# RyoK3N/Camera-Aware-Neural-Networks-for-Few-View-Depth-Estimation

Measured on AMD Instinct MI355X. Metric: images/sec (640×480 bs32) at 1/2/4/8 MI355X; abs_rel vs CPU ref, higher is better.
Workload: dtype fp32; 1 GPU; baseline_unet train step, configs[1]: bs32/GPU 480x640 fp32 SI-only loss; model=baseline, global_batch=32, height=480, width=640, init_features=64, params=31037633, parallelism=dp1, optimizer=adam(lr1e-4,wd1e-5)+clip1.0

## Files before the change

camera-aware-neural-networks-for-few-view-depth-estimation_amd/csrc/host/cad_api.cpp:

```cpp
#include <hip/hip_runtime.h>

#include <algorithm>
#include <cmath>
#include <cstdio>
#include <cstdlib>
#include <cstring>
#include <deque>
#include <memory>
#include <random>
#include <stdexcept>
#include <string>
#include <vector>

#include "../../../include/cad/cad.h"
#include "../kernels/eval_align.hpp"
#include "../kernels/kernels.hpp"

namespace {

thread_local std::string g_err;

struct CadError : std::runtime_error {
    cad_status st;
    CadError(cad_status s, const std::string& m) : std::runtime_error(m), st(s) {}
};

#define HIPCHK(expr)                                                                            \
    do {                                                                                        \
        hipError_t e_ = (expr);                                                                 \
        if (e_ != hipSuccess)                                                                   \
            throw CadError(e_ == hipErrorOutOfMemory ? CAD_ERR_OOM : CAD_ERR_HIP,               \
                           std::string(#expr) + ": " + hipGetErrorString(e_));                 \
    } while (0)

void require(bool c, const std::string& m, cad_status s = CAD_ERR_INVALID) {
    if (!c) throw CadError(s, m);
}

template <class F>
cad_status guard(F&& f) {
    try {
        f();
        return CAD_OK;
    } catch (const CadError& e) {
        g_err = e.what();
        return e.st;
    } catch (const std::exception& e) {
        g_err = e.what();
        return CAD_ERR_INVALID;
    }
}

inline hipStream_t S(void* s) { return reinterpret_cast<hipStream_t>(s); }

struct Arena {
    char* base = nullptr;
    size_t off = 0;
    void* take(size_t bytes) {
        off = (off + 255) & ~size_t(255);
        void* p = base ? base + off : nullptr;
        off += bytes;
        return p;
    }
    float* f(int64_t n) { return static_cast<float*>(take(sizeof(float) * (size_t)std::max<int64_t>(n, 1))); }
    double* d(int64_t n) { return static_cast<double*>(take(sizeof(double) * (size_t)std::max<int64_t>(n, 1))); }
    uint8_t* u8(int64_t n) { return static_cast<uint8_t*>(take((size_t)std::max<int64_t>(n, 1))); }
    int* i(int64_t n) { return static_cast<int*>(take(sizeof(int) * (size_t)std::max<int64_t>(n, 1))); }
};

enum PKind {
    P_CONV3, P_BNW, P_BNB, P_CONVT_W, P_CONVT_B, P_HEAD_W, P_HEAD_B,
    P_FC_W, P_FC_B,
    P_FILM_HEAD_W, P_FILM_GAMMA_B, P_FILM_BETA_B,
    P_SCONV
};

struct PInfo {
    std::string name;
    int ndim;
    int64_t shape[4];
    PKind kind;
    int64_t off;
    int64_t n_int;
    int64_t n_ref;
    int cin_ref = 0, cin_int = 0, cout = 0;
};

struct BufInfo {
    std::string name;
    int64_t C;
    float* ptr;
};

struct BN {
    int C = 0, widx = -1, bidx = -1;
    float *rm = nullptr, *rv = nullptr;
    float *mean = nullptr, *invstd = nullptr, *scale = nullptr, *shift = nullptr, *coef = nullptr;
};
struct Conv {
    int pidx = -1, cin = 0, cout = 0;
    float* wd = nullptr;
    void *ws = nullptr, *wds = nullptr;
};
struct Film {
    int p0 = -1;
    float *rm1, *rv1, *rm2, *rv2;
    float *xh1, *h1, *xh2, *h2, *is1, *is2, *gam, *bet, *dgam, *dbet, *dh2, *dh1;
};
struct DoubleConv {
    Conv c1, c2;
    BN b1, b2;
    Film film;
    int level = 0;
    float *y1 = nullptr, *a1 = nullptr, *y2 = nullptr;
    bool y1b = false, y2b = false;
    bool y1_f32 = false;
    void* a1s = nullptr;
    int first_param = 0, last_param = 0;
    bool has_film() const { return film.p0 >= 0; }
};
struct Up {
    int widx = -1, bidx = -1, cin = 0, cout = 0;
    float* wf = nullptr;
    void *wfs = nullptr, *wms = nullptr;
};

}

namespace cad {
void set_last_error(const std::string& msg) { g_err = msg; }
}

struct cad_unet {
    int device = 0;
    int model = CAD_MODEL_BASELINE;
    int in_ch = 3, f = 64, Bmax = 1, H = 0, W = 0;
    int x0_ld = 8;
    float* camn = nullptr;
    float max_depth = 10.f;
    bool train = true;
    bool have_fwd = false;
    int64_t nbt = 0, nbt_film = 0;
    int fwd_B = 0;
    std::vector<PInfo> params;
    std::vector<BufInfo> bufs;
    int64_t n_flat = 0;
    float *flat_p = nullptr, *flat_g = nullptr;
    float* norm_coef = nullptr;
    void* arena_base = nullptr;
    hipStream_t side = nullptr;
    hipEvent_t ev_fork = nullptr, evA = nullptr, evB = nullptr, ev_tail = nullptr;
    bool defer_join = false;
    float* Sb2 = nullptr;
    void* dYs2 = nullptr;
    double* dscr2 = nullptr;
    DoubleConv enc[5];
    DoubleConv dec[4];
    Up up[4];
    int head_w = -1, head_b = -1;
    int att_p0[4] = {-1, -1, -1, -1};
    cad::Cbam att[4];
    float* zatt[4] = {};
    float* Sd = nullptr;
    float *hq = nullptr, *hdp = nullptr;
    bool att_head_fused = false;
    bool attn() const { return model == CAD_MODEL_INTRINSICS_ATTN; }
    float* x0 = nullptr;
    float* cat[4] = {};
    float* pool[5] = {};
    uint8_t* pidx[5] = {};
    float* a2_bott = nullptr;
    float* dout[4] = {};
    float* sig = nullptr;
    void* x0s = nullptr;
    void* cats[4] = {};
    void* pools[5] = {};
    void* botts = nullptr;
    void* douts[4] = {};
    void* dcats[4] = {};
    void* dskips[4] = {};
    void* dYs = nullptr;
    int fwd_np = 0;
    bool head_fused = false;
    float* dcat[4] = {};
    float *Sa = nullptr, *Sb = nullptr, *Sc = nullptr;
// ... 88 lines not shown
    for (int l = 3; l >= 0; --l) {
        for (int i = h->dec[l].first_param; i <= h->dec[l].last_param; ++i) order.push_back(i);
        for (int j = 0; j < 5; ++j) order.push_back(h->att_p0[l] + j);
    }
    order.push_back(h->head_w);
    order.push_back(h->head_b);
    if (order.size() != h->params.size()) throw std::runtime_error("internal: attention slab order misses a parameter");
    int64_t off = 0;
    for (int i : order) {
        off = (off + 63) & ~int64_t(63);
        h->params[i].off = off;
        off += h->params[i].n_int;
    }
    h->n_flat = (off + 63) & ~int64_t(63);
}

void build_tables(cad_unet* h) {
    const int f = h->f;
    if (h->model == CAD_MODEL_RAY_FILM)
        add_double_conv(h, h->enc[0], "enc1.", h->in_ch + 3, 8, f, 0);
    else
        add_double_conv(h, h->enc[0], "enc1.", h->in_ch, 8, f, 0);
    h->enc[0].y1_f32 = h->model != CAD_MODEL_RAY_FILM;
    const char* enames[4] = {"enc2", "enc3", "enc4", "bottleneck"};
    for (int i = 0; i < 4; ++i)
        add_double_conv(h, h->enc[i + 1], std::string(enames[i]) + ".conv.", f << i, f << i, f << (i + 1), i + 1);
    for (int k = 0; k < 4; ++k) {
        const int l = 3 - k;
        const int cin = f << (l + 1), cout = f << l;
        const std::string pre = "dec" + std::to_string(l + 1) + ".";
        add_param(h, pre + "up.weight", {cin, cout, 2, 2}, P_CONVT_W);
        add_param(h, pre + "up.bias", {cout}, P_CONVT_B);
        h->up[l] = Up{(int)h->params.size() - 2, (int)h->params.size() - 1, cin, cout, nullptr};
        add_double_conv(h, h->dec[l], pre + "conv.", cin, cin, cout, l);
        h->dec[l].first_param = h->up[l].widx;
    }
    if (h->attn()) {
        for (int l = 3; l >= 0; --l) {
            const int C = f << l, Cr = std::max(1, C / 16);
            const std::string pre = "att" + std::to_string(l + 1) + ".";
            h->att_p0[l] = (int)h->params.size();
            add_param(h, pre + "channel_attention.fc1.weight", {Cr, C}, P_FC_W);
            add_param(h, pre + "channel_attention.fc1.bias", {Cr}, P_FC_B);
            add_param(h, pre + "channel_attention.fc2.weight", {C, Cr}, P_FC_W);
            add_param(h, pre + "channel_attention.fc2.bias", {C}, P_FC_B);
            add_param(h, pre + "spatial_attention.conv.weight", {1, 2, 7, 7}, P_SCONV);
        }
    }
    add_param(h, "out_conv.weight", {1, f, 1, 1}, P_HEAD_W);
    add_param(h, "out_conv.bias", {1}, P_HEAD_B);
    h->head_w = (int)h->params.size() - 2;
    h->head_b = (int)h->params.size() - 1;
    h->n_flat = (h->n_flat + 63) & ~int64_t(63);
    if (h->attn()) assign_attn_slab_offsets(h);
}

void bn_alloc(Arena& a, BN& b) {
    b.rm = a.f(b.C); b.rv = a.f(b.C);
    b.mean = a.f(b.C); b.invstd = a.f(b.C); b.scale = a.f(b.C); b.shift = a.f(b.C); b.coef = a.f(3 * b.C);
}

void film_alloc(Arena& a, DoubleConv& dc, int B) {
    if (!dc.has_film()) return;
    Film& F = dc.film;
    const int H1 = cad::kFilmH1, H2 = cad::kFilmH2, C = dc.c1.cout;
    F.rm1 = a.f(H1); F.rv1 = a.f(H1); F.rm2 = a.f(H2); F.rv2 = a.f(H2);
    F.xh1 = a.f((int64_t)B * H1); F.h1 = a.f((int64_t)B * H1); F.dh1 = a.f((int64_t)B * H1);
    F.xh2 = a.f((int64_t)B * H2); F.h2 = a.f((int64_t)B * H2); F.dh2 = a.f((int64_t)B * H2);
    F.is1 = a.f(H1); F.is2 = a.f(H2);
    F.gam = a.f((int64_t)B * C); F.bet = a.f((int64_t)B * C);
    F.dgam = a.f((int64_t)B * C); F.dbet = a.f((int64_t)B * C);
}

void layout(cad_unet* h, Arena& a) {
    const int B = h->Bmax;
    const bool film = h->model != CAD_MODEL_BASELINE;
    auto sp = [&](int64_t elems) -> void* { return a.take((size_t)elems * 2 * cad::kMaxPlanes); };
    auto conv_split_alloc = [&](Conv& c, bool dgrad) {
        if (c.cin % 8) return;
        const int64_t n = (int64_t)c.cout * 9 * c.cin;
        c.ws = sp(n);
        if (dgrad) c.wds = sp(n);
    };
    h->flat_p = a.f(h->n_flat);
    h->flat_g = a.f(h->n_flat);
    h->norm_coef = a.f(4);
    h->camn = a.f((int64_t)B * 4);
    for (int l = 0; l < 5; ++l) {
        DoubleConv& e = h->enc[l];
        bn_alloc(a, e.b1); bn_alloc(a, e.b2);
        const int64_t MC = h->Ml(l, B) * h->Cl(l);
        e.y1 = a.f(MC); e.y2 = a.f(MC);
        e.a1 = a.f(MC);
        e.a1s = sp(MC);
        film_alloc(a, e, B);
        if (l > 0) e.c1.wd = a.f((int64_t)e.c1.cout * 9 * e.c1.cin);
        e.c2.wd = a.f((int64_t)e.c2.cout * 9 * e.c2.cin);
        conv_split_alloc(e.c1, l > 0);
        conv_split_alloc(e.c2, true);
        if (l < 4) { h->cat[l] = a.f(2 * MC); h->cats[l] = sp(2 * MC); }
        if (l > 0) {
            h->pool[l] = a.f(h->Ml(l, B) * h->Cl(l - 1));
            h->pools[l] = sp(h->Ml(l, B) * h->Cl(l - 1));
            h->pidx[l] = a.u8(h->Ml(l, B) * h->Cl(l - 1));
        }
    }
    h->a2_bott = a.f(h->Ml(4, B) * h->Cl(4));
    h->botts = sp(h->Ml(4, B) * h->Cl(4));
    for (int l = 0; l < 4; ++l) {
        DoubleConv& d = h->dec[l];
        bn_alloc(a, d.b1); bn_alloc(a, d.b2);
        const int64_t MC = h->Ml(l, B) * h->Cl(l);
        d.y1 = a.f(MC); d.y2 = a.f(MC);
        d.a1 = a.f(MC);
        d.a1s = sp(MC);
        film_alloc(a, d, B);
        h->dout[l] = a.f(MC);
        if (l > 0) h->douts[l] = sp(MC);
        d.c1.wd = a.f((int64_t)d.c1.cout * 9 * d.c1.cin);
        d.c2.wd = a.f((int64_t)d.c2.cout * 9 * d.c2.cin);
        conv_split_alloc(d.c1, true);
        conv_split_alloc(d.c2, true);
        h->up[l].wf = a.f((int64_t)4 * h->up[l].cout * h->up[l].cin);
        h->up[l].wfs = sp((int64_t)4 * h->up[l].cout * h->up[l].cin);
        h->up[l].wms = sp((int64_t)4 * h->up[l].cout * h->up[l].cin);
        h->dcat[l] = a.f(2 * MC);
        h->dcats[l] = sp(MC);
        h->dskips[l] = sp(MC);
    }
    h->x0 = a.f(h->Ml(0, B) * h->x0_ld);
    if (h->x0_ld % 8 == 0) h->x0s = sp(h->Ml(0, B) * h->x0_ld);
    h->dYs = sp(h->Ml(0, B) * h->Cl(0));
    h->sig = a.f(h->Ml(0, B));
    const int64_t M0C0 = h->Ml(0, B) * h->Cl(0);
    h->Sa = a.f(M0C0);
    h->Sb = a.f(M0C0);
    h->Sb2 = a.f(M0C0);
    h->dYs2 = sp(h->Ml(0, B) * h->Cl(0));
    h->Sc = a.f(h->Ml(1, B) * h->Cl(0));
    if (h->attn()) {
        h->Sd = a.f(M0C0);
        for (int l = 0; l < 4; ++l) {
            const int C = h->Cl(l), Cr = std::max(1, C / 16);
            const int64_t M = h->Ml(l, B);
            const bool fused = l == 0 && cad::head_fusable(C);
            h->zatt[l] = fused ? nullptr : a.f(M * C);
            cad::Cbam& A = h->att[l];
            A.C = C; A.Cr = Cr;
            A.avg = a.f((int64_t)B * C); A.mx = a.f((int64_t)B * C); A.amax = a.i((int64_t)B * C);
            A.ha = a.f((int64_t)B * Cr); A.hm = a.f((int64_t)B * Cr); A.att = a.f((int64_t)B * C);
            A.s = a.f(2 * M); A.sidx = a.i(M); A.sa = a.f(M);
            A.dlog = a.f(M); A.ds = a.f(2 * M);
            A.dO = a.f((int64_t)B * C); A.dha = a.f((int64_t)B * Cr); A.dhm = a.f((int64_t)B * Cr);
            A.dva = a.f((int64_t)B * C); A.dvm = a.f((int64_t)B * C);
            if (fused) { h->hq = a.f(M); h->hdp = a.f(M); }
        }
    }
    int64_t st = 0, colmax = 0;
    for (int l = 0; l < 5; ++l) {
        const int64_t r = (h->Ml(l, B) + 63) / 64;
        st = std::max<int64_t>(st, r * (2 * h->Cl(l) + 1));
        colmax = std::max<int64_t>(colmax, h->Cl(l));
    }
    h->stats = a.f(st);
    int64_t dscr = (int64_t)(cad::colsum_slices(h->Ml(0, B)) + 2) * 4 * colmax + 4 * colmax + 8192;
    for (int l = 0; l < 5 && film; ++l)
        dscr = std::max(dscr, cad::film_reduce_doubles(B, (int64_t)h->Hl(l) * h->Wl(l), h->Cl(l)) + 8192);
    for (int l = 0; l < 4 && h->attn(); ++l)
        dscr = std::max(dscr, cad::cbam_head_scratch_doubles(B, (int64_t)h->Hl(l) * h->Wl(l), h->Cl(l)) + 8192);
    h->dscr = a.d(dscr);
    h->dscr2 = a.d(dscr);
    int64_t sl = 0;
    for (int l = 0; l < 5; ++l) {
        const int64_t Kp = h->Ml(l, B);
        sl = std::max(sl, cad::wgrad_slab_floats(h->Cl(l), 9 * h->Cl(l) * 2, (int)std::min<int64_t>(Kp, INT32_MAX)));
    }
    h->slab_cap = std::min<int64_t>(sl, (int64_t)64 << 20);
    h->slab = a.f(h->slab_cap);
    h->part_cap = (h->Ml(0, B) + 63) / 64 * 2 * h->Cl(0);
    h->rc_part = a.d(h->part_cap);
    h->bufs.clear();
    auto add_bn_bufs = [&](const std::string& pre, BN& b) {
        h->bufs.push_back({pre + ".running_mean", b.C, b.rm});
        h->bufs.push_back({pre + ".running_var", b.C, b.rv});
    };
    auto add_block = [&](const std::string& pre, DoubleConv& dc) {
        add_bn_bufs(pre + "bn1", dc.b1);
        add_bn_bufs(pre + "bn2", dc.b2);
        if (!dc.has_film()) return;
        h->bufs.push_back({pre + "film.bn1.running_mean", cad::kFilmH1, dc.film.rm1});
        h->bufs.push_back({pre + "film.bn1.running_var", cad::kFilmH1, dc.film.rv1});
        h->bufs.push_back({pre + "film.bn2.running_mean", cad::kFilmH2, dc.film.rm2});
        h->bufs.push_back({pre + "film.bn2.running_var", cad::kFilmH2, dc.film.rv2});
    };
    const char* en[5] = {"enc1.", "enc2.conv.", "enc3.conv.", "enc4.conv.", "bottleneck.conv."};
    for (int l = 0; l < 5; ++l) add_block(en[l], h->enc[l]);
    for (int k = 0; k < 4; ++k) {
        const int l = 3 - k;
        add_block("dec" + std::to_string(l + 1) + ".conv.", h->dec[l]);
    }
}

cad::FilmLayer film_view(const cad_unet* h, const DoubleConv& dc) {
    const Film& F = dc.film;
    const int i = F.p0;
    cad::FilmLayer L;
    L.C = dc.c1.cout;
    L.w1 = h->P(i); L.b1 = h->P(i + 1); L.w2 = h->P(i + 2); L.b2 = h->P(i + 3);
    L.wg = h->P(i + 4); L.bg = h->P(i + 5); L.wb = h->P(i + 6); L.bb = h->P(i + 7);
    L.g1 = h->P(i + 8); L.be1 = h->P(i + 9); L.g2 = h->P(i + 10); L.be2 = h->P(i + 11);
    L.rm1 = F.rm1; L.rv1 = F.rv1; L.rm2 = F.rm2; L.rv2 = F.rv2;
    L.xh1 = F.xh1; L.h1 = F.h1; L.xh2 = F.xh2; L.h2 = F.h2; L.is1 = F.is1; L.is2 = F.is2;
    L.gam = F.gam; L.bet = F.bet; L.dgam = F.dgam; L.dbet = F.dbet; L.dh2 = F.dh2; L.dh1 = F.dh1;
    L.gw1 = h->G(i); L.gb1 = h->G(i + 1); L.gw2 = h->G(i + 2); L.gb2 = h->G(i + 3);
    L.gwg = h->G(i + 4); L.gbg = h->G(i + 5); L.gwb = h->G(i + 6); L.gbb = h->G(i + 7);
    L.gg1 = h->G(i + 8); L.gbe1 = h->G(i + 9); L.gg2 = h->G(i + 10); L.gbe2 = h->G(i + 11);
    return L;
}

cad::Cbam cbam_view(const cad_unet* h, int l) {
    cad::Cbam A = h->att[l];
    const int i = h->att_p0[l];
    A.w1 = h->P(i); A.b1 = h->P(i + 1); A.w2 = h->P(i + 2); A.b2 = h->P(i + 3); A.wsp = h->P(i + 4);
    A.gw1 = h->G(i); A.gb1 = h->G(i + 1); A.gw2 = h->G(i + 2); A.gb2 = h->G(i + 3); A.gwsp = h->G(i + 4);
    return A;
}
cad::CbamHead cbam_head_view(const cad_unet* h) {
    const DoubleConv& d = h->dec[0];
    cad::CbamHead Hd;
    Hd.y = d.y2; Hd.y_bf16 = d.y2b;
    Hd.scale = d.b2.scale; Hd.shift = d.b2.shift;
    Hd.w = h->P(h->head_w); Hd.b = h->P(h->head_b);
    Hd.md = h->max_depth;
    Hd.q = h->hq; Hd.sig = h->sig; Hd.dp = h->hdp;
    Hd.gw = h->G(h->head_w); Hd.gb = h->G(h->head_b);
    return Hd;
}

cad::Split sv(const void* p, int64_t ld, int coff = 0) {
    cad::Split v;
    v.p = p; v.ld = ld; v.coff = coff;
    return v;
}
void split_into(const float* x, int64_t ldx, int xcoff, int C, int64_t M, void* out, int64_t ldo, int ocoff,
                hipStream_t st) {
    if (out) cad::split_rows(x, ldx, xcoff, C, M, out, ldo, ocoff, st);
}
void wprep_add(cad::WPrepList& L, int kind, const float* src, float* d32, void* d16, int cout, int cin, int64_t n) {
    if (!d32 && !d16) return;
    if (L.njobs == cad::kWPrepMaxJobs) throw std::runtime_error("weight_prep: job list full");
    cad::WPrepJob& j = L.job[L.njobs++];
    j.src = src; j.d32 = d32; j.d16 = d16; j.kind = kind; j.cout = cout; j.cin = cin; j.n = n;
}
void prep_fwd_weights(const cad_unet* h, bool ps, hipStream_t st) {
    cad::WPrepList L{};
    for (int l = 0; l < 4; ++l) {
        const Up& u = h->up[l];
        wprep_add(L, cad::WPREP_CONVT, h->P(u.widx), u.wf, ps ? u.wfs : nullptr, u.cout, u.cin, (int64_t)4 * u.cout * u.cin);
    }
    if (ps) {
        auto sw = [&](const Conv& c) {
            if (c.ws) wprep_add(L, cad::WPREP_SPLIT, h->P(c.pidx), nullptr, c.ws, c.cout, c.cin, (int64_t)c.cout * 9 * c.cin);
        };
        for (int l = 0; l < 5; ++l) { sw(h->enc[l].c1); sw(h->enc[l].c2); }
        for (int l = 0; l < 4; ++l) { sw(h->dec[l].c1); sw(h->dec[l].c2); }
    }
    cad::weight_prep(L, st);
}

int env_flag(const char* name, int dflt) {
    const char* e = std::getenv(name);
    return e && e[0] ? std::atoi(e) : dflt;
}
bool conv1_presplit(cad_unet* h, const DoubleConv& dc, bool ps, const cad::Split& in_s) {
    static const bool enc1_ps = env_flag("CAD_ENC1PS", 1) != 0;
    return ps && in_s.p && dc.c1.ws && (enc1_ps || &dc != &h->enc[0]);
}
struct PoolOut {
    float* pool;
    uint8_t* idx;
    void* pool_s;
};
bool bn_pool_on() {
    static const bool on = env_flag("CAD_BNPOOL", 1) != 0;
    return on;
}

void double_conv_fwd(cad_unet* h, DoubleConv& dc, const float* in, int64_t ldin, cad::Split in_s, int B, float* out,
                     int64_t ldo, int ocoff, cad::Split out_s, hipStream_t st, bool out_f32 = true,
                     float* head_pred = nullptr, const PoolOut* pool = nullptr, bool att_head = false) {
    const int l = dc.level, Hh = h->Hl(l), Ww = h->Wl(l), C = dc.c1.cout;
    const int64_t M = h->Ml(l, B);
    const bool tr = h->train;
    const bool ps = h->fwd_np > 0;
    auto bn = [&](BN& b, int cin, bool ps_conv) {
        const int rows = cad::conv3x3_stats_rows(cin, B, Hh, Ww, C, ps_conv);
        if (tr)
            cad::bn_fwd_finalize(h->stats, rows, C, M, h->P(b.widx), h->P(b.bidx), b.rm, b.rv, 0.1f, 1e-5f, h->dscr,
                                 b.mean, b.invstd, b.scale, b.shift, st);
        else
            cad::bn_eval_coeffs(h->P(b.widx), h->P(b.bidx), b.rm, b.rv, C, 1e-5f, b.mean, b.invstd, b.scale, b.shift, st);
    };
    float* stats = tr ? h->stats : nullptr;
    const bool ps1 = conv1_presplit(h, dc, ps, in_s);
    static const bool enc1_bf16 = env_flag("CAD_ENC1BF16", 0) != 0;
    dc.y1b = ps1 && (!dc.y1_f32 || enc1_bf16);
    dc.y2b = ps;
    if (ps1) {
        cad::conv3x3_fwd_ps(in_s, dc.c1.cin, sv(dc.c1.ws, 9 * dc.c1.cin), C, dc.y1, C, 0, B, Hh, Ww, stats, st, dc.y1b);
    } else {
        cad::conv3x3_fwd(in, ldin, 0, dc.c1.cin, h->P(dc.c1.pidx), C, dc.y1, C, 0, B, Hh, Ww, stats, st);
    }
    bn(dc.b1, dc.c1.cin, ps1);
    if (dc.has_film()) {
        cad::film_apply(dc.y1, C, dc.b1.scale, dc.b1.shift, dc.film.gam, dc.film.bet, B, (int64_t)Hh * Ww,
                        ps ? nullptr : dc.a1, st, dc.y1b, ps ? dc.a1s : nullptr);
    } else {
        cad::bn_relu_fwd(dc.y1, C, dc.b1.scale, dc.b1.shift, ps ? nullptr : dc.a1, C, 0, M, st, ps ? dc.a1s : nullptr,
                         C, 0, dc.y1b);
    }
    if (ps)
        cad::conv3x3_fwd_ps(sv(dc.a1s, C), C, sv(dc.c2.ws, 9 * C), C, dc.y2, C, 0, B, Hh, Ww, stats, st, true);
    else
        cad::conv3x3_fwd(dc.a1, C, 0, C, h->P(dc.c2.pidx), C, dc.y2, C, 0, B, Hh, Ww, stats, st);
    bn(dc.b2, C, ps);
    if (head_pred && att_head) {
        cad::cbam_head_fwd(cbam_view(h, 0), cbam_head_view(h), B, Hh, Ww, head_pred, h->dscr, st);
        return;
    }
    if (head_pred) {
        cad::bn_relu_head_fwd(dc.y2, C, dc.b2.scale, dc.b2.shift, h->P(h->head_w), h->P(h->head_b), h->max_depth, h->sig,
                              head_pred, M, st, dc.y2b);
        return;
    }
    const bool twin = ps && out_s.p;
    if (pool) {
        if (ocoff != 0 || (twin && out_s.coff != 0)) throw std::runtime_error("bn_relu_pool_fwd: offset outputs");
        cad::bn_relu_pool_fwd(dc.y2, C, dc.b2.scale, dc.b2.shift, (out_f32 || !twin) ? out : nullptr, ldo,
                              twin ? const_cast<void*>(out_s.p) : nullptr, out_s.ld, B, Hh, Ww, dc.y2b, pool->pool,
                              pool->idx, pool->pool_s, st);
        return;
    }
    cad::bn_relu_fwd(dc.y2, C, dc.b2.scale, dc.b2.shift, (out_f32 || !twin) ? out : nullptr, ldo, ocoff, M, st,
                     twin ? const_cast<void*>(out_s.p) : nullptr, out_s.ld, out_s.coff, dc.y2b);
}

bool dcat_split_on() {
    static const bool on = env_flag("CAD_DCATSPLIT", 1) != 0;
    return on;
}

bool pool_fold_on() {
    static const bool on = env_flag("CAD_POOLFOLD", 1) != 0;
    return on;
}

bool head_fusion_on() {
    static const bool on = [] {
        const char* e = std::getenv("CAD_HEADFUSE");
        return !(e && e[0] == '0');
    }();
    return on;
}

void unet_forward(cad_unet* h, const float* rgb, const float* cam4, float* depth, int B, hipStream_t st) {
    const int f = h->f;
    h->fwd_np = h->f % 8 ? 0 : cad::split_planes();
    const bool ps = h->fwd_np > 0;
    prep_fwd_weights(h, ps, st);
    if (h->model != CAD_MODEL_BASELINE) {
        cad::camera_normalize(cam4, B, h->H, h->W, h->camn, st);
        cad::FilmList fl;
        for (int l = 0; l < 5; ++l) fl.l[fl.n++] = film_view(h, h->enc[l]);
        for (int l = 3; l >= 0; --l) fl.l[fl.n++] = film_view(h, h->dec[l]);
        cad::film_mlp_fwd_all(fl, h->camn, B, h->train, st);
    }
    if (h->model == CAD_MODEL_RAY_FILM)
        cad::rgb_rays_to_nhwc8(rgb, cam4, B, h->H, h->W, h->x0, st);
    else
        cad::rgb_to_nhwc8(rgb, h->x0, B, h->H, h->W, st);
    const cad::Split none{};
    cad::Split x0s = none;
    if (ps && h->x0s) {
        cad::split_rows(h->x0, h->x0_ld, 0, h->x0_ld, h->Ml(0, B), h->x0s, h->x0_ld, 0, st);
        x0s = sv(h->x0s, h->x0_ld);
    }
    auto pool_of = [&](int l) {
        const bool ptwin = ps && h->pools[l];
        return PoolOut{ptwin ? nullptr : h->pool[l], h->pidx[l], ptwin ? h->pools[l] : nullptr};
    };
    const bool fuse_pool = bn_pool_on();
    PoolOut po = pool_of(1);
    double_conv_fwd(h, h->enc[0], h->x0, h->x0_ld, x0s, B, h->cat[0], 2 * f, 0, sv(h->cats[0], 2 * f), st, !ps, nullptr,
                    fuse_pool ? &po : nullptr);
    for (int l = 1; l <= 4; ++l) {
        const int Cp = h->Cl(l - 1);
        if (!fuse_pool) {
            const PoolOut p = pool_of(l);
            cad::maxpool_fwd(ps ? static_cast<const float*>(h->cats[l - 1]) : h->cat[l - 1], 2 * Cp, Cp, B, h->Hl(l - 1),
                             h->Wl(l - 1), p.pool, p.idx, st, p.pool_s, ps);
        }
        const cad::Split pin = sv(h->pools[l], Cp);
        if (l < 4) {
            po = pool_of(l + 1);
            double_conv_fwd(h, h->enc[l], h->pool[l], Cp, pin, B, h->cat[l], 2 * h->Cl(l), 0,
                            sv(h->cats[l], 2 * h->Cl(l)), st, !ps, nullptr, fuse_pool ? &po : nullptr);
        } else {
// ... 3 lines not shown
    }
    const bool attn = h->attn();
    h->head_fused = !attn && head_fusion_on() && cad::head_fusable(f);
    h->att_head_fused = attn && cad::head_fusable(f);
    for (int l = 3; l >= 0; --l) {
        const float* upin = l == 3 ? h->a2_bott : h->dout[l + 1];
        const void* upins = l == 3 ? h->botts : h->douts[l + 1];
        const Up& u = h->up[l];
        const int C = h->Cl(l);
        if (ps) {
            cad::convT_fwd_ps(sv(upins, u.cin), u.cin, sv(u.wfs, u.cin), h->P(u.bidx), u.cout,
                              static_cast<float*>(h->cats[l]), 2 * C, C, B, h->Hl(l + 1), h->Wl(l + 1), st, true);
        } else {
            cad::convT_fwd(upin, u.cin, u.cin, u.wf, h->P(u.bidx), u.cout, h->cat[l], 2 * C, C, B, h->Hl(l + 1),
                           h->Wl(l + 1), st);
        }
        if (attn) {
            if (l == 0 && h->att_head_fused) {
                double_conv_fwd(h, h->dec[0], h->cat[0], 2 * C, sv(h->cats[0], 2 * C), B, nullptr, C, 0, none, st, true,
                                depth, nullptr, true);
                continue;
            }
            double_conv_fwd(h, h->dec[l], h->cat[l], 2 * C, sv(h->cats[l], 2 * C), B, h->zatt[l], C, 0, none, st, true);
            cad::cbam_fwd(cbam_view(h, l), h->zatt[l], B, h->Hl(l), h->Wl(l), h->dout[l], C, 0, h->dscr, st);
            if (ps && l > 0) cad::split_rows(h->dout[l], C, 0, C, h->Ml(l, B), h->douts[l], C, 0, st);
            continue;
        }
        double_conv_fwd(h, h->dec[l], h->cat[l], 2 * C, sv(h->cats[l], 2 * C), B, h->dout[l], C, 0,
                        l > 0 ? sv(h->douts[l], C) : none, st, l == 0, l == 0 && h->head_fused ? depth : nullptr);
    }
    if (!h->head_fused && !h->att_head_fused)
        cad::head_fwd(h->dout[0], f, h->P(h->head_w), h->P(h->head_b), h->max_depth, h->sig, depth, h->Ml(0, B), st);
}

void side_fork(cad_unet* h, hipStream_t st) {
    HIPCHK(hipEventRecord(h->ev_fork, st));
    HIPCHK(hipStreamWaitEvent(h->side, h->ev_fork, 0));
}
void side_join(cad_unet* h, hipStream_t st) {
    HIPCHK(hipEventRecord(h->ev_tail, h->side));
    HIPCHK(hipStreamWaitEvent(st, h->ev_tail, 0));
}
hipStream_t wgrad_stream(cad_unet* h, bool ps, hipStream_t st) {
    const int f = env_flag("CAD_SIDE_WGRAD", -1);
    const bool side = f < 0 ? !ps : f != 0;
    if (!side) return st;
    side_fork(h, st);
    return h->side;
}

void double_conv_bwd(cad_unet* h, DoubleConv& dc, const float* g, int64_t ldg, int gcoff, const float* in,
                     int64_t ldin, cad::Split in_s, int B, float* din, int64_t lddin, hipStream_t st,
                     const cad::HeadGrad* head = nullptr, const cad::PoolAdd* pool = nullptr, void* din_hi = nullptr,
                     bool* din_hi_done = nullptr, bool g_bf16 = false, bool din_bf16 = false) {
    const int l = dc.level, Hh = h->Hl(l), Ww = h->Wl(l), C = dc.c1.cout;
    const int64_t M = h->Ml(l, B);
    const bool ps = h->fwd_np > 0 && h->fwd_np == cad::split_planes();
    hipStream_t sd = h->side;
    float* dY = h->Sb;
    void* dYs = h->dYs;
    float* dY1 = h->Sb2;
    void* dYs1 = h->dYs2;
    float* dA1 = h->Sa;
    HIPCHK(hipStreamWaitEvent(st, h->evA, 0));
    cad::bn_relu_bwd(g, ldg, gcoff, dc.y2, C, dc.b2.mean, dc.b2.invstd, dc.b2.scale, dc.b2.shift, h->P(dc.b2.widx), M,
                     h->dscr, dc.b2.coef, h->G(dc.b2.widx), h->G(dc.b2.bidx), ps ? nullptr : dY, st, nullptr, 1,
                     ps ? dYs : nullptr, true, dc.y2b, head, g_bf16, pool);
    static const bool bnsums = env_flag("CAD_BNSUMS", 1) != 0;
    int bn1_tiles = 0;
    cad::BnSums bs;
    if (bnsums && !ps && !dc.has_film() && h->rc_part) {
        bs.y = dc.y1; bs.ldy = C; bs.y_bf16 = dc.y1b;
        bs.mean = dc.b1.mean; bs.invstd = dc.b1.invstd; bs.scale = dc.b1.scale; bs.shift = dc.b1.shift;
        bs.part = h->rc_part; bs.part_cap = h->part_cap;
    }
    hipStream_t wg = wgrad_stream(h, ps, st);
    if (ps) {
        cad::conv3x3_wgrad_ps(sv(dYs, C), C, sv(dc.a1s, C), C, h->G(dc.c2.pidx), B, Hh, Ww, h->slab, h->slab_cap, wg);
        HIPCHK(hipEventRecord(h->evA, wg));
        cad::conv3x3_dgrad_ps(sv(dYs, C), C, sv(dc.c2.wds, 9 * C), C, dA1, C, B, Hh, Ww, st, true);
    } else {
        cad::conv3x3_wgrad(dY, C, dc.a1, C, 0, C, h->G(dc.c2.pidx), B, Hh, Ww, h->slab, h->slab_cap, wg);
        HIPCHK(hipEventRecord(h->evA, wg));
        if (bs.part) bn1_tiles = cad::conv3x3_dgrad_bnsums(dY, C, dc.c2.wd, C, dA1, C, B, Hh, Ww, bs, st);
        if (!bn1_tiles) cad::conv3x3_dgrad(dY, C, dc.c2.wd, C, dA1, C, B, Hh, Ww, st);
    }
    const int64_t HW = (int64_t)Hh * Ww;
    static const bool film_fuse = env_flag("CAD_FILMFUSE", 1) != 0;
    const bool film_sep = dc.has_film() && !film_fuse;
    if (film_sep)
        cad::film_affine_bwd(dA1, dc.y1, C, dc.b1.scale, dc.b1.shift, B, HW, h->dscr, dc.film.dgam, dc.film.dbet, st,
                             dc.y1b, ps);
    const bool ps1 = conv1_presplit(h, dc, ps, in_s);
    const bool dy1_f32 = !ps1 || (din && !(ps && dc.c1.wds));
    HIPCHK(hipStreamWaitEvent(st, h->evB, 0));
    {
        const bool ff = dc.has_film() && !film_sep;
        cad::bn_relu_bwd(dA1, C, 0, dc.y1, C, dc.b1.mean, dc.b1.invstd, dc.b1.scale, dc.b1.shift, h->P(dc.b1.widx), M,
                         h->dscr, dc.b1.coef, h->G(dc.b1.widx), h->G(dc.b1.bidx), dy1_f32 ? dY1 : nullptr, st,
                         dc.has_film() ? dc.film.gam : nullptr, HW, ps ? dYs1 : nullptr, true, dc.y1b, nullptr, ps,
                         nullptr, ff ? dc.film.dgam : nullptr, ff ? dc.film.dbet : nullptr,
                         bn1_tiles ? h->rc_part : nullptr, bn1_tiles);
    }
    if (dc.has_film()) {
        side_fork(h, st);
        cad::film_mlp_bwd(film_view(h, dc), h->camn, B, sd);
    }
    hipStream_t wg1 = wgrad_stream(h, ps, st);
    if (ps1)
        cad::conv3x3_wgrad_ps(sv(dYs1, C), C, in_s, dc.c1.cin, h->G(dc.c1.pidx), B, Hh, Ww, h->slab, h->slab_cap, wg1);
    else
        cad::conv3x3_wgrad(dY1, C, in, ldin, 0, dc.c1.cin, h->G(dc.c1.pidx), B, Hh, Ww, h->slab, h->slab_cap, wg1);
    HIPCHK(hipEventRecord(h->evB, wg1));
    if (din) {
        if (ps && dc.c1.wds) {
            const bool done = cad::conv3x3_dgrad_ps(sv(dYs1, C), C, sv(dc.c1.wds, 9 * C), dc.c1.cin, din, lddin, B, Hh,
                                                    Ww, st, din_bf16, din_hi, dc.c1.cin / 2, dc.c1.cin / 2);
            if (din_hi_done) *din_hi_done = done && din_hi;
        } else
            cad::conv3x3_dgrad(dY1, C, dc.c1.wd, dc.c1.cin, din, lddin, B, Hh, Ww, st);
    }
}

void repack_dgrad_weights(cad_unet* h, hipStream_t st) {
    const bool ps = h->fwd_np > 0 && h->fwd_np == cad::split_planes();
    cad::WPrepList L{};
    auto rp = [&](Conv& c) {
        wprep_add(L, cad::WPREP_DGRAD, h->P(c.pidx), c.wd, ps ? c.wds : nullptr, c.cout, c.cin, (int64_t)c.cout * 9 * c.cin);
    };
    for (int l = 0; l < 5; ++l) {
        if (l > 0) rp(h->enc[l].c1);
        rp(h->enc[l].c2);
    }
    for (int l = 0; l < 4; ++l) {
        rp(h->dec[l].c1);
        rp(h->dec[l].c2);
        const Up& u = h->up[l];
        if (ps) wprep_add(L, cad::WPREP_SPLIT, h->P(u.widx), nullptr, u.wms, u.cout, u.cin, (int64_t)4 * u.cout * u.cin);
    }
    cad::weight_prep(L, st);
}

constexpr int kStages = 10;

void backward_stage_body(cad_unet* h, int stage, const float* dpred, hipStream_t st);
void backward_stage(cad_unet* h, int stage, const float* dpred, hipStream_t st) {
    backward_stage_body(h, stage, dpred, st);
    if (!h->defer_join) side_join(h, st);
}
void backward_stage_body(cad_unet* h, int stage, const float* dpred, hipStream_t st) {
    const int B = h->fwd_B;
    const int f = h->f;
    const bool ps = h->fwd_np > 0 && h->fwd_np == cad::split_planes();
    if (stage == 0) {
        HIPCHK(hipEventRecord(h->evA, st));
        HIPCHK(hipEventRecord(h->evB, st));
        repack_dgrad_weights(h, st);
        if (h->attn()) {
            if (h->att_head_fused) {
                cad::cbam_head_bwd(cbam_view(h, 0), cbam_head_view(h), dpred, B, h->H, h->W, h->Sa, h->dscr, st);
            } else {
                cad::head_bwd(h->dout[0], f, h->P(h->head_w), dpred, h->sig, h->max_depth, h->Sd, h->Ml(0, B), h->dscr,
                              h->G(h->head_w), h->G(h->head_b), st);
                cad::cbam_bwd(cbam_view(h, 0), h->zatt[0], h->Sd, f, 0, B, h->H, h->W, h->Sa, h->dscr, st);
            }
            return;
        }
        if (h->head_fused) {
            const DoubleConv& d = h->dec[0];
            cad::head_bwd_y(d.y2, f, d.b2.scale, d.b2.shift, dpred, h->sig, h->max_depth, h->Ml(0, B), h->dscr,
                            h->G(h->head_w), h->G(h->head_b), st, d.y2b);
        } else {
            cad::head_bwd(h->dout[0], f, h->P(h->head_w), dpred, h->sig, h->max_depth, h->Sa, h->Ml(0, B), h->dscr,
                          h->G(h->head_w), h->G(h->head_b), st);
        }
        return;
    }
    if (stage <= 4) {
        const int l = stage - 1;
        const int C = h->Cl(l);
        const cad::HeadGrad hg{dpred, h->sig, h->P(h->head_w), h->max_depth};
        const bool hf = l == 0 && h->head_fused;
        const bool split = ps && dcat_split_on() &&
                           cad::conv3x3_dgrad_split_ok(sv(h->dYs, C), C, sv(h->dec[l].c1.wds, 9 * C), 2 * C, h->Wl(l), C);
        bool up_twin = false;
        const bool attn = h->attn();
        const float* g = h->Sa;
        if (attn && l > 0) {
            cad::cbam_bwd(cbam_view(h, l), h->zatt[l], h->Sa, C, 0, B, h->Hl(l), h->Wl(l), h->Sd, h->dscr, st);
            g = h->Sd;
        }
        double_conv_bwd(h, h->dec[l], hf ? nullptr : g, C, 0, h->cat[l], 2 * C, sv(h->cats[l], 2 * C), B,
                        split ? static_cast<float*>(h->dskips[l]) : h->dcat[l], split ? C : 2 * C, st,
                        hf ? &hg : nullptr, nullptr, split ? h->dcats[l] : nullptr, &up_twin, ps && l > 0 && !attn, split);
        if (split != up_twin) throw std::runtime_error("decoder dgrad split store not taken");
        const Up& u = h->up[l];
        const float* upin = l == 3 ? h->a2_bott : h->dout[l + 1];
        const void* upins = l == 3 ? h->botts : h->douts[l + 1];
        if (ps && !split) {
            cad::split_rows(h->dcat[l], 2 * C, C, C, h->Ml(l, B), h->dcats[l], C, 0, st);
            cad::split_rows(h->dcat[l], 2 * C, 0, C, h->Ml(l, B), h->dskips[l], C, 0, st);
        }
        hipStream_t sd = wgrad_stream(h, ps, st);
        if (ps) {
            cad::convT_wgrad_ps(sv(upins, u.cin), u.cin, sv(h->dcats[l], C), u.cout, h->G(u.widx), B, h->Hl(l + 1),
                                h->Wl(l + 1), h->slab, h->slab_cap, sd);
        } else {
            cad::convT_wgrad(upin, u.cin, h->dcat[l], 2 * C, C, u.cout, h->G(u.widx), B, h->Hl(l + 1), h->Wl(l + 1),
                             h->slab, h->slab_cap, sd);
        }
        if (ps) cad::colsum_bf16(h->dcats[l], C, 0, h->Ml(l, B), C, h->dscr2, sd);
// ... 1495 lines not shown
        HIPCHK(hipEventRecord(b->staged, S(stream)));
        float* rgb_tmp = b->tmp;
        float* depth_tmp = b->tmp + 3 * (size_t)b->Bmax * H * W;
        cad::batch_assemble(b->dev, B, H, W, any_aug, any_color, rgb, depth, rgb_tmp, depth_tmp, S(stream));
        HIPCHK(hipGetLastError());
    });
}

struct cad_aug_sampler {
    cad_aug_config cfg;
    std::mt19937 rng;
};
cad_status cad_aug_sampler_create(const cad_aug_config* cfg, uint32_t seed, cad_aug_sampler** out) {
    return guard([&] {
        require(cfg && out, "null argument");
        require(cfg->crop_scale_min > 0.f && cfg->crop_scale_min <= cfg->crop_scale_max && cfg->crop_scale_max <= 1.f,
                "crop scale range must satisfy 0 < min <= max <= 1");
        require(cfg->saturation_delta >= 0.f && cfg->saturation_delta <= 1.f, "saturation_delta must be in [0, 1]");
        require(cfg->hue_delta >= 0.f && cfg->hue_delta <= 0.5f, "hue_delta must be in [0, 0.5]");
        if (cfg->enable_random_gamma) {
            require(std::isfinite(cfg->gamma_min) && cfg->gamma_min > 0.f, "gamma_min must be positive and finite");
            require(std::isfinite(cfg->gamma_max) && cfg->gamma_max >= cfg->gamma_min, "gamma_max must be finite and at least gamma_min");
        }
        auto s = std::make_unique<cad_aug_sampler>();
        s->cfg = *cfg;
        s->rng.seed(seed);
        *out = s.release();
    });
}
void cad_aug_sampler_destroy(cad_aug_sampler* s) { delete s; }
cad_status cad_aug_sampler_draw(cad_aug_sampler* s, int height, int width, cad_sample* smp) {
    return guard([&] {
        require(s && smp && height >= 1 && width >= 1, "bad arguments");
        const cad_aug_config& c = s->cfg;
        smp->aug = 1;
        smp->crop = c.enable_random_crop;
        if (c.enable_random_crop) {
            std::uniform_real_distribution<float> scale_dist(c.crop_scale_min, c.crop_scale_max);
            const float scale = scale_dist(s->rng);
            const int crop_h = static_cast<int>(height * scale), crop_w = static_cast<int>(width * scale);
            std::uniform_int_distribution<int> x_dist(0, std::max(1, width - crop_w));
            std::uniform_int_distribution<int> y_dist(0, std::max(1, height - crop_h));
            smp->crop_scale = scale;
            smp->crop_x = x_dist(s->rng);
            smp->crop_y = y_dist(s->rng);
        }
        smp->flip = 0;
        if (c.enable_horizontal_flip) {
            std::uniform_real_distribution<float> flip_dist(0.0f, 1.0f);
            smp->flip = flip_dist(s->rng) < c.horizontal_flip_prob;
        }
        smp->jitter = c.enable_color_jitter;
        if (c.enable_color_jitter) {
            std::uniform_real_distribution<float> bd(1.0f - c.brightness_delta, 1.0f + c.brightness_delta);
            std::uniform_real_distribution<float> cd(1.0f - c.contrast_delta, 1.0f + c.contrast_delta);
            smp->brightness = bd(s->rng);
            smp->contrast = cd(s->rng);
        }
        smp->color = 0; smp->saturation = 1.f; smp->hue = 0.f;
        if (c.enable_color_jitter && c.saturation_delta > 0.f) {
            std::uniform_real_distribution<float> sd(1.0f - c.saturation_delta, 1.0f + c.saturation_delta);
            smp->saturation = sd(s->rng);
            smp->color = 1;
        }
        if (c.enable_color_jitter && c.hue_delta > 0.f) {
            std::uniform_real_distribution<float> hd(-c.hue_delta, c.hue_delta);
            smp->hue = hd(s->rng);
            smp->color = 1;
        }
        smp->gamma_on = c.enable_random_gamma ? 1 : 0;
        smp->gamma = 1.f;
        if (c.enable_random_gamma) {
            std::uniform_real_distribution<float> gd(c.gamma_min, c.gamma_max);
            smp->gamma = gd(s->rng);
        }
    });
}

cad_status cad_op_conv3x3_fwd(const float* x, int64_t ldx, int xcoff, int cin, const float* w, int cout, float* y,
                              int64_t ldy, int ycoff, int B, int H, int W, void* stream) {
    return guard([&] {
        require(cin % 4 == 0 && cout % 4 == 0 && ldx % 4 == 0 && ldy % 4 == 0 && xcoff % 4 == 0 && ycoff % 4 == 0,
                "channels / strides must be multiples of 4");
        cad::conv3x3_fwd(x, ldx, xcoff, cin, w, cout, y, ldy, ycoff, B, H, W, nullptr, S(stream));
        HIPCHK(hipGetLastError());
    });
}
cad_status cad_op_conv3x3_dgrad(const float* dz, int cout, const float* w, int cin, float* dx, int64_t lddx, int B,
                                int H, int W, void* stream) {
    return guard([&] {
        require(cin % 4 == 0 && cout % 4 == 0, "channels must be multiples of 4");
        float* wd = nullptr;
        HIPCHK(hipMallocAsync((void**)&wd, sizeof(float) * (size_t)cout * 9 * cin, S(stream)));
        cad::repack_conv_dgrad(w, wd, cout, cin, S(stream));
        cad::conv3x3_dgrad(dz, cout, wd, cin, dx, lddx, B, H, W, S(stream));
        HIPCHK(hipFreeAsync(wd, S(stream)));
        HIPCHK(hipGetLastError());
    });
}
cad_status cad_op_conv3x3_wgrad(const float* dz, int cout, const float* x, int64_t ldx, int xcoff, int cin, float* dw,
                                int B, int H, int W, void* stream) {
    return guard([&] {
        require(cin % 4 == 0 && cout % 4 == 0, "channels must be multiples of 4");
        const int64_t cap = cad::wgrad_slab_floats(cout, 9 * cin, B * H * W);
        float* slab = nullptr;
        HIPCHK(hipMallocAsync((void**)&slab, sizeof(float) * (size_t)std::max<int64_t>(cap, 4), S(stream)));
        cad::conv3x3_wgrad(dz, cout, x, ldx, xcoff, cin, dw, B, H, W, slab, cap, S(stream));
        HIPCHK(hipFreeAsync(slab, S(stream)));
        HIPCHK(hipGetLastError());
    });
}
cad_status cad_op_conv3x3_wgrad_bf16(const void* dz, int64_t lddz, int cout, const void* x, int64_t ldx, int xcoff,
                                     int cin, float* dw, int B, int H, int W, void* stream) {
    return guard([&] {
        require(cad::gemm_engine() == 2, "the pre-split weight gradient runs on the bf16 engine (CAD_GEMM_BF16)");
        const int64_t cap = cad::wgrad_slab_floats(cout, 9 * cin, B * H * W);
        float* slab = nullptr;
        HIPCHK(hipMallocAsync((void**)&slab, sizeof(float) * (size_t)std::max<int64_t>(cap, 4), S(stream)));
        cad::conv3x3_wgrad_ps(cad::Split{dz, lddz, 0}, cout, cad::Split{x, ldx, xcoff}, cin, dw, B, H, W, slab, cap,
                              S(stream));
        HIPCHK(hipFreeAsync(slab, S(stream)));
        HIPCHK(hipGetLastError());
    });
}
cad_status cad_op_conv3x3_fwd_bf16(const void* x, int64_t ldx, int xcoff, int cin, const float* w, int cout, void* y,
                                  int64_t ldy, int ycoff, int y_bf16, int with_stats, int B, int H, int W, void* stream) {
    return guard([&] {
        require(cad::gemm_engine() == 2, "the pre-split convolution runs on the bf16 engine (CAD_GEMM_BF16)");
        require(x && w && y && cin % 8 == 0 && xcoff % 8 == 0 && ldx % 8 == 0 && B > 0 && H > 0 && W > 0,
                "bad arguments (bf16 rows: ldx, xcoff, cin multiples of 8)");
        void* ws = nullptr;
        float* stats = nullptr;
        HIPCHK(hipMallocAsync(&ws, sizeof(uint16_t) * (size_t)cout * 9 * cin, S(stream)));
        cad::split_rows(w, 9 * cin, 0, 9 * cin, cout, ws, 9 * cin, 0, S(stream));
        if (with_stats) {
            const int rows = cad::conv3x3_stats_rows(cin, B, H, W, cout, true);
            HIPCHK(hipMallocAsync((void**)&stats, sizeof(float) * ((size_t)rows * (2 * cout + 1) + 4), S(stream)));
        }
        cad::conv3x3_fwd_ps(cad::Split{x, ldx, xcoff}, cin, cad::Split{ws, 9 * cin, 0}, cout, static_cast<float*>(y), ldy,
                            ycoff, B, H, W, stats, S(stream), y_bf16 != 0);
        if (stats) HIPCHK(hipFreeAsync(stats, S(stream)));
        HIPCHK(hipFreeAsync(ws, S(stream)));
        HIPCHK(hipGetLastError());
    });
}
cad_status cad_op_conv3x3_dgrad_bf16(const void* dz, int64_t lddz, int cout, const float* w, int cin, void* dx,
                                    int64_t lddx, int dx_bf16, int B, int H, int W, void* stream) {
    return guard([&] {
        require(cad::gemm_engine() == 2, "the pre-split convolution runs on the bf16 engine (CAD_GEMM_BF16)");
        require(dz && w && dx && cout % 8 == 0 && cin % 8 == 0 && lddz % 8 == 0 && B > 0 && H > 0 && W > 0,
                "bad arguments (bf16 rows: lddz, cout, cin multiples of 8)");
        float* wd = nullptr;
        void* wds = nullptr;
        HIPCHK(hipMallocAsync((void**)&wd, sizeof(float) * (size_t)cout * 9 * cin, S(stream)));
        HIPCHK(hipMallocAsync(&wds, sizeof(uint16_t) * (size_t)cout * 9 * cin, S(stream)));
        cad::repack_conv_dgrad(w, wd, cout, cin, S(stream));
        cad::split_rows(wd, 9 * cout, 0, 9 * cout, cin, wds, 9 * cout, 0, S(stream));
        cad::conv3x3_dgrad_ps(cad::Split{dz, lddz, 0}, cout, cad::Split{wds, 9 * cout, 0}, cin, static_cast<float*>(dx),
                              lddx, B, H, W, S(stream), dx_bf16 != 0);
        HIPCHK(hipFreeAsync(wds, S(stream)));
        HIPCHK(hipFreeAsync(wd, S(stream)));
        HIPCHK(hipGetLastError());
    });
}
cad_status cad_op_mx8_quantize(const void* src, int src_bf16, int64_t lds, int scoff, int C, int64_t M, void* q,
                               void* s, int64_t ldq, int qcoff, void* stream) {
    return guard([&] {
        require(src && q && s && M >= 0, "null argument");
        cad::Mx8 d;
        d.q = q; d.s = s; d.ld = ldq; d.coff = qcoff;
        cad::mx8_quantize(src, src_bf16 != 0, lds, scoff, C, M, d, S(stream));
        HIPCHK(hipGetLastError());
    });
}
cad_status cad_op_dense_x8(const void* xq, const void* xs, int64_t ldx, int K, const void* wq, const void* ws,
                           int64_t ldw, int N, float* y, int64_t M, void* stream) {
    return guard([&] {
        require(cad::dense_x8_ok(K, N), "dense MX-fp8 GEMM: K % 128 == 0 and N % 64 == 0 required");
// ... 81 lines not shown
```

camera-aware-neural-networks-for-few-view-depth-estimation_amd/csrc/kernels/conv_kernels.hip:

```cpp
#include <algorithm>
#include <cstdio>
#include <cstdlib>
#include <stdexcept>

#include "gemm_mfma.hpp"
#include "gemm_s3.hpp"
#include "gemm_ps.hpp"
#include "gemm_win.hpp"
#include "kernels.hpp"
#include "epilogues.hpp"

namespace cad {

template <int WM, int WN, int KB, class Epi>
__global__ __launch_bounds__(256) void k_conv3x3_fwd(GemmArgs a) {
    using LA = KcIm2col3x3<64 * WM, KB>;
    using LB = KcDense<64 * WN, KB>;
    gemm_body<WM, WN, KB, LA, true, LB, true>(
        a,
        [&](LA& l, int r0, int t, int kb) { l.init(a.A, a.lda, a.a_coff, a.a_cin, a.B, a.H, a.W, r0, t, kb); },
        [&](LB& l, int r0, int t, int kb) { l.init(a.Bm, a.ldb, a.b_coff, a.N, a.K, r0, t, kb); }, Epi{});
}

template <int WM, int WN, int KB>
// ... 9 lines not shown
__global__ __launch_bounds__(256) void k_convT_dgrad(GemmArgs a) {
    using LA = KcUpGather<64 * WM, KB>;
    using LB = KcDense<64 * WN, KB>;
    gemm_body<WM, WN, KB, LA, true, LB, true>(
        a, [&](LA& l, int r0, int t, int kb) { l.init(a.A, a.lda, a.a_coff, a.a_cin, a.B, a.H, a.W, r0, t, kb); },
        [&](LB& l, int r0, int t, int kb) { l.init(a.Bm, a.ldb, a.b_coff, a.N, a.K, r0, t, kb); }, EpiStore{});
}

template <int WM, int WN, int KB>
__global__ __launch_bounds__(256) void k_conv3x3_wgrad(GemmArgs a) {
    using LA = MNcDense<64 * WM, KB>;
    using LB = MNcIm2col3x3<64 * WN, KB>;
    gemm_body<WM, WN, KB, LA, false, LB, false>(
        a, [&](LA& l, int r0, int t, int kb) { l.init(a.A, a.lda, a.a_coff, a.M, a.K, r0, t, kb); },
        [&](LB& l, int r0, int t, int kb) { l.init(a.Bm, a.ldb, a.b_coff, a.b_cin, a.B, a.H, a.W, r0, t, kb); },
        EpiSlab{});
}

template <int WM, int WN, int KB>
__global__ __launch_bounds__(256) void k_convT_wgrad(GemmArgs a) {
    using LA = MNcDense<64 * WM, KB>;
    using LB = MNcUpGather<64 * WN, KB>;
    gemm_body<WM, WN, KB, LA, false, LB, false>(
        a, [&](LA& l, int r0, int t, int kb) { l.init(a.A, a.lda, a.a_coff, a.M, a.K, r0, t, kb); },
        [&](LB& l, int r0, int t, int kb) { l.init(a.Bm, a.ldb, a.b_coff, a.b_cin, a.B, a.H, a.W, r0, t, kb); },
        EpiSlab{});
}

template <int NP, int WM, int WN, int MI, int NJ, int KB, class Epi>
__device__ __forceinline__ void conv3x3_fwd_np(const GemmArgs& a) {
    using LA = KcIm2col3x3<32 * MI * WM, KB>;
    using LB = KcDense<32 * NJ * WN, KB>;
    gemm_body_s3<NP, WM, WN, MI, NJ, KB, LA, LB>(
        a,
        [&](LA& l, int r0, int t, int kb) { l.init(a.A, a.lda, a.a_coff, a.a_cin, a.B, a.H, a.W, r0, t, kb); },
        [&](LB& l, int r0, int t, int kb) { l.init(a.Bm, a.ldb, a.b_coff, a.N, a.K, r0, t, kb); }, Epi{});
}
template <int NP, int WM, int WN, int MI, int NJ, int KB>
__device__ __forceinline__ void convT_fwd_np(const GemmArgs& a) {
    using LA = KcDense<32 * MI * WM, KB>;
    using LB = KcDense<32 * NJ * WN, KB>;
    gemm_body_s3<NP, WM, WN, MI, NJ, KB, LA, LB>(
        a, [&](LA& l, int r0, int t, int kb) { l.init(a.A, a.lda, a.a_coff, a.M, a.K, r0, t, kb); },
        [&](LB& l, int r0, int t, int kb) { l.init(a.Bm, a.ldb, a.b_coff, a.N, a.K, r0, t, kb); }, EpiConvT{});
}
template <int NP, int WM, int WN, int MI, int NJ, int KB>
__device__ __forceinline__ void convT_dgrad_np(const GemmArgs& a) {
    using LA = KcUpGather<32 * MI * WM, KB>;
    using LB = KcDense<32 * NJ * WN, KB>;
    gemm_body_s3<NP, WM, WN, MI, NJ, KB, LA, LB>(
        a, [&](LA& l, int r0, int t, int kb) { l.init(a.A, a.lda, a.a_coff, a.a_cin, a.B, a.H, a.W, r0, t, kb); },
        [&](LB& l, int r0, int t, int kb) { l.init(a.Bm, a.ldb, a.b_coff, a.N, a.K, r0, t, kb); }, EpiStore{});
}
template <int NP, int WM, int WN, int MI, int NJ, int KB>
__device__ __forceinline__ void conv3x3_wgrad_np(const GemmArgs& a) {
    using LA = MNcDense<32 * MI * WM, KB>;
    using LB = MNcIm2col3x3<32 * NJ * WN, KB>;
    gemm_body_s3m<NP, WM, WN, MI, NJ, KB, LA, LB>(
        a, [&](LA& l, int r0, int t, int kb) { l.init(a.A, a.lda, a.a_coff, a.M, a.K, r0, t, kb); },
        [&](LB& l, int r0, int t, int kb) { l.init(a.Bm, a.ldb, a.b_coff, a.b_cin, a.B, a.H, a.W, r0, t, kb); },
        EpiSlab{});
}
template <int NP, int WM, int WN, int MI, int NJ, int KB>
__device__ __forceinline__ void convT_wgrad_np(const GemmArgs& a) {
    using LA = MNcDense<32 * MI * WM, KB>;
    using LB = MNcUpGather<32 * NJ * WN, KB>;
    gemm_body_s3m<NP, WM, WN, MI, NJ, KB, LA, LB>(
        a, [&](LA& l, int r0, int t, int kb) { l.init(a.A, a.lda, a.a_coff, a.M, a.K, r0, t, kb); },
        [&](LB& l, int r0, int t, int kb) { l.init(a.Bm, a.ldb, a.b_coff, a.b_cin, a.B, a.H, a.W, r0, t, kb); },
        EpiSlab{});
}

template <int WM, int WN, int KB, class Epi>
__global__ __launch_bounds__(256) void k_conv3x3_fwd_s3(GemmArgs a) { conv3x3_fwd_np<3, WM, WN, 2, 2, KB, Epi>(a); }
template <int WM, int WN, int KB>
__global__ __launch_bounds__(256) void k_convT_fwd_s3(GemmArgs a) { convT_fwd_np<3, WM, WN, 2, 2, KB>(a); }
template <int WM, int WN, int KB>
__global__ __launch_bounds__(256) void k_convT_dgrad_s3(GemmArgs a) { convT_dgrad_np<3, WM, WN, 2, 2, KB>(a); }
template <int WM, int WN, int KB>
__global__ __launch_bounds__(256) void k_conv3x3_wgrad_s3(GemmArgs a) { conv3x3_wgrad_np<3, WM, WN, 2, 2, KB>(a); }
template <int WM, int WN, int KB>
__global__ __launch_bounds__(256) void k_convT_wgrad_s3(GemmArgs a) { convT_wgrad_np<3, WM, WN, 2, 2, KB>(a); }

template <int R, int CW, class Epi>
__global__ __launch_bounds__(256, 3) void k_conv3x3_win_s3(GemmArgs a) {
    conv3x3_win_body<3, R, CW, R * CW == 128 ? 2 : 4, R * CW == 128 ? 2 : 1, Epi>(a);
}

template <int R, int CW, class Epi>
__global__ __launch_bounds__(256, 3) void k_conv3x3_win_bf16p(GemmArgs a) {
    conv3x3_win_ps_body<R, CW, R * CW == 128 ? 2 : 4, R * CW == 128 ? 2 : 1, Epi>(a);
}
template <int R, int CW, class Epi, bool BN64 = false>
__global__ __launch_bounds__(256, 2) void k_conv3x3_win_bf16p4(GemmArgs a) {
    conv3x3_win_ps_body<R, CW, BN64 ? 4 : 2, BN64 ? 1 : 2, Epi, 4, 2, (CW <= 16) || (CAD_WIN16 != 0)>(a);
}

template <int R, int CW, class Epi>
__global__ __launch_bounds__(256, 2) void k_conv3x3_win_bf16p3(GemmArgs a) {
    conv3x3_win_ps_body<R, CW, 4, 1, Epi, 2, 3>(a);
}

__global__ __launch_bounds__(256, 2) void k_conv3x3_wgrad_win_s3(GemmArgs a) { conv3x3_wgrad_win_body<3>(a); }
__global__ __launch_bounds__(256, 2) void k_conv3x3_wgrad_strip_s3(GemmArgs a) { conv3x3_wgrad_strip_body<3>(a); }
template <int P>
__global__ __launch_bounds__(256, 2) void k_conv3x3_wgrad_win_bf16p(GemmArgs a) { conv3x3_wgrad_win_ps_body<P>(a); }
template <int P, int NBUF>
__global__ __launch_bounds__(256, 2) void k_conv3x3_wgrad_win_bf16d(GemmArgs a) { conv3x3_wgrad_win_dma_body<P, NBUF>(a); }
template <int P>
__global__ __launch_bounds__(256, 2) void k_conv3x3_wgrad_strip_bf16d(GemmArgs a) { conv3x3_wgrad_strip_dma_body<P>(a); }
template <int P>
__global__ __launch_bounds__(256, 2) void k_conv3x3_wgrad_strip2_bf16d(GemmArgs a) { conv3x3_wgrad_strip2_dma_body<P>(a); }

template <int WM, int WN, int KB, class Epi>
__global__ __launch_bounds__(256) void k_conv3x3_fwd_bf16(GemmArgs a) { conv3x3_fwd_np<1, WM, WN, 2, 2, KB, Epi>(a); }
template <int WM, int WN, int KB>
__global__ __launch_bounds__(256) void k_convT_fwd_bf16(GemmArgs a) { convT_fwd_np<1, WM, WN, 2, 2, KB>(a); }
template <int WM, int WN, int KB>
__global__ __launch_bounds__(256) void k_convT_dgrad_bf16(GemmArgs a) { convT_dgrad_np<1, WM, WN, 2, 2, KB>(a); }
template <int WM, int WN, int KB>
__global__ __launch_bounds__(256) void k_conv3x3_wgrad_bf16(GemmArgs a) { conv3x3_wgrad_np<1, WM, WN, 2, 2, KB>(a); }
template <int WM, int WN, int KB>
__global__ __launch_bounds__(256) void k_convT_wgrad_bf16(GemmArgs a) { convT_wgrad_np<1, WM, WN, 2, 2, KB>(a); }

template <int NP, int WM, int WN, int MI, int NJ, int KB, class Epi>
__device__ __forceinline__ void conv3x3_fwd_psb(const GemmArgs& a) {
    using LA = PsKcIm2col3x3<32 * MI * WM, KB, NP>;
    using LB = PsKcDense<32 * NJ * WN, KB, NP>;
    gemm_body_ps<NP, WM, WN, MI, NJ, KB, LA, LB>(
        a,
        [&](LA& l, int r0, int t, int kb) {
            l.init(a.A, a.lda, a.a_coff, a.a_cin, a.B, a.H, a.W, r0, t, kb, a.cimajor);
        },
        [&](LB& l, int r0, int t, int kb) { l.init(a.Bm, a.ldb, a.b_coff, a.N, a.K, r0, t, kb, a.cimajor, a.a_cin); },
        Epi{});
}
template <int NP, int WM, int WN, int MI, int NJ, int KB, class Epi = EpiConvT>
__device__ __forceinline__ void convT_fwd_psb(const GemmArgs& a) {
    using LA = PsKcDense<32 * MI * WM, KB, NP>;
    using LB = PsKcDense<32 * NJ * WN, KB, NP>;
    gemm_body_ps<NP, WM, WN, MI, NJ, KB, LA, LB>(
        a, [&](LA& l, int r0, int t, int kb) { l.init(a.A, a.lda, a.a_coff, a.M, a.K, r0, t, kb); },
        [&](LB& l, int r0, int t, int kb) { l.init(a.Bm, a.ldb, a.b_coff, a.N, a.K, r0, t, kb); }, Epi{});
}
template <int NP, int WM, int WN, int MI, int NJ, int KB, class Epi = EpiStore>
__device__ __forceinline__ void convT_dgrad_psb(const GemmArgs& a) {
    using LA = PsKcUpGather<32 * MI * WM, KB, NP>;
    using LB = PsKcDense<32 * NJ * WN, KB, NP>;
    gemm_body_ps<NP, WM, WN, MI, NJ, KB, LA, LB>(
        a, [&](LA& l, int r0, int t, int kb) { l.init(a.A, a.lda, a.a_coff, a.a_cin, a.B, a.H, a.W, r0, t, kb); },
        [&](LB& l, int r0, int t, int kb) { l.init(a.Bm, a.ldb, a.b_coff, a.N, a.K, r0, t, kb); }, Epi{});
}
template <int NP, int WM, int WN, int MI, int NJ, int KB>
__device__ __forceinline__ void conv3x3_wgrad_psb(const GemmArgs& a) {
    using LA = PsMNcDense<32 * MI * WM, KB, NP>;
    using LB = PsMNcIm2col3x3<32 * NJ * WN, KB, NP>;
    gemm_body_psm<NP, WM, WN, MI, NJ, KB, LA, LB>(
        a, [&](LA& l, int r0, int t, int kb) { l.init(a.A, a.lda, a.a_coff, a.M, a.K, r0, t, kb); },
        [&](LB& l, int r0, int t, int kb) { l.init(a.Bm, a.ldb, a.b_coff, a.b_cin, a.B, a.H, a.W, r0, t, kb); },
        EpiSlab{});
}
template <int NP, int WM, int WN, int MI, int NJ, int KB>
__device__ __forceinline__ void convT_wgrad_psb(const GemmArgs& a) {
    using LA = PsMNcDense<32 * MI * WM, KB, NP>;
    using LB = PsMNcUpGather<32 * NJ * WN, KB, NP>;
    gemm_body_psm<NP, WM, WN, MI, NJ, KB, LA, LB>(
        a, [&](LA& l, int r0, int t, int kb) { l.init(a.A, a.lda, a.a_coff, a.M, a.K, r0, t, kb); },
        [&](LB& l, int r0, int t, int kb) { l.init(a.Bm, a.ldb, a.b_coff, a.b_cin, a.B, a.H, a.W, r0, t, kb); },
        EpiSlab{});
// ... 116 lines not shown
        hipLaunchKernelGGL(K::fn(), grid, dim3(256), 0, st, a);
        prof_pop(st);
    } else {
        hipLaunchKernelGGL(K::fn(), grid, dim3(256), 0, st, a);
    }
}
template <template <int, int, int> class KT, int KB>
void launch_cfg(Cfg c, const GemmArgs& a, int splits, hipStream_t st) {
    switch (c) {
        case C41: launch_one<KT, 4, 1, KB>(a, splits, st); break;
        case C22: launch_one<KT, 2, 2, KB>(a, splits, st); break;
        case C14: launch_one<KT, 1, 4, KB>(a, splits, st); break;
    }
}
template <template <int, int, int> class KT, int... KBs>
void launch_kb(Cfg c, int kb, const GemmArgs& a, int splits, hipStream_t st) {
    const bool done = ((kb == KBs ? (launch_cfg<KT, KBs>(c, a, splits, st), true) : false) || ...);
    if (!done) throw std::runtime_error("GEMM stage depth not built for this kernel family");
}
#define CAD_KT(NAME, EXPR, FMT)                                                  \
    template <int WM, int WN, int KB> struct NAME {                              \
        static auto fn() { return EXPR; }                                        \
        static constexpr const char* fmt = FMT;                                  \
    };
CAD_KT(KConvFwd, (k_conv3x3_fwd<WM, WN, KB, EpiStore>), "void cad::k_conv3x3_fwd<%d, %d, %d, cad::EpiStore>(cad::GemmArgs)")
CAD_KT(KConvFwdS, (k_conv3x3_fwd<WM, WN, KB, EpiStoreStats>),
       "void cad::k_conv3x3_fwd<%d, %d, %d, cad::EpiStoreStats>(cad::GemmArgs)")
CAD_KT(KConvWgrad, (k_conv3x3_wgrad<WM, WN, KB>), "void cad::k_conv3x3_wgrad<%d, %d, %d>(cad::GemmArgs)")
CAD_KT(KConvTFwd, (k_convT_fwd<WM, WN, KB>), "void cad::k_convT_fwd<%d, %d, %d>(cad::GemmArgs)")
CAD_KT(KConvTDgrad, (k_convT_dgrad<WM, WN, KB>), "void cad::k_convT_dgrad<%d, %d, %d>(cad::GemmArgs)")
CAD_KT(KConvTWgrad, (k_convT_wgrad<WM, WN, KB>), "void cad::k_convT_wgrad<%d, %d, %d>(cad::GemmArgs)")
#define CAD_NP_KT(SUF, T)                                                                                  \
    CAD_KT(KConvFwd##T, (k_conv3x3_fwd_##SUF<WM, WN, KB, EpiStore>),                                       \
           "void cad::k_conv3x3_fwd_" #SUF "<%d, %d, %d, cad::EpiStore>(cad::GemmArgs)")                   \
    CAD_KT(KConvFwdS##T, (k_conv3x3_fwd_##SUF<WM, WN, KB, EpiStoreStats>),                                 \
           "void cad::k_conv3x3_fwd_" #SUF "<%d, %d, %d, cad::EpiStoreStats>(cad::GemmArgs)")              \
    CAD_KT(KConvTFwd##T, (k_convT_fwd_##SUF<WM, WN, KB>), "void cad::k_convT_fwd_" #SUF "<%d, %d, %d>(cad::GemmArgs)") \
    CAD_KT(KConvTDgrad##T, (k_convT_dgrad_##SUF<WM, WN, KB>),                                              \
           "void cad::k_convT_dgrad_" #SUF "<%d, %d, %d>(cad::GemmArgs)")                                  \
    CAD_KT(KConvWgrad##T, (k_conv3x3_wgrad_##SUF<WM, WN, KB>),                                             \
           "void cad::k_conv3x3_wgrad_" #SUF "<%d, %d, %d>(cad::GemmArgs)")                                \
    CAD_KT(KConvTWgrad##T, (k_convT_wgrad_##SUF<WM, WN, KB>),                                              \
           "void cad::k_convT_wgrad_" #SUF "<%d, %d, %d>(cad::GemmArgs)")
CAD_KT(KDenseP1, (k_dense_bf16p<WM, WN, KB, EpiStore>), "void cad::k_dense_bf16p<%d, %d, %d, cad::EpiStore>(cad::GemmArgs)")
CAD_KT(KDenseSP1, (k_dense_bf16p<WM, WN, KB, EpiStoreStats>),
       "void cad::k_dense_bf16p<%d, %d, %d, cad::EpiStoreStats>(cad::GemmArgs)")
CAD_KT(KDenseP1B, (k_dense_bf16p<WM, WN, KB, EpiStoreB16>), "void cad::k_dense_bf16p<%d, %d, %d, cad::EpiStoreB16>(cad::GemmArgs)")
CAD_KT(KDenseSP1B, (k_dense_bf16p<WM, WN, KB, EpiStoreStatsB16>),
       "void cad::k_dense_bf16p<%d, %d, %d, cad::EpiStoreStatsB16>(cad::GemmArgs)")
CAD_KT(KConvFwdP1B, (k_conv3x3_fwd_bf16p<WM, WN, KB, EpiStoreB16>),
       "void cad::k_conv3x3_fwd_bf16p<%d, %d, %d, cad::EpiStoreB16>(cad::GemmArgs)")
CAD_KT(KConvFwdSP1B, (k_conv3x3_fwd_bf16p<WM, WN, KB, EpiStoreStatsB16>),
       "void cad::k_conv3x3_fwd_bf16p<%d, %d, %d, cad::EpiStoreStatsB16>(cad::GemmArgs)")
CAD_KT(KDenseWgradP1, (k_dense_wgrad_bf16p<WM, WN, KB>), "void cad::k_dense_wgrad_bf16p<%d, %d, %d>(cad::GemmArgs)")
CAD_KT(KConvTFwdP1T, (k_convT_fwd_bf16pt<WM, WN, KB>), "void cad::k_convT_fwd_bf16pt<%d, %d, %d>(cad::GemmArgs)")
CAD_KT(KConvTDgradP1B, (k_convT_dgrad_bf16pb<WM, WN, KB>), "void cad::k_convT_dgrad_bf16pb<%d, %d, %d>(cad::GemmArgs)")
CAD_KT(KDenseAddP1, (k_dense_bf16p<WM, WN, KB, EpiStoreAdd>), "void cad::k_dense_bf16p<%d, %d, %d, cad::EpiStoreAdd>(cad::GemmArgs)")
CAD_NP_KT(s3, 3)
CAD_NP_KT(bf16, B)
CAD_NP_KT(bf16p, P1)
#undef CAD_NP_KT
#undef CAD_KT

template <template <int, int, int> class F, template <int, int, int> class T3, template <int, int, int> class TB>
void launch_on_engine(Cfg c, int kb, const GemmArgs& a, int splits, hipStream_t st) {
    if (engine() == 1) launch_kb<T3, kS3KB>(c, kb, a, splits, st);
    else if (engine() == 2) launch_kb<TB, kB1KB>(c, kb, a, splits, st);
    else launch_kb<F, 16, 32>(c, kb, a, splits, st);
}
int engine_kb(bool fwd_kind, Cfg c) { return engine() == 1 ? kS3KB : engine() == 2 ? kB1KB : f32_kb(fwd_kind, c); }
template <template <int, int, int> class F, template <int, int, int> class T3, template <int, int, int> class TB>
void launch_engine(Cfg c, bool fwd_kind, GemmArgs& a, hipStream_t st) {
    const int kb = engine_kb(fwd_kind, c);
    a.kstages_per_split = cdiv(a.K, kb);
    launch_on_engine<F, T3, TB>(c, kb, a, 1, st);
}

struct WinPick {
    int R = 0, CW = 0;
    bool big = false;
    bool n96 = false;
    int bn() const { return n96 ? 96 : big ? (R * CW == 256 ? 128 : 64) : R * CW == 128 ? 128 : 64; }
};
WinPick pick_win(int cin, int W, int N) {
    WinPick w;
    if (engine() != 1 || cin % 16) return w;
    const int BM = N <= 64 ? 256 : 128;
    if (N % (BM == 128 ? 128 : 64)) return w;
    static const int c128[] = {64, 32, 16, 8}, c256[] = {128, 64};
    const int* cws = BM == 128 ? c128 : c256;
    const int ncw = BM == 128 ? 4 : 2;
    for (int i = 0; i < ncw; ++i)
        if (W % cws[i] == 0) {
            w.CW = cws[i];
            w.R = BM / cws[i];
            return w;
        }
    return w;
}
int win_blocks(const WinPick& w, int B, int H, int W) { return B * cdiv(H, w.R) * (W / w.CW); }
template <bool PS, int R, int CW, class Epi, bool BIG = false, bool N96 = false>
void launch_win1(const GemmArgs& a, hipStream_t st) {
    constexpr int BN = N96 ? 96 : BIG ? (R * CW == 256 ? 128 : 64) : R * CW == 128 ? 128 : 64;
    if (a.N % BN) throw std::runtime_error("window conv: N not a multiple of the tile");
    const dim3 grid(win_blocks(WinPick{R, CW}, a.B, a.H, a.W), cdiv(a.N, BN));
    void (*fn)(GemmArgs);
    if constexpr (N96) fn = k_conv3x3_win_bf16p3<R, CW, Epi>;
    else if constexpr (BIG) fn = k_conv3x3_win_bf16p4<R, CW, Epi, BN == 64>;
    else fn = PS ? (void (*)(GemmArgs))k_conv3x3_win_bf16p<R, CW, Epi> : (void (*)(GemmArgs))k_conv3x3_win_s3<R, CW, Epi>;
    if (prof_enabled()) {
        char name[160];
        snprintf(name, sizeof(name), "void cad::k_conv3x3_win_%s<%d, %d, cad::%s%s>(cad::GemmArgs)",
                 N96 ? "bf16p3" : BIG ? "bf16p4" : PS ? "bf16p" : "s3", R, CW,
                 Epi::STATS ? "EpiStoreStats" : is_bnsums<Epi>::value ? "EpiStoreBnSums" : "EpiStore",
                 Epi::BF16 ? "B16" : "");
        prof_push(name, 2.0 * a.M * a.N * (double)a.K, st);
        hipLaunchKernelGGL(fn, grid, dim3(256), 0, st, a);
        prof_pop(st);
    } else {
        hipLaunchKernelGGL(fn, grid, dim3(256), 0, st, a);
    }
}
template <class Epi, bool PS = false>
void launch_win(const WinPick& w, const GemmArgs& a, hipStream_t st) {
    if constexpr (PS) {
        if (w.n96) {
            switch (w.CW) {
                case 128: launch_win1<PS, 2, 128, Epi, true, true>(a, st); return;
                case 64: launch_win1<PS, 4, 64, Epi, true, true>(a, st); return;
                case 32: launch_win1<PS, 8, 32, Epi, true, true>(a, st); return;
                case 16: launch_win1<PS, 16, 16, Epi, true, true>(a, st); return;
                case 8: launch_win1<PS, 32, 8, Epi, true, true>(a, st); return;
            }
            throw std::runtime_error("window conv: block shape not built");
        }
        if (w.big && w.R * w.CW == 256) {
            switch (w.CW) {
                case 128: launch_win1<PS, 2, 128, Epi, true>(a, st); return;
                case 64: launch_win1<PS, 4, 64, Epi, true>(a, st); return;
                case 32: launch_win1<PS, 8, 32, Epi, true>(a, st); return;
                case 16: launch_win1<PS, 16, 16, Epi, true>(a, st); return;
                case 8: launch_win1<PS, 32, 8, Epi, true>(a, st); return;
            }
            throw std::runtime_error("window conv: block shape not built");
        }
        if (w.big) {
            switch (w.CW) {
                case 128: launch_win1<PS, 4, 128, Epi, true>(a, st); return;
                case 64: launch_win1<PS, 8, 64, Epi, true>(a, st); return;
            }
            throw std::runtime_error("window conv: block shape not built");
        }
    }
    if (w.R * w.CW == 128) {
        switch (w.CW) {
            case 64: launch_win1<PS, 2, 64, Epi>(a, st); return;
            case 32: launch_win1<PS, 4, 32, Epi>(a, st); return;
            case 16: launch_win1<PS, 8, 16, Epi>(a, st); return;
            case 8: launch_win1<PS, 16, 8, Epi>(a, st); return;
        }
    } else {
        switch (w.CW) {
            case 128: launch_win1<PS, 2, 128, Epi>(a, st); return;
            case 64: launch_win1<PS, 4, 64, Epi>(a, st); return;
        }
    }
    throw std::runtime_error("window conv: block shape not built");
}
WinPick pick_win_ps(int cin, int W, int N, int acoff) {
    WinPick w;
    if (engine() != 2 || cin % 32 || acoff % 8) return w;
    if (N % 128 == 0) {
        static const int cb[] = {128, 64, 32, 16, 8};
        for (int cw : cb)
            if (W % cw == 0) {
                w.CW = cw;
                w.R = 256 / cw;
                w.big = true;
                return w;
            }
        return w;
    }
    static const bool big64 = [] {
        const char* e = std::getenv("CAD_WIN64");
        return !(e && e[0] == '0');
    }();
    if (N == 64 && big64 && (W % 128 == 0 || W % 64 == 0)) {
        w.CW = W % 128 == 0 ? 128 : 64;
        w.R = 512 / w.CW;
        w.big = true;
        return w;
    }
    if (N % 96 == 0) {
        static const int cb[] = {128, 64, 32, 16, 8};
        for (int cw : cb)
            if (W % cw == 0) {
                w.CW = cw;
                w.R = 256 / cw;
// ... 166 lines not shown
    if (s > 1 && (int64_t)s * per > slab_cap) return false;
    float* out = s == 1 ? dw : slab;
    const dim3 grid(s, cout / 64);
    if (prof_enabled()) prof_push("cad::k_wgrad_narrow_s3", 2.0 * M * per, st);
    if (9 * cin <= 32)
        hipLaunchKernelGGL(k_wgrad_narrow_s3<1>, grid, dim3(256), 0, st, dz, ldz, x, ldx, xoff, cin, cout, B, H, W, ppw, out);
    else if (9 * cin <= 64)
        hipLaunchKernelGGL(k_wgrad_narrow_s3<2>, grid, dim3(256), 0, st, dz, ldz, x, ldx, xoff, cin, cout, B, H, W, ppw, out);
    else
        hipLaunchKernelGGL(k_wgrad_narrow_s3<3>, grid, dim3(256), 0, st, dz, ldz, x, ldx, xoff, cin, cout, B, H, W, ppw, out);
    if (prof_enabled()) prof_pop(st);
    if (s > 1) finish_slabs(slab, s, per, dw, st);
    return true;
}

bool use_wgrad_win(int cout, int cin, int W) {
    return engine() == 1 && cout % 64 == 0 && cin % 64 == 0 && W % 16 == 0;
}
bool wg_strip() {
    static const bool on = [] {
        const char* e = std::getenv("CAD_WGSTRIP");
        return !(e && e[0] == '0');
    }();
    return on;
}
void launch_wgrad_win(GemmArgs& a, float* dw, float* slab, int64_t slab_cap, int64_t kbytes, hipStream_t st) {
    const int cin = a.b_cin;
    const int tiles = (a.M / 64) * (cin / 64);
    const int nst = a.K / 16;
    const bool strip = wg_strip();
    int s = std::max(1, std::min(cdiv(2048, tiles), nst / 32));
    const int64_t per = (int64_t)a.M * a.N;
    if (slab_cap > 0) s = (int)std::max<int64_t>(1, std::min<int64_t>(s, slab_cap / per));
    const int64_t img = (int64_t)a.H * a.W;
    auto span_ok = [&](int splits) {
        const int64_t px = (int64_t)cdiv(nst, splits) * 16;
        const int64_t span = strip ? (cdiv(px, img) + 1) * img : px;
        return span * kbytes <= ((int64_t)1 << 30);
    };
    if (!span_ok(s)) {
        int need = s;
        while (!span_ok(need) && need < nst) ++need;
        if (!span_ok(need) || (int64_t)need * per > slab_cap)
            throw std::runtime_error("weight-gradient K-slice exceeds the 1 GB window and the slab");
        s = need;
    }
    a.kstages_per_split = cdiv(nst, s);
    s = cdiv(nst, a.kstages_per_split);
    a.ldc = a.N; a.slab_stride = per;
    a.C = s == 1 ? dw : slab;
    const dim3 grid(a.M / 64, cin / 64, s);
    const char* name = strip ? "void cad::k_conv3x3_wgrad_strip_s3(cad::GemmArgs)" : "void cad::k_conv3x3_wgrad_win_s3(cad::GemmArgs)";
    if (prof_enabled()) prof_push(name, 2.0 * a.M * a.N * (double)a.K, st);
    if (strip) hipLaunchKernelGGL(k_conv3x3_wgrad_strip_s3, grid, dim3(256), 0, st, a);
    else hipLaunchKernelGGL(k_conv3x3_wgrad_win_s3, grid, dim3(256), 0, st, a);
    if (prof_enabled()) prof_pop(st);
    if (s > 1) finish_slabs(slab, s, per, dw, st);
}

template <template <int, int, int> class F, template <int, int, int> class T3, template <int, int, int> class TB>
void launch_wgrad(GemmArgs& a, float* dw, float* slab, int64_t slab_cap, int64_t kbytes, hipStream_t st) {
    const Cfg c = pick_cfg(a.M, a.N);
    const int kb = engine() == 1 ? kS3KB : engine() == 2 ? kB1KB : 16;
    int s = plan_splits(a, c, kb, slab_cap, kbytes);
    a.kstages_per_split = cdiv(cdiv(a.K, kb), s);
    s = cdiv(cdiv(a.K, kb), a.kstages_per_split);
    const int64_t per = (int64_t)a.M * a.N;
    a.ldc = a.N; a.slab_stride = per;
    a.C = s == 1 ? dw : slab;
    launch_on_engine<F, T3, TB>(c, kb, a, s, st);
    if (s > 1) finish_slabs(slab, s, per, dw, st);
}
}

void set_gemm_engine(int e) { g_engine = (e == 1 || e == 2) ? e : 0; }
int gemm_engine() { return engine(); }

int conv3x3_stats_rows(int cin, int B, int H, int W, int cout, bool ps) {
    const WinPick w = ps ? pick_win_ps(cin, W, cout, 0) : pick_win(cin, W, cout);
    if (w.R) return win_blocks(w, B, H, W);
    return cdiv((int64_t)B * H * W, tile_m(pick_cfg(B * H * W, cout)));
}

void conv3x3_fwd(const float* x, int64_t ldx, int xcoff, int cin, const float* w, int cout, float* y,
                 int64_t ldy, int ycoff, int B, int H, int W, float* stats, hipStream_t st) {
    CAD_NO_ALIAS("conv3x3_fwd", {aview(y, (int64_t)B * H * W, ldy, ycoff, cout, 4, "y")},
                 {aview(x, (int64_t)B * H * W, ldx, xcoff, cin, 4, "x"), aview(w, cout, 9 * cin, 0, 9 * cin, 4, "w")});
    GemmArgs a{};
    a.M = B * H * W; a.N = cout; a.K = 9 * cin;
    a.B = B; a.H = H; a.W = W;
    a.A = x; a.lda = ldx; a.a_coff = xcoff; a.a_cin = cin;
    a.Bm = w; a.ldb = 9 * cin; a.b_coff = 0;
    a.C = y; a.ldc = ldy; a.c_coff = ycoff;
    a.stats = stats;
    if (const WinPick w = pick_win(cin, W, cout); w.R) {
        if (stats) launch_win<EpiStoreStats>(w, a, st);
        else launch_win<EpiStore>(w, a, st);
        return;
    }
    const Cfg c = pick_cfg(a.M, a.N);
    if (stats) launch_engine<KConvFwdS, KConvFwdS3, KConvFwdSB>(c, true, a, st);
    else launch_engine<KConvFwd, KConvFwd3, KConvFwdB>(c, true, a, st);
}

void convT_fwd(const float* x, int64_t ldx, int cin, const float* wf, const float* bias, int cout,
               float* y, int64_t ldy, int ycoff, int B, int H, int W, hipStream_t st) {
    CAD_NO_ALIAS("convT_fwd", {aview(y, (int64_t)B * 4 * H * W, ldy, ycoff, cout, 4, "y")},
                 {aview(x, (int64_t)B * H * W, ldx, 0, cin, 4, "x"), aview(wf, 4 * cout, cin, 0, cin, 4, "w")});
    GemmArgs a{};
    a.M = B * H * W; a.N = 4 * cout; a.K = cin;
    a.B = B; a.H = H; a.W = W;
    a.A = x; a.lda = ldx; a.a_coff = 0;
    a.Bm = wf; a.ldb = cin;
    a.C = y; a.ldc = ldy; a.c_coff = ycoff; a.bias = bias;
    launch_engine<KConvTFwd, KConvTFwd3, KConvTFwdB>(pick_cfg(a.M, a.N), false, a, st);
}

void conv3x3_dgrad(const float* dz, int cout, const float* wd, int cin, float* dx, int64_t lddx,
                   int B, int H, int W, hipStream_t st) {
    CAD_NO_ALIAS("conv3x3_dgrad", {aview(dx, (int64_t)B * H * W, lddx, 0, cin, 4, "dx")},
                 {aview(dz, (int64_t)B * H * W, cout, 0, cout, 4, "dz"), aview(wd, cin, 9 * cout, 0, 9 * cout, 4, "w")});
    GemmArgs a{};
    a.M = B * H * W; a.N = cin; a.K = 9 * cout;
    a.B = B; a.H = H; a.W = W;
    a.A = dz; a.lda = cout; a.a_coff = 0; a.a_cin = cout;
    a.Bm = wd; a.ldb = 9 * cout;
    a.C = dx; a.ldc = lddx; a.c_coff = 0;
    if (const WinPick w = pick_win(cout, W, cin); w.R) {
        launch_win<EpiStore>(w, a, st);
        return;
    }
    launch_engine<KConvFwd, KConvFwd3, KConvFwdB>(pick_cfg(a.M, a.N), true, a, st);
}

void convT_dgrad(const float* g, int64_t ldg, int gcoff, int cout, const float* wm, int cin, float* dx,
                 int B, int H, int W, hipStream_t st) {
    CAD_NO_ALIAS("convT_dgrad", {aview(dx, (int64_t)B * H * W, cin, 0, cin, 4, "dx")},
                 {aview(g, (int64_t)B * 4 * H * W, ldg, gcoff, cout, 4, "g"), aview(wm, cin, 4 * cout, 0, 4 * cout, 4, "w")});
    GemmArgs a{};
    a.M = B * H * W; a.N = cin; a.K = 4 * cout;
    a.B = B; a.H = H; a.W = W;
    a.A = g; a.lda = ldg; a.a_coff = gcoff; a.a_cin = cout;
    a.Bm = wm; a.ldb = 4 * cout;
    a.C = dx; a.ldc = cin; a.c_coff = 0;
    launch_engine<KConvTDgrad, KConvTDgrad3, KConvTDgradB>(pick_cfg(a.M, a.N), false, a, st);
}

int64_t wgrad_slab_floats(int M, int N, int Kpix) {
    GemmArgs a{};
    a.M = M; a.N = N; a.K = Kpix;
    return (int64_t)plan_splits(a, pick_cfg(M, N), 16, 0, 0) * M * N;
}

void conv3x3_wgrad(const float* dz, int cout, const float* x, int64_t ldx, int xcoff, int cin, float* dw,
                   int B, int H, int W, float* slab, int64_t slab_cap, hipStream_t st) {
    CAD_NO_ALIAS("conv3x3_wgrad",
                 {aview(dw, cout, 9 * cin, 0, 9 * cin, 4, "dw"), aview(slab, 1, slab_cap, 0, slab ? slab_cap : 0, 4, "slab")},
                 {aview(dz, (int64_t)B * H * W, cout, 0, cout, 4, "dz"), aview(x, (int64_t)B * H * W, ldx, xcoff, cin, 4, "x")});
    GemmArgs a{};
    a.M = cout; a.N = 9 * cin; a.K = B * H * W;
    a.B = B; a.H = H; a.W = W;
    a.A = dz; a.lda = cout; a.a_coff = 0;
    a.Bm = x; a.ldb = ldx; a.b_coff = xcoff; a.b_cin = cin;
    if (use_wgrad_win(cout, cin, W)) {
        launch_wgrad_win(a, dw, slab, slab_cap, 4 * std::max<int64_t>(a.lda, ldx), st);
        return;
    }
    if (wgrad_narrow_s3(dz, cout, x, ldx, xcoff, cin, cout, dw, B, H, W, slab, slab_cap, st)) return;
    launch_wgrad<KConvWgrad, KConvWgrad3, KConvWgradB>(a, dw, slab, slab_cap, 4 * std::max<int64_t>(a.lda, ldx), st);
}

void convT_wgrad(const float* x, int cin, const float* g, int64_t ldg, int gcoff, int cout, float* dw,
                 int B, int H, int W, float* slab, int64_t slab_cap, hipStream_t st) {
    CAD_NO_ALIAS("convT_wgrad",
                 {aview(dw, cin, 4 * cout, 0, 4 * cout, 4, "dw"), aview(slab, 1, slab_cap, 0, slab ? slab_cap : 0, 4, "slab")},
                 {aview(x, (int64_t)B * H * W, cin, 0, cin, 4, "x"), aview(g, (int64_t)B * 4 * H * W, ldg, gcoff, cout, 4, "g")});
    GemmArgs a{};
    a.M = cin; a.N = 4 * cout; a.K = B * H * W;
    a.B = B; a.H = H; a.W = W;
    a.A = x; a.lda = cin; a.a_coff = 0;
    a.Bm = g; a.ldb = ldg; a.b_coff = gcoff; a.b_cin = cout;
    launch_wgrad<KConvTWgrad, KConvTWgrad3, KConvTWgradB>(a, dw, slab, slab_cap, 4 * std::max<int64_t>(a.lda, 4 * ldg),
                                                           st);
}

int split_planes() { return engine() == 2 ? 1 : 0; }

void split_rows(const float* x, int64_t ldx, int xcoff, int C, int64_t M, void* out, int64_t ldo, int ocoff,
                hipStream_t st) {
    if (C % 8 || xcoff % 4 || ldx % 4 || ocoff % 8 || ldo % 8) throw std::runtime_error("split_rows: alignment");
    if (split_planes() != 1) throw std::runtime_error("split_rows needs the bf16 engine");
    CAD_NO_ALIAS("split_rows", {aview(out, M, ldo, ocoff, C, 2, "out")}, {aview(x, M, ldx, xcoff, C, 4, "x")});
    const int G = C / 8;
    const int64_t n = M * G;
    if (n == 0) return;
    hipLaunchKernelGGL(k_split_rows<1>, dim3((unsigned)((n + 255) / 256)), dim3(256), 0, st, x, ldx, xcoff, G, n,
                       (char*)out, ldo, ocoff);
}

namespace {
void ps_check(const Split& s, int channels, const char* what) {
    if (!s.p || s.ld % 8 || s.coff % 8 || channels % 8) throw std::runtime_error(std::string("pre-split operand: ") + what);
    if (engine() != 2) throw std::runtime_error("pre-split GEMM launched off the bf16 engine");
}
}

void conv3x3_fwd_ps(Split x, int cin, Split w, int cout, float* y, int64_t ldy, int ycoff, int B, int H, int W,
                    float* stats, hipStream_t st, bool y_bf16) {
    ps_check(x, cin, "conv3x3_fwd x");
    ps_check(w, 9 * cin, "conv3x3_fwd w");
    CAD_NO_ALIAS("conv3x3_fwd_ps", {aview(y, (int64_t)B * H * W, ldy, ycoff, cout, y_bf16 ? 2 : 4, "y")},
                 {aview(x.p, (int64_t)B * H * W, x.ld, x.coff, cin, 2, "x"), aview(w.p, cout, w.ld, w.coff, 9 * cin, 2, "w")});
    GemmArgs a{};
    a.M = B * H * W; a.N = cout; a.K = 9 * cin;
    a.B = B; a.H = H; a.W = W;
    a.A = (const float*)x.p; a.lda = x.ld; a.a_coff = x.coff; a.a_cin = cin;
    a.Bm = (const float*)w.p; a.ldb = w.ld; a.b_coff = w.coff;
    a.C = y; a.ldc = ldy; a.c_coff = ycoff;
    a.stats = stats;
    if (const WinPick wp = pick_win_ps(cin, W, cout, x.coff); wp.R && w.coff == 0) {
        if (y_bf16) {
            if (stats) launch_win<EpiStoreStatsB16, true>(wp, a, st);
            else launch_win<EpiStoreB16, true>(wp, a, st);
        } else {
            if (stats) launch_win<EpiStoreStats, true>(wp, a, st);
            else launch_win<EpiStore, true>(wp, a, st);
        }
        return;
    }
    const Cfg c = pick_cfg(a.M, a.N);
    const int kb = ps_kb(true, c);
    a.kstages_per_split = cdiv(a.K, kb);
    a.cimajor = cin % kb == 0;
    if (y_bf16) {
        if (stats) launch_kb<KConvFwdSP1B, 32, 64>(c, kb, a, 1, st);
        else launch_kb<KConvFwdP1B, 32, 64>(c, kb, a, 1, st);
    } else {
        if (stats) launch_kb<KConvFwdSP1, 32, 64>(c, kb, a, 1, st);
        else launch_kb<KConvFwdP1, 32, 64>(c, kb, a, 1, st);
    }
}

namespace {
template <bool OB16, bool PS>
int dgrad_bnsums_launch(const WinPick& wp, GemmArgs& a, const BnSums& bn, hipStream_t st) {
    const int tiles = win_blocks(wp, a.B, a.H, a.W);
    if (!bn.part || (int64_t)tiles * 2 * a.N > bn.part_cap) return 0;
    a.bn_g = bn.y; a.bn_ldg = bn.ldy;
    a.bn_mean = bn.mean; a.bn_invstd = bn.invstd; a.bn_scale = bn.scale; a.bn_shift = bn.shift;
    a.bn_part = bn.part;
    if (bn.y_bf16) launch_win<EpiStoreBnSums<OB16, true>, PS>(wp, a, st);
    else launch_win<EpiStoreBnSums<OB16, false>, PS>(wp, a, st);
    return tiles;
}
}

int conv3x3_dgrad_bnsums(const float* dz, int cout, const float* wd, int cin, float* dx, int64_t lddx, int B, int H,
                         int W, const BnSums& bn, hipStream_t st) {
    const WinPick w = pick_win(cout, W, cin);
    if (!w.R || bn.y_bf16) return 0;
    GemmArgs a{};
    a.M = B * H * W; a.N = cin; a.K = 9 * cout;
    a.B = B; a.H = H; a.W = W;
    a.A = dz; a.lda = cout; a.a_coff = 0; a.a_cin = cout;
    a.Bm = wd; a.ldb = 9 * cout;
    a.C = dx; a.ldc = lddx; a.c_coff = 0;
    return dgrad_bnsums_launch<false, false>(w, a, bn, st);
}

bool conv3x3_dgrad_split_ok(Split dz, int cout, Split wd, int cin, int W, int split_n) {
    return split_n > 0 && split_n % 32 == 0 && split_n < cin && pick_win_ps(cout, W, cin, dz.coff).R && wd.coff == 0;
}

bool conv3x3_dgrad_ps(Split dz, int cout, Split wd, int cin, float* dx, int64_t lddx, int B, int H, int W,
                      hipStream_t st, bool dx_bf16, void* hi, int64_t ldhi, int split_n) {
    if (hi && (!conv3x3_dgrad_split_ok(dz, cout, wd, cin, W, split_n) || ldhi < cin - split_n)) {
        if (dx_bf16) throw std::runtime_error("conv3x3_dgrad_ps: bf16 split store not possible for this shape");
        hi = nullptr;
    }
    ps_check(dz, cout, "conv3x3_dgrad dz");
    ps_check(wd, 9 * cout, "conv3x3_dgrad w");
    CAD_NO_ALIAS("conv3x3_dgrad_ps",
                 {aview(dx, (int64_t)B * H * W, lddx, 0, hi ? split_n : cin, dx_bf16 ? 2 : 4, "dx"),
                  aview(hi, (int64_t)B * H * W, ldhi, 0, hi ? cin - split_n : 0, 2, "hi (split store)")},
                 {aview(dz.p, (int64_t)B * H * W, dz.ld, dz.coff, cout, 2, "dz"), aview(wd.p, cin, wd.ld, wd.coff, 9 * cout, 2, "w")});
    GemmArgs a{};
    a.M = B * H * W; a.N = cin; a.K = 9 * cout;
    a.B = B; a.H = H; a.W = W;
    a.A = (const float*)dz.p; a.lda = dz.ld; a.a_coff = dz.coff; a.a_cin = cout;
    a.Bm = (const float*)wd.p; a.ldb = wd.ld; a.b_coff = wd.coff;
    a.C = dx; a.ldc = lddx; a.c_coff = 0;
    if (const WinPick wp = pick_win_ps(cout, W, cin, dz.coff); wp.R && wd.coff == 0) {
        if (hi) {
            a.C2 = hi; a.ldc2 = ldhi; a.split_n = split_n;
            if (dx_bf16) launch_win<EpiStoreSplit2B16, true>(wp, a, st);
            else launch_win<EpiStoreSplitB16, true>(wp, a, st);
            return true;
        }
        if (dx_bf16) launch_win<EpiStoreB16, true>(wp, a, st);
        else launch_win<EpiStore, true>(wp, a, st);
        return false;
    }
    const Cfg c = pick_cfg(a.M, a.N);
    const int kb = ps_kb(true, c);
    a.kstages_per_split = cdiv(a.K, kb);
    a.cimajor = cout % kb == 0;
    if (dx_bf16) launch_kb<KConvFwdP1B, 32, 64>(c, kb, a, 1, st);
    else launch_kb<KConvFwdP1, 32, 64>(c, kb, a, 1, st);
    return false;
}

#ifndef CAD_WGWIN_P
#define CAD_WGWIN_P 32
#endif
#ifdef CAD_NO_WGWIN
constexpr bool g_no_wgwin = true;
#else
constexpr bool g_no_wgwin = false;
#endif
int wgrad_win_ps_stage(int cout, int cin, int W) {
    if (cout % 64 || cin % 64) return 0;
    static const int pref = [] {
        const char* e = std::getenv("CAD_WGP");
        return (e && e[0] == '6') ? 64 : CAD_WGWIN_P;
    }();
    for (int p : {pref, 32, 16})
        if (W % p == 0) return p;
    return 0;
}
bool wg_dma() {
    static const bool on = [] {
        const char* e = std::getenv("CAD_WGDMA");
        return !(e && e[0] == '0');
    }();
    return on;
}
int wg_nbuf() {
    static const int n = [] {
        const char* e = std::getenv("CAD_WGBUF");
        return (e && e[0] == '2') ? 2 : 3;
    }();
    return n;
}
bool wg_strip2() {
    static const bool on = [] {
        const char* e = std::getenv("CAD_WGSTRIP2");
        return !(e && e[0] == '0');
    }();
    return on;
// ... 322 lines not shown
```

camera-aware-neural-networks-for-few-view-depth-estimation_amd/csrc/kernels/gemm_mfma.hpp:

```cpp
#pragma once
#include <hip/hip_runtime.h>
#include <stdint.h>

#include <type_traits>

namespace cad {

typedef float floatx16 __attribute__((ext_vector_type(16)));
typedef float floatx4 __attribute__((ext_vector_type(4)));

template <int KB>
struct KS {
    static_assert(KB == 16 || KB == 32, "K-stage depth");
    static constexpr int BK = KB;
    static constexpr int LDK = KB + 4;
    static constexpr int TPR = KB / 4;
    static constexpr int RPP = 256 / TPR;
    static constexpr int HK = KB / 2;
};

struct GemmArgs {
    int M, N, K;
    int B, H, W;
    const float* A; int64_t lda; int a_coff; int a_cin;
    const float* Bm; int64_t ldb; int b_coff; int b_cin;
    float* C; int64_t ldc; int c_coff;
    const float* bias;
    float* stats;
    int kstages_per_split;
    int64_t slab_stride;
    int cimajor;
    void* C2; int64_t ldc2; int split_n;
    const float *bn_scale, *bn_shift, *bn_mean, *bn_invstd, *bn_coef;
    const void* bn_g; int64_t bn_ldg;
    double* bn_part;
};


constexpr uint32_t kOOB = 0x80000000u;
constexpr uint32_t kRecords = 0x7FFFFFF0u;

__device__ __forceinline__ __amdgpu_buffer_rsrc_t make_rsrc(const float* base, uint32_t records = kRecords) {
    const uint64_t a = reinterpret_cast<uint64_t>(base);
    const uint32_t lo = __builtin_amdgcn_readfirstlane((uint32_t)a);
    const uint32_t hi = __builtin_amdgcn_readfirstlane((uint32_t)(a >> 32));
    void* p = reinterpret_cast<void*>(((uint64_t)hi << 32) | lo);
    return __builtin_amdgcn_make_buffer_rsrc(p, 0, __builtin_amdgcn_readfirstlane(records), 0x00020000);
}
__device__ __forceinline__ float4 bload4(__amdgpu_buffer_rsrc_t r, uint32_t off) {
    return __builtin_bit_cast(float4, __builtin_amdgcn_raw_buffer_load_b128(r, off, 0, 0));
}

template <int ROWS, int KB>
struct KcDense {
    using G = KS<KB>;
    static constexpr int NV = ROWS / G::RPP;
    __amdgpu_buffer_rsrc_t rs;
    uint32_t roff[NV];
    int K, k;
    __device__ void init(const float* P, int64_t ld, int coff, int nrows, int K_, int row0, int tid, int kbeg) {
        K = K_;
        k = kbeg * KB + (tid % G::TPR) * 4;
        rs = make_rsrc(P + (int64_t)row0 * ld + coff);
#pragma unroll
        for (int j = 0; j < NV; ++j) {
            const int rr = tid / G::TPR + G::RPP * j;
            roff[j] = row0 + rr < nrows ? (uint32_t)(rr * ld * 4) : kOOB;
        }
    }
    __device__ void load(float4 (&v)[NV]) {
        const bool kin = k < K;
#pragma unroll
        for (int j = 0; j < NV; ++j) v[j] = bload4(rs, kin ? roff[j] + (uint32_t)k * 4 : kOOB);
        k += KB;
    }
    __device__ void finish(float4 (&)[NV]) {}
};

template <int KB>
__device__ __forceinline__ void tapci_advance(int& tap, int& ci, int cin) {
    ci += KB;
    if (cin >= KB) {
        const bool w = ci >= cin;
        ci -= w ? cin : 0;
        tap += w;
    } else {
        while (ci >= cin) { ci -= cin; ++tap; }
    }
}

template <int ROWS, int KB>
struct KcIm2col3x3 {
    using G = KS<KB>;
    static constexpr int NV = ROWS / G::RPP;
    __amdgpu_buffer_rsrc_t rs;
    int ld4;
    uint32_t poff[NV];
    int y[NV], x[NV];
    bool ok[NV];
    int H, W, cin, tap, ci;
    __device__ void init(const float* P, int64_t ld_, int coff, int cin_, int B, int H_, int W_,
                         int row0, int tid, int kbeg) {
        H = H_; W = W_; cin = cin_; ld4 = (int)ld_ * 4;
        const int pb = max(row0 - W_ - 1, 0);
        rs = make_rsrc(P + (int64_t)pb * ld_ + coff);
        const int k = kbeg * KB + (tid % G::TPR) * 4;
        tap = k / cin;
        ci = k - tap * cin;
        const int M = B * H * W;
#pragma unroll
        for (int j = 0; j < NV; ++j) {
            const int r = row0 + tid / G::TPR + G::RPP * j;
            ok[j] = r < M;
            const int rr = ok[j] ? r : 0;
            x[j] = rr % W;
            y[j] = (rr / W) % H;
            poff[j] = (uint32_t)((rr - pb) * ld4);
        }
// ... 615 lines not shown
```

camera-aware-neural-networks-for-few-view-depth-estimation_amd/csrc/kernels/gemm_win.hpp:

```cpp
#pragma once
#include "gemm_s3.hpp"
#include "gemm_ps.hpp"

namespace cad {

template <int R, int CW, int BN>
struct WinGeo {
    static constexpr int BM = R * CW;
    static constexpr int WC = CW + 2;
    static constexpr int WPIX = R * WC;
    static constexpr int NFA = WPIX * 4;
    static constexpr int NVA = (NFA + 255) / 256;
    static constexpr int NFB = 3 * BN * 4;
    static_assert(NFB % 256 == 0, "BN");
    static constexpr int NVB = NFB / 256;
    static constexpr int PLA = WPIX * 16;
    static constexpr int PLB = BN * 16;
};

template <int R, int CW, int BN>
struct WinA {
    using G = WinGeo<R, CW, BN>;
    __amdgpu_buffer_rsrc_t rs;
    int poff[G::NVA];
    int wr[G::NVA];
    int H, y0, rowbytes, cb, ky;
    __device__ void init(const float* P, int64_t ld, int coff, int H_, int W, int b, int y0_, int x0, int tid,
                         int kbeg) {
        H = H_; y0 = y0_;
        const int ld4 = (int)ld * 4;
        rowbytes = W * ld4;
        const int64_t pbase = ((int64_t)b * H + y0 - 1) * W + x0 - 1;
        const int64_t pb = pbase > 0 ? pbase : 0;
        rs = make_rsrc(P + pb * ld + coff);
#pragma unroll
        for (int j = 0; j < G::NVA; ++j) {
            const int f = tid + 256 * j;
            const int w = f >> 2, q = f & 3;
            const int r = w / G::WC, c = w - r * G::WC;
            const int x = x0 - 1 + c;
            const bool ok = f < G::NFA && (unsigned)x < (unsigned)W;
            wr[j] = ok ? r : -(1 << 28);
            poff[j] = (int)((r * (int64_t)W + c + (pbase - pb)) * ld4) + q * 16;
        }
        cb = kbeg / 3;
        ky = kbeg - 3 * cb;
    }
    __device__ void load(float4 (&v)[G::NVA]) {
        const int add = ky * rowbytes + cb * 64;
#pragma unroll
        for (int j = 0; j < G::NVA; ++j) {
            const int y = y0 - 1 + ky + wr[j];
            v[j] = bload4(rs, (unsigned)y < (unsigned)H ? (uint32_t)(poff[j] + add) : kOOB);
        }
        if (++ky == 3) { ky = 0; ++cb; }
    }
};

template <int R, int CW, int BN>
struct WinB {
    using G = WinGeo<R, CW, BN>;
    static constexpr int JPT = BN * 4 / 256;
    __amdgpu_buffer_rsrc_t rs;
    int base, ldb4, cin4, cb, ky;
    __device__ void init(const float* Wt, int64_t ldb, int cin, int n0, int tid, int kbeg) {
        rs = make_rsrc(Wt + (int64_t)n0 * ldb);
        ldb4 = (int)ldb * 4;
        cin4 = cin * 4;
        base = (tid >> 2) * ldb4 + (tid & 3) * 16;
        cb = kbeg / 3;
        ky = kbeg - 3 * cb;
    }
    __device__ void load(float4 (&v)[G::NVB]) {
        const int add = base + 3 * ky * cin4 + cb * 64;
#pragma unroll
        for (int j = 0; j < G::NVB; ++j) {
            const int t = j / JPT, rstep = (j % JPT) * 64;
            v[j] = bload4(rs, (uint32_t)(add + rstep * ldb4 + t * cin4));
        }
        if (++ky == 3) { ky = 0; ++cb; }
    }
};

#ifndef CAD_XP_WIN
#define CAD_XP_WIN 0
#endif
template <int NB, int CB, bool YB>
struct WinBnSums {
    double s0[NB], s1[NB];
    float sc[NB], sh[NB], mu[NB], is[NB];
    __amdgpu_buffer_rsrc_t ry;
    int64_t ldyb;
    __device__ void init(const GemmArgs& a, int b, int y0, int x0, int ncol0) {
        constexpr int YS = YB ? 2 : 4;
        ldyb = a.bn_ldg * YS;
        ry = make_rsrc(reinterpret_cast<const float*>(static_cast<const char*>(a.bn_g) +
                                                      (((int64_t)b * a.H + y0) * a.W + x0) * ldyb));
#pragma unroll
        for (int j = 0; j < NB; ++j) {
            const int n = min(ncol0 + j * CB, a.N - 1);
            sc[j] = a.bn_scale[n]; sh[j] = a.bn_shift[n]; mu[j] = a.bn_mean[n]; is[j] = a.bn_invstd[n];
// ... 150 lines not shown
                }
            }
        }
    if constexpr (Epi::STATS && (CAD_XP_WIN & 2) == 0) bnp.template finish<WM, WN>(a, lds, tile_lin, n0);
    if constexpr (BNS) bns.template finish<WM, WN>(a, lds, tile_lin, n0);
}

template <int WM, int WN, int MB, int NB, int CW, class Epi>
__device__ __forceinline__ void win_epilogue16(const GemmArgs& a, const floatx4 (&acc)[MB][NB], int tile_lin, int n0,
                                               int b, int y0, int x0, float* lds) {
    const int tid = threadIdx.x;
    const int wave = __builtin_amdgcn_readfirstlane(tid >> 6), lane = tid & 63;
    const int wm = wave / WN, wn = wave % WN;
    BnTilePartials16<NB> bnp;
    if constexpr (Epi::STATS) {
        bnp.init();
#pragma unroll
        for (int j = 0; j < NB; ++j) bnp.shift(j, acc[0][j][0]);
    }
    constexpr bool BNS = is_bnsums<Epi>::value;
    [[maybe_unused]] WinBnSums<BNS ? NB : 1, 16, epi_y_bf16<Epi>()> bns;
    if constexpr (BNS) bns.init(a, b, y0, x0, n0 + wn * 16 * NB + (lane & 15));
    constexpr int ES = Epi::BF16 ? 2 : 4;
    const int64_t ldc4 = a.ldc * ES;
    const __amdgpu_buffer_rsrc_t rs = make_rsrc(reinterpret_cast<const float*>(
        reinterpret_cast<const char*>(a.C) + ((((int64_t)b * a.H + y0) * a.W + x0) * a.ldc + a.c_coff) * ES));
    [[maybe_unused]] __amdgpu_buffer_rsrc_t rs2;
    [[maybe_unused]] int64_t ldc2b = 0;
    if constexpr (Epi::SPLIT) {
        ldc2b = a.ldc2 * 2;
        rs2 = make_rsrc(reinterpret_cast<const float*>(static_cast<const char*>(a.C2) +
                                                       (((int64_t)b * a.H + y0) * a.W + x0) * ldc2b));
    }
#pragma unroll
    for (int i = 0; i < MB; ++i)
#pragma unroll
        for (int j = 0; j < NB; ++j) {
            const int n = n0 + wn * 16 * NB + j * 16 + (lane & 15);
            const int mr = wm * 16 * MB + i * 16 + 4 * (lane >> 4);
            const int r = mr / CW, c = mr - r * CW;
            const bool ok = n < a.N && y0 + r < a.H;
            float v[4];
#pragma unroll
            for (int q = 0; q < 4; ++q) v[q] = acc[i][j][q];
            if constexpr (Epi::BF16) {
#pragma unroll
                for (int q = 0; q < 4; ++q) v[q] = (float)(__bf16)v[q];
            }
            if constexpr (Epi::SPLIT) {
                if (n0 + wn * 16 * NB + j * 16 >= a.split_n) {
                    const uint32_t lo2 =
                        ok ? (uint32_t)((r * (int64_t)a.W + c) * ldc2b + (int64_t)(n - a.split_n) * 2) : kOOB;
#pragma unroll
                    for (int q = 0; q < 4; ++q)
                        __builtin_amdgcn_raw_buffer_store_b16(__builtin_bit_cast(uint16_t, (__bf16)v[q]), rs2,
                                                              lo2 + (uint32_t)(q * ldc2b), 0, 0);
                    continue;
                }
            }
            const uint32_t lo = ok ? (uint32_t)((r * (int64_t)a.W + c) * ldc4 + (int64_t)n * ES) : kOOB;
            if constexpr (BNS) {
                float yv[4];
                bns.load4(r * (int64_t)a.W + c, n, ok, yv);
                if (ok) {
#pragma unroll
                    for (int q = 0; q < 4; ++q) bns.add(j, v[q], yv[q]);
                }
            }
#pragma unroll
            for (int q = 0; q < 4; ++q) {
                if constexpr (Epi::BF16)
                    __builtin_amdgcn_raw_buffer_store_b16(__builtin_bit_cast(uint16_t, (__bf16)v[q]), rs,
                                                          lo + (uint32_t)(q * ldc4), 0, 0);
                else
                    __builtin_amdgcn_raw_buffer_store_b32(__builtin_bit_cast(uint32_t, v[q]), rs,
                                                          lo + (uint32_t)(q * ldc4), 0, 0);
                if constexpr (Epi::STATS) bnp.add(j, v[q], y0 + r < a.H);
            }
        }
    if constexpr (Epi::STATS) bnp.template finish<WM, WN>(a, lds, tile_lin, n0);
    if constexpr (BNS) bns.template finish<WM, WN>(a, lds, tile_lin, n0);
}

template <int NP, int R, int CW, int WM, int WN, class Epi>
__device__ __forceinline__ void conv3x3_win_body(const GemmArgs& a) {
    constexpr int MI = 2, NJ = 2;
    constexpr int BM = 32 * MI * WM, BN = 32 * NJ * WN;
    static_assert(BM == R * CW, "tile");
    using G = WinGeo<R, CW, BN>;
    constexpr int SA = NP * G::PLA, SB = 3 * NP * G::PLB;
    __shared__ __attribute__((aligned(16))) uint16_t lds[SA + SB];

    const int tid = threadIdx.x;
    const int wave = tid >> 6, lane = tid & 63;
    const int wm = wave / WN, wn = wave % WN;
    const TileId tile = xcd_tile();
    const int nbx = a.W / CW, nby = (a.H + R - 1) / R;
    const int tx = tile.x % nbx, t2 = tile.x / nbx, ty = t2 % nby, b = t2 / nby;
    const int y0 = ty * R, x0 = tx * CW, n0 = tile.y * BN;
    const int cin = a.a_cin;
    const int S = 3 * (cin / 16);

    WinA<R, CW, BN> la;
    WinB<R, CW, BN> lb;
    la.init(a.A, a.lda, a.a_coff, a.H, a.W, b, y0, x0, tid, 0);
    lb.init(a.Bm, a.ldb, cin, n0, tid, 0);

    int wpix[MI];
#pragma unroll
    for (int i = 0; i < MI; ++i) {
        const int p = wm * 32 * MI + i * 32 + (lane & 31);
        const int r = p / CW;
        wpix[i] = r * G::WC + (p - r * CW);
    }

    floatx16 acc[MI][NJ];
    acc_zero(acc);
    float4 ra[G::NVA], rb[G::NVB];

    auto store = [&]() {
#pragma unroll
        for (int j = 0; j < G::NVA; ++j) {
            const int f = tid + 256 * j;
            if (f < G::NFA) {
                const auto sp = split_np<NP>(ra[j]);
                const int off = s3_off<16>(f >> 2, (f & 3) * 4);
#pragma unroll
                for (int p = 0; p < NP; ++p) *reinterpret_cast<uint2*>(lds + p * G::PLA + off) = sp.p[p];
            }
        }
#pragma unroll
        for (int j = 0; j < G::NVB; ++j) {
            const int f = tid + 256 * j;
            const int t = f / (BN * 4), rem = f - t * (BN * 4);
            const auto sp = split_np<NP>(rb[j]);
            const int off = SA + t * NP * G::PLB + s3_off<16>(rem >> 2, (rem & 3) * 4);
#pragma unroll
            for (int p = 0; p < NP; ++p) *reinterpret_cast<uint2*>(lds + off + p * G::PLB) = sp.p[p];
        }
    };
    auto compute = [&]() {
#pragma unroll
        for (int kx = 0; kx < 3; ++kx) {
            bf16x8 fa[MI][NP], fb[NJ][NP];
#pragma unroll
            for (int j = 0; j < NJ; ++j) s3_frag<BN, 16, NP>(lds + SA + kx * NP * G::PLB, wn * 32 * NJ + j * 32, 0, fb[j]);
#pragma unroll
            for (int i = 0; i < MI; ++i) {
                const uint16_t* base = lds + s3_off<16>(wpix[i] + kx, (lane >> 5) * 8);
#pragma unroll
                for (int p = 0; p < NP; ++p) fa[i][p] = *reinterpret_cast<const bf16x8*>(base + p * G::PLA);
            }
            s3_mfma<NP>(acc, fa, fb);
        }
    };

    if (S > 0) {
        la.load(ra);
        lb.load(rb);
        store();
    }
    __syncthreads();
    for (int s = 0; s < S; ++s) {
        const bool more = s + 1 < S;
        if (more) {
            la.load(ra);
            lb.load(rb);
        }
        compute();
        __syncthreads();
        if (more) {
            store();
            __syncthreads();
        }
    }
    win_epilogue<WM, WN, MI, NJ, CW, Epi>(a, acc, tile.x, n0, b, y0, x0, reinterpret_cast<float*>(lds));
}

template <int R, int CW, int BN>
struct WinPsGeo {
    static constexpr int WC = CW + 2;
    static constexpr int WPIX = R * WC;
    static constexpr int LDK = S3<32>::LDK;
    static constexpr int NTA = WPIX * 4;
    static constexpr int NVA = (NTA + 255) / 256;
    static constexpr int NTB = BN * 4;
    static constexpr int JB = (NTB + 255) / 256;
    static constexpr int SA = WPIX * LDK, SBT = BN * LDK;
};

#ifndef CAD_WIN16
#define CAD_WIN16 0
#endif
template <int R, int CW, int WM, int WN, class Epi, int MI = 2, int NJ = 2, bool M16 = (CAD_WIN16 != 0)>
__device__ __forceinline__ void conv3x3_win_ps_body(const GemmArgs& a) {
    constexpr int BM = 32 * MI * WM, BN = 32 * NJ * WN;
    static_assert(BM == R * CW, "tile");
    using G = WinPsGeo<R, CW, BN>;
    __shared__ __attribute__((aligned(16))) uint16_t lds[G::SA + 3 * G::SBT];

    const int tid = threadIdx.x;
    const int wave = tid >> 6, lane = tid & 63;
    const int wm = wave / WN, wn = wave % WN;
    const TileId tile = xcd_tile_yfast();
    const int nbx = a.W / CW, nby = (a.H + R - 1) / R;
    const int tx = tile.x % nbx, t2 = tile.x / nbx, ty = t2 % nby, b = t2 / nby;
    const int y0 = ty * R, x0 = tx * CW, n0 = tile.y * BN;
    const int H = a.H, W = a.W, cin = a.a_cin;
    const int S = 3 * (cin / 32);

    const int rowb = (int)a.lda * 2;
    const int64_t pbase = ((int64_t)b * H + y0 - 1) * W + x0 - 1;
    const int64_t pb = pbase > 0 ? pbase : 0;
    const __amdgpu_buffer_rsrc_t rsa =
        make_rsrc(reinterpret_cast<const float*>(reinterpret_cast<const char*>(a.A) + (pb * a.lda + a.a_coff) * 2));
    static_assert(G::NVA <= 10, "amask: 3 bits per piece");
    int aoff[G::NVA];
    uint32_t amask = 0;
#pragma unroll
    for (int j = 0; j < G::NVA; ++j) {
        const int f = tid + 256 * j;
        const int w = f >> 2, g = f & 3;
        const int r = w / G::WC, c = w - r * G::WC;
        const int x = x0 - 1 + c;
        const bool okx = f < G::NTA && (unsigned)x < (unsigned)W;
#pragma unroll
        for (int ky = 0; ky < 3; ++ky)
            if (okx && (unsigned)(y0 - 1 + ky + r) < (unsigned)H) amask |= 1u << (3 * j + ky);
        aoff[j] = (int)((r * (int64_t)W + c + (pbase - pb)) * rowb) + g * 16;
    }
    const int alds0 = (tid >> 2) * G::LDK + (tid & 3) * 8;
    const int rowbb = (int)a.ldb * 2;
    const __amdgpu_buffer_rsrc_t rsb =
        make_rsrc(reinterpret_cast<const float*>(reinterpret_cast<const char*>(a.Bm) + ((int64_t)n0 * a.ldb + a.b_coff) * 2));
    const int boff0 = (tid >> 2) * rowbb + (tid & 3) * 16, blds0 = (tid >> 2) * G::LDK + (tid & 3) * 8;
    auto bact = [&](int jj) { return 256 * (jj + 1) <= G::NTB || tid + 256 * jj < G::NTB; };

    constexpr int MR = M16 ? 2 * MI : MI;
    int wpix[MR];
#pragma unroll
    for (int i = 0; i < MR; ++i) {
        const int p = M16 ? wm * 32 * MI + i * 16 + (lane & 15) : wm * 32 * MI + i * 32 + (lane & 31);
        const int r = p / CW;
        wpix[i] = r * G::WC + (p - r * CW);
    }

    floatx16 acc[M16 ? 1 : MI][M16 ? 1 : NJ];
    floatx4 acc4[M16 ? 2 * MI : 1][M16 ? 2 * NJ : 1];
    if constexpr (M16) {
#pragma unroll
        for (int i = 0; i < 2 * MI; ++i)
#pragma unroll
            for (int j = 0; j < 2 * NJ; ++j) acc4[i][j] = floatx4{0.f, 0.f, 0.f, 0.f};
    } else {
        acc_zero(acc);
    }
// ... 490 lines not shown
        }
        sx0 += P;
        if (sx0 == W) { sx0 = 0; if (++sy == H) { sy = 0; ++sb_; } }
    };
    auto store = [&](int buf) {
        char* da = lds + buf * (PLA + PLB);
#pragma unroll
        for (int j = 0; j < NVA; ++j)
            if (NCA % 256 == 0 || tid + 256 * j < NCA) *reinterpret_cast<uint4*>(da + alds[j]) = ra[j];
#pragma unroll
        for (int j = 0; j < NVB; ++j)
            if (NCB % 256 == 0 || tid + 256 * j < NCB) *reinterpret_cast<uint4*>(da + PLA + blds[j]) = rb[j];
    };
    auto compute = [&](int buf) {
        const char* sa = lds + buf * (PLA + PLB);
        const char* sb = sa + PLA;
#pragma unroll
        for (int q = 0; q < P / 16; ++q) {
            bf16x8 fa[1];
            mnc_frag_at<kWgRows, 1>(sa, PLA, cbk * 32, 16 * q, fa);
#pragma unroll
            for (int t = 0; t < 9; ++t) {
                bf16x8 fb[1];
                mnc_frag_at<kWgRows, 1>(sb, PLB, cib * 32, (t / 3) * (P + 2) + (t % 3) + 16 * q, fb);
                acc[t] = __builtin_amdgcn_mfma_f32_32x32x16_bf16(fa[0], fb[0], acc[t], 0, 0, 0);
            }
        }
    };

    if (kbeg < kend) {
        load();
        store(0);
    }
    __syncthreads();
    int cur = 0;
    for (int kt = kbeg; kt < kend; ++kt) {
        const bool more = kt + 1 < kend;
        if (more) load();
        compute(cur);
        if (more) store(cur ^ 1);
        __syncthreads();
        cur ^= 1;
    }
    const int lane = tid & 63;
    const int cin = a.b_cin;
    float* dst = a.C + (int64_t)tile.z * a.slab_stride;
#pragma unroll
    for (int t = 0; t < 9; ++t)
#pragma unroll
        for (int g = 0; g < 4; ++g) {
            const int n = t * cin + ci0 + cib * 32 + (lane & 31);
            const int co = co0 + cbk * 32 + 4 * (lane >> 5) + 8 * g;
#pragma unroll
            for (int q = 0; q < 4; ++q) dst[(int64_t)(co + q) * a.ldc + n] = acc[t][4 * g + q];
        }
}


__device__ __forceinline__ int wgd_off(int kr, int byte) {
    return kr * 128 + ((((byte >> 4) ^ (((kr >> 1) & 1) << 2))) << 4) + (byte & 15);
}
__device__ __forceinline__ void wgd_frag(const char* s, int rb, int krow0, bf16x8& f) {
    const int lane = threadIdx.x & 63;
    const int g = (lane >> 4) & 1, h = lane >> 5, i = lane & 15;
    const int krow = krow0 + 8 * h + (i >> 2);
    const int byte = 2 * (rb + 16 * g + 4 * (i & 3));
    typedef __attribute__((address_space(3))) v4i16 lds_v4;
    const v4i16 lo = __builtin_amdgcn_ds_read_tr16_b64_v4i16((lds_v4*)(s + wgd_off(krow, byte)));
    const v4i16 hi = __builtin_amdgcn_ds_read_tr16_b64_v4i16((lds_v4*)(s + wgd_off(krow + 4, byte)));
    const uint2 ul = __builtin_bit_cast(uint2, lo), uh = __builtin_bit_cast(uint2, hi);
    f = __builtin_bit_cast(bf16x8, make_uint4(ul.x, ul.y, uh.x, uh.y));
}
template <int P, int NBUF_ = 3>
struct WgdGeo {
    static constexpr int KW = 3 * (P + 2);
    static constexpr int NIA = P / 8;
    static constexpr int NIB = (KW + 7) / 8;
    static constexpr int NI = NIA + NIB;
    static constexpr int SLOTS = (NI + 3) / 4;
    static constexpr int WAIT = NI / 4;
    static constexpr int SA = P * 128, SB = NIB * 8 * 128, STAGE = SA + SB;
    static constexpr int NBUF = NBUF_;
};

typedef int i32x4_t __attribute__((ext_vector_type(4)));
struct DmaRsrc {
    i32x4_t d;
};
__device__ __forceinline__ DmaRsrc dma_rsrc(const void* base) {
    const uint64_t a = reinterpret_cast<uint64_t>(base);
    DmaRsrc r;
    r.d[0] = __builtin_amdgcn_readfirstlane((int)(uint32_t)a);
    r.d[1] = __builtin_amdgcn_readfirstlane((int)((uint32_t)(a >> 32) & 0xFFFF));
    r.d[2] = (int)kRecords;
    r.d[3] = 0x00020000;
    return r;
}
__device__ __forceinline__ void dma16(const DmaRsrc& r, const void* lds_dst, uint32_t voff) {
    const uint32_t m0 = __builtin_amdgcn_readfirstlane(
        (uint32_t)reinterpret_cast<uintptr_t>((const __attribute__((address_space(3))) void*)lds_dst));
    asm volatile("s_mov_b32 m0, %2\n\tbuffer_load_dwordx4 %0, %1, 0 offen lds" ::"v"(voff), "s"(r.d), "s"(m0)
                 : "memory", "m0");
}

template <int WAITN>
__device__ __forceinline__ void wgd_wait_barrier() {
    if constexpr (WAITN == 0) asm volatile("s_waitcnt vmcnt(0)\n\ts_waitcnt lgkmcnt(0)\n\ts_barrier" ::: "memory");
    else asm volatile("s_waitcnt vmcnt(%0)\n\ts_waitcnt lgkmcnt(0)\n\ts_barrier" ::"n"(WAITN) : "memory");
}

template <int P, int NBUF = 3>
__device__ __forceinline__ void conv3x3_wgrad_win_dma_body(const GemmArgs& a) {
    static_assert(P % 16 == 0 && (NBUF == 2 || NBUF == 3), "stage / ring");
    using G = WgdGeo<P, NBUF>;
    __shared__ __attribute__((aligned(1024))) char lds[G::NBUF * G::STAGE];

    const int tid = threadIdx.x;
    const int wave = __builtin_amdgcn_readfirstlane(tid >> 6), lane = tid & 63;
    const int cbk = wave & 1, cib = wave >> 1;
    const TileId tile = xcd_tile();
    const int co0 = tile.x * 64, ci0 = tile.y * 64;
    const int H = a.H, W = a.W;
    const int nst = a.K / P;
    const int kbeg = tile.z * a.kstages_per_split;
    const int kend = min(nst, kbeg + a.kstages_per_split);
    const int segs = W / P;

    const int64_t p0 = (int64_t)kbeg * P;
    const int64_t pb = p0 - W - 1 > 0 ? p0 - W - 1 : 0;
    const int rowA = (int)a.lda * 2, rowB = (int)a.ldb * 2;
    const DmaRsrc rsa = dma_rsrc(ps_at(a.A, (p0 * a.lda + a.a_coff + co0) * 2));
    const DmaRsrc rsb = dma_rsrc(ps_at(a.Bm, (pb * a.ldb + a.b_coff + ci0) * 2));

    const int lrow = lane >> 3, lch = lane & 7;
    int sj[G::SLOTS];
    int soff[G::SLOTS];
    int sky[G::SLOTS], skk[G::SLOTS];
#pragma unroll
    for (int t = 0; t < G::SLOTS; ++t) {
        const int j = wave + 4 * t;
        sj[t] = j < G::NI ? j : -1;
        if (j < G::NIA) {
            const int kr = 8 * j + lrow;
            const int gch = lch ^ (((kr >> 1) & 1) << 2);
            soff[t] = kr * rowA + gch * 16;
            sky[t] = 0; skk[t] = 0;
        } else {
            const int kr = 8 * (j - G::NIA) + lrow;
            const int gch = lch ^ (((kr >> 1) & 1) << 2);
            const bool in = kr < G::KW;
            sky[t] = in ? kr / (P + 2) : -(1 << 28);
            skk[t] = in ? kr - (kr / (P + 2)) * (P + 2) : 0;
            soff[t] = in ? ((sky[t] - 1) * W + skk[t] - 1) * rowB + gch * 16 : 0;
        }
    }
    auto issue = [&](int stage, int buf) {
        const int row = stage / segs;
        const int sx0 = (stage - row * segs) * P, sy = row % H, sb = row / H;
        const int64_t pix = ((int64_t)sb * H + sy) * W + sx0;
        const uint32_t da = (uint32_t)((pix - p0) * rowA), db = (uint32_t)((pix - pb) * rowB);
        char* base = lds + buf * G::STAGE;
#pragma unroll
        for (int t = 0; t < G::SLOTS; ++t) {
            const int j = sj[t];
            if (j < 0) continue;
            if (j < G::NIA) {
                dma16(rsa, base + j * 1024, da + (uint32_t)soff[t]);
            } else {
                const int yy = sy + sky[t] - 1, xx = sx0 + skk[t] - 1;
                const bool ok = (unsigned)yy < (unsigned)H && (unsigned)xx < (unsigned)W;
                dma16(rsb, base + G::SA + (j - G::NIA) * 1024, ok ? db + (uint32_t)soff[t] : kOOB);
            }
        }
    };

    floatx16 acc[9];
#pragma unroll
    for (int t = 0; t < 9; ++t)
#pragma unroll
        for (int r = 0; r < 16; ++r) acc[t][r] = 0.f;

    auto compute = [&](int buf) {
        const char* sa = lds + buf * G::STAGE;
        const char* sb = sa + G::SA;
#pragma unroll
        for (int q = 0; q < P / 16; ++q) {
            bf16x8 fa;
            wgd_frag(sa, cbk * 32, 16 * q, fa);
#pragma unroll
            for (int t = 0; t < 9; ++t) {
                bf16x8 fb;
                wgd_frag(sb, cib * 32, (t / 3) * (P + 2) + (t % 3) + 16 * q, fb);
// ... 391 lines not shown
```

camera-aware-neural-networks-for-few-view-depth-estimation_amd/csrc/kernels/kernels.hpp:

```cpp
#pragma once
#include <hip/hip_runtime.h>
#include <stdint.h>

#include <initializer_list>

namespace cad {

bool prof_enabled();
void prof_push(const char* name, double flops, hipStream_t st);
void prof_pop(hipStream_t st);

struct AliasView {
    const void* p = nullptr;
    int64_t rows = 0, ld = 0, coff = 0, cols = 0;
    int es = 4;
    const char* what = "";
};
inline AliasView aview(const void* p, int64_t rows, int64_t ld, int64_t coff, int64_t cols, int es, const char* what) {
    AliasView v;
    v.p = p; v.rows = rows; v.ld = ld; v.coff = coff; v.cols = cols; v.es = es; v.what = what;
    return v;
}
int alias_mode();
bool views_overlap(const AliasView& a, const AliasView& b);
void alias_check_impl(const char* op, std::initializer_list<AliasView> outs, std::initializer_list<AliasView> ins,
                      bool same_view_ok = false);
#define CAD_NO_ALIAS(...)                                                     \
    do {                                                                      \
        if (::cad::alias_mode()) ::cad::alias_check_impl(__VA_ARGS__);        \
    } while (0)

void set_gemm_engine(int e);
int gemm_engine();
void conv3x3_fwd(const float* x, int64_t ldx, int xcoff, int cin, const float* w, int cout, float* y,
                 int64_t ldy, int ycoff, int B, int H, int W, float* stats, hipStream_t st);
int conv3x3_stats_rows(int cin, int B, int H, int W, int cout, bool ps = false);
void conv3x3_dgrad(const float* dz, int cout, const float* wd, int cin, float* dx, int64_t lddx,
                   int B, int H, int W, hipStream_t st);
void conv3x3_wgrad(const float* dz, int cout, const float* x, int64_t ldx, int xcoff, int cin, float* dw,
                   int B, int H, int W, float* slab, int64_t slab_cap, hipStream_t st);
void convT_fwd(const float* x, int64_t ldx, int cin, const float* wf, const float* bias, int cout,
               float* y, int64_t ldy, int ycoff, int B, int H, int W, hipStream_t st);
void convT_dgrad(const float* g, int64_t ldg, int gcoff, int cout, const float* wm, int cin, float* dx,
                 int B, int H, int W, hipStream_t st);
void convT_wgrad(const float* x, int cin, const float* g, int64_t ldg, int gcoff, int cout, float* dw,
                 int B, int H, int W, float* slab, int64_t slab_cap, hipStream_t st);
int64_t wgrad_slab_floats(int M, int N, int Kpix);

struct Split {
    const void* p = nullptr;
    int64_t ld = 0;
    int coff = 0;
};
int split_planes();
constexpr int kMaxPlanes = 1;
void split_rows(const float* x, int64_t ldx, int xcoff, int C, int64_t M, void* out, int64_t ldo, int ocoff,
                hipStream_t st);
void conv3x3_fwd_ps(Split x, int cin, Split w, int cout, float* y, int64_t ldy, int ycoff, int B, int H, int W,
                    float* stats, hipStream_t st, bool y_bf16 = false);
bool conv3x3_dgrad_ps(Split dz, int cout, Split wd, int cin, float* dx, int64_t lddx, int B, int H, int W,
                      hipStream_t st, bool dx_bf16 = false, void* hi = nullptr, int64_t ldhi = 0, int split_n = 0);
bool conv3x3_dgrad_split_ok(Split dz, int cout, Split wd, int cin, int W, int split_n);
void conv3x3_wgrad_ps(Split dz, int cout, Split x, int cin, float* dw, int B, int H, int W, float* slab,
                      int64_t slab_cap, hipStream_t st);
void convT_fwd_ps(Split x, int cin, Split wf, const float* bias, int cout, float* y, int64_t ldy, int ycoff, int B,
                  int H, int W, hipStream_t st, bool y_bf16 = false);
void convT_dgrad_ps(Split g, int cout, Split wm, int cin, float* dx, int B, int H, int W, hipStream_t st,
                    bool dx_bf16 = false);
void convT_wgrad_ps(Split x, int cin, Split g, int cout, float* dw, int B, int H, int W, float* slab,
                    int64_t slab_cap, hipStream_t st);

void dense_fwd_ps(Split x, int K, Split w, int N, float* y, int64_t ldy, int ycoff, int64_t M, float* stats,
                  hipStream_t st, bool y_bf16 = false, const float* add = nullptr, const float* mask = nullptr,
                  int64_t ldadd = 0);
void mask_inplace(float* y, int64_t ldy, int ycoff, const float* mask, int C, int64_t M, hipStream_t st);
int dense_stats_rows(int64_t M, int N);
void dense_wgrad_ps(Split dz, int N, Split x, int K, float* dw, int64_t ldw, int64_t M, float* slab, int64_t slab_cap,
                    hipStream_t st);

struct Mx8 {
    const void* q = nullptr;
    const void* s = nullptr;
    int64_t ld = 0;
    int coff = 0;
};
void mx8_quantize(const void* src, bool src_bf16, int64_t lds, int scoff, int C, int64_t M, Mx8 dst, hipStream_t st);
struct Mx8WJob {
    const float* src;
    uint8_t* q;
    uint8_t* s;
    int64_t ldq;
    int rows, C;
    int blk0;
};
constexpr int kMx8WMaxJobs = 56;
struct Mx8WList {
    Mx8WJob job[kMx8WMaxJobs];
    int njobs = 0;
};
void mx8_quantize_weights(Mx8WList& list, hipStream_t st);
bool dense_x8_ok(int K, int N);
void dense_fwd_x8(Mx8 x, int K, Mx8 w, int N, float* y, int64_t ldy, int ycoff, int64_t M, float* stats, hipStream_t st,
                  bool y_bf16 = false);
int dense_x8_stats_rows(int64_t M, int N);
bool conv3x3_x8_ok(int cin, int W, int N);
void conv3x3_fwd_x8(Mx8 x, int cin, Mx8 w, int cout, float* y, int64_t ldy, int ycoff, int B, int H, int W,
                    float* stats, hipStream_t st, bool y_bf16 = false);
int conv3x3_x8_stats_rows(int cin, int B, int H, int W, int cout);

void im2col_f32(const float* x, int64_t ldx, int xcoff, int C, int B, int H, int W, int KH, int KW, int S, int P,
                void* col, int Kp, hipStream_t st);
void im2col_ps(Split x, int C, int B, int H, int W, int KH, int KW, int S, int P, void* col, int Kp, hipStream_t st);
void col2im(const float* dcol, int Kc, int C, int B, int H, int W, int KH, int KW, int S, int P, float* dx,
            int64_t lddx, hipStream_t st);
void maxpool3s2_fwd(const float* x, int C, int B, int H, int W, float* out, uint8_t* idx, void* out_split,
                    hipStream_t st);
void maxpool3s2_bwd(const float* dout, const uint8_t* idx, int C, int B, int H, int W, float* dx, hipStream_t st,
                    const float* add = nullptr, int64_t ldadd = 0);
void bn_add_relu(const float* y, const float* scale, const float* shift, const float* yd, const float* dscale,
                 const float* dshift, const float* x, int64_t ldx, int C, int64_t M, float* out, void* out_split,
                 hipStream_t st, bool y_bf16 = false, const Mx8* qx = nullptr);
void relu_mask(const float* g, int64_t ldg, int gcoff, const float* out, int C, int64_t M, float* gs, hipStream_t st);
void add_strided(float* dst, int64_t lddst, const float* src, int64_t ldsrc, int scoff, int C, int B, int H, int W,
                 int S, hipStream_t st);
void copy_twin(Split src, int C, int B, int H, int W, int S, void* dst, int64_t ldd, int dcoff, hipStream_t st);
void transpose_split(const float* w, int64_t ldw, int N, int K, void* wt, hipStream_t st);

int colsum_slices(int64_t R);
void colsum(const float* x, int64_t ld, int coff, int64_t R, int C, double* part, hipStream_t st);
void colsum_bf16(const void* x, int64_t ld, int coff, int64_t R, int C, double* part, hipStream_t st);
void colsum_finalize(const double* part, int S, int C, float* dst, float scale, hipStream_t st);
void bn_fwd_finalize(const float* tile_part, int rows, int C, int64_t count, const float* gamma,
                     const float* beta, float* run_mean, float* run_var, float momentum, float eps,
                     double* scratch, float* mean, float* invstd, float* scale, float* shift,
                     hipStream_t st);
void bn_eval_coeffs(const float* gamma, const float* beta, const float* run_mean, const float* run_var,
                    int C, float eps, float* mean, float* invstd, float* scale, float* shift, hipStream_t st);
void bn_relu_fwd(const float* y, int C, const float* scale, const float* shift, float* out, int64_t ldo,
                 int ocoff, int64_t M, hipStream_t st, void* os = nullptr, int64_t ldos = 0, int oscoff = 0,
                 bool y_bf16 = false, const Mx8* qx = nullptr);
struct HeadGrad {
    const float* dpred = nullptr;
    const float* sig = nullptr;
    const float* w = nullptr;
    float md = 0.f;
};
struct FastDiv {
    uint32_t m = 0;
    int s1 = 0, s2 = 0;
};
inline FastDiv make_fastdiv(uint32_t d) {
    int l = 0;
    while ((1ull << l) < d) ++l;
    FastDiv f;
    f.m = (uint32_t)((((1ull << 32) * ((1ull << l) - d)) / d) + 1);
    f.s1 = l > 0 ? 1 : 0;
    f.s2 = l > 0 ? l - 1 : 0;
    return f;
}
__device__ __forceinline__ uint32_t fdiv(const FastDiv& f, uint32_t n) {
    const uint32_t t = __umulhi(f.m, n);
    return (t + ((n - t) >> f.s1)) >> f.s2;
}
struct PoolAdd {
    const float* d = nullptr;
    const uint8_t* idx = nullptr;
    int H = 0, W = 0;
    FastDiv divW, divH;
};
void bn_relu_bwd(const float* g, int64_t ldg, int gcoff, const float* y, int C, const float* mean,
                 const float* invstd, const float* scale, const float* shift, const float* gamma,
                 int64_t M, double* scratch, float* coef, float* dgamma, float* dbeta, float* dy,
                 hipStream_t st, const float* gmul = nullptr, int64_t HW = 1, void* dy_split = nullptr,
                 bool relu = true, bool y_bf16 = false, const HeadGrad* head = nullptr, bool g_bf16 = false,
                 const PoolAdd* pool = nullptr, float* film_dgam = nullptr, float* film_dbet = nullptr,
                 const double* tile_part = nullptr, int tiles = 0);
void maxpool_fwd(const float* x, int64_t ldx, int C, int B, int H, int W, float* out, uint8_t* idx,
                 hipStream_t st, void* out_split = nullptr, bool x_bf16 = false);
struct BnSums {
    const void* y = nullptr; int64_t ldy = 0; bool y_bf16 = false;
    const float *mean = nullptr, *invstd = nullptr, *scale = nullptr, *shift = nullptr;
    double* part = nullptr; int64_t part_cap = 0;
};
int conv3x3_dgrad_bnsums(const float* dz, int cout, const float* wd, int cin, float* dx, int64_t lddx, int B, int H,
                         int W, const BnSums& bn, hipStream_t st);
void bn_relu_pool_fwd(const float* y, int C, const float* scale, const float* shift, float* out, int64_t ldo,
                      void* os, int64_t ldos, int B, int H, int W, bool y_bf16, float* pool, uint8_t* idx,
                      void* pool_split, hipStream_t st);
void maxpool_bwd(const float* dout, const uint8_t* idx, int C, int B, int H, int W, float* dx,
                 int64_t lddx, hipStream_t st);
void rgb_to_nhwc4(const float* rgb, float* out, int B, int H, int W, hipStream_t st);
void rgb_to_nhwc8(const float* rgb, float* out, int B, int H, int W, hipStream_t st);
void head_fwd(const float* a, int C, const float* w, const float* b, float max_depth, float* sig,
              float* pred, int64_t M, hipStream_t st);
void head_bwd(const float* a, int C, const float* w, const float* dpred, const float* sig,
              float max_depth, float* da, int64_t M, double* scratch, float* dw, float* db,
              hipStream_t st);
bool head_fusable(int C);
void bn_relu_head_fwd(const float* y, int C, const float* scale, const float* shift, const float* w, const float* b,
                      float max_depth, float* sig, float* pred, int64_t M, hipStream_t st, bool y_bf16);
void head_bwd_y(const float* y, int C, const float* scale, const float* shift, const float* dpred, const float* sig,
                float max_depth, int64_t M, double* scratch, float* dw, float* db, hipStream_t st, bool y_bf16);
int metrics_blocks(int64_t HW);
void depth_metrics_partials(const float* pred, const float* gt, int B, int64_t HW, double* part, int nb,
                            hipStream_t st);
constexpr int kHistBins = 1548;
constexpr int kHistStats = 6;
constexpr int kHistChunk = 16384;
struct HistSegment {
    int64_t offset, count, period, keep;
    int64_t inner_period, inner_keep;
    int first_chunk, nchunks;
};
struct HistChunk {
    int64_t start;
    int seg, len;
};
void hist_run(const float* base, const HistSegment* segs, int nseg, const HistChunk* chunks, int nchunks, const unsigned* ukey,
              unsigned key_hi, double* stats, unsigned* bins, double* part, int64_t span, hipStream_t st);
int eval_blocks(int64_t HW);
void eval_update(const float* pred, const float* gt, const uint8_t* mask, int B, int64_t HW, float min_depth,
                 float max_depth, int clamp_pred, double* part, int nb, double* table, int64_t base, hipStream_t st,
                 const float* align = nullptr);
struct EvalStrata {
    int n_depth_cuts, n_angle_cuts;
    float depth_cuts[15];
    float angle_cuts[15];
};
void eval_update_strata(const float* pred, const float* gt, const uint8_t* mask, const float* K, int B, int64_t HW, int W,
                        float min_depth, float max_depth, int clamp_pred, double* part, int nb, double* table, int64_t base,
                        hipStream_t st, const float* align, const EvalStrata& sp, double* spart, double* stable);
struct EvalAlignWs {
    double* part;
    double* stats;
    unsigned* hist;
    unsigned* sel;
    float* med;
};
size_t eval_align_ws_bytes(int max_batch, int nb);
EvalAlignWs eval_align_ws_carve(void* base, int max_batch, int nb);
void eval_valid_medians(const float* pred, const float* gt, const uint8_t* mask, int B, int64_t HW, float min_depth,
                        float max_depth, const EvalAlignWs& ws, int nb, float* med, hipStream_t st);
void eval_align(int mode, const float* pred, const float* gt, const uint8_t* mask, int B, int64_t HW, float min_depth,
                float max_depth, const EvalAlignWs& ws, int nb, float* table, uint8_t* flags, int64_t base, hipStream_t st);
void repack_conv_dgrad(const float* w, float* wd, int cout, int cin, hipStream_t st);
void repack_convT_fwd(const float* wm, float* wf, int cin, int cout, hipStream_t st);
enum { WPREP_SPLIT = 0, WPREP_DGRAD = 1, WPREP_CONVT = 2, WPREP_TRANSPOSE = 3 };
struct WPrepJob {
    const float* src;
    float* d32;
    void* d16;
    int kind, cout, cin;
    int blk0;
    int64_t n;
};
constexpr int kWPrepMaxJobs = 24;
struct WPrepList {
    WPrepJob job[kWPrepMaxJobs];
    int njobs;
};
void weight_prep(WPrepList& list, hipStream_t st);

struct LossWorkspace {
    double* part;
    float* scal;
    float* pyr;
    int64_t part_cap;
};
int64_t loss_workspace_floats(int B, int H, int W);
int64_t loss_part_doubles(int B, int H, int W);
void loss_fwd_bwd(const float* pred, const float* gt, const float* rgb, const float* K, const uint8_t* mask, int B,
                  int H, int W, const float w[4], float* out5, float* dpred, LossWorkspace ws, hipStream_t st);

int sumsq_blocks(int64_t n);
void grad_norm_clip(const float* g, int64_t n, float max_norm, float prescale, double* scratch,
                    float* norm_coef, hipStream_t st);
void adam_step(float* p, float* g, float* m, float* v, int64_t n, const float* norm_coef, float lr,
               float b1, float b2, float eps, float wd, int step, hipStream_t st);
enum { kOptimAdam = 0, kOptimAdamW = 1, kOptimSGD = 2 };
void optim_step(int rule, float* p, float* g, float* m, float* v, float* ema, int64_t n, const float* norm_coef,
                float lr, float b1, float b2, float eps, float wd, float mu, float ema_d, int step, hipStream_t st);
void slab_swap(float* a, float* b, int64_t n, hipStream_t st);

struct BatchSample {
    const uint8_t* rgb;
    const uint16_t* depth;
    int h0, w0, bgr;
    int dh0, dw0;
    float depth_scale;
    int aug;
    int cy, cx, ch, cw;
    int flip, jitter;
    float contrast, brightness;
    int color;
    float m[9];
    int gamma_on;
    float gamma;
};
void batch_assemble(const BatchSample* samples_dev, int B, int H, int W, bool any_aug, bool any_color, float* rgb,
                    float* depth, float* rgb_tmp, float* depth_tmp, hipStream_t st);

void ray_directions(const float* K, int B, int H, int W, float* rays_nchw, hipStream_t st);
void camera_from_K(const float* K, int B, float* cam4, hipStream_t st);
void camera_normalize(const float* cam4, int B, int H, int W, float* camn, hipStream_t st);
void rgb_rays_to_nhwc8(const float* rgb, const float* cam4, int B, int H, int W, float* out, hipStream_t st);

constexpr int kFilmH1 = 128, kFilmH2 = 256;
struct FilmLayer {
    int C = 0;
    const float *w1, *b1, *w2, *b2, *wg, *bg, *wb, *bb, *g1, *be1, *g2, *be2;
    float *rm1, *rv1, *rm2, *rv2;
    float *xh1, *h1, *xh2, *h2, *is1, *is2;
    float *gam, *bet;
    float *dgam, *dbet, *dh2, *dh1;
    float *gw1, *gb1, *gw2, *gb2, *gwg, *gbg, *gwb, *gbb, *gg1, *gbe1, *gg2, *gbe2;
};
void film_mlp_fwd(const FilmLayer& L, const float* camn, int B, bool train, hipStream_t st);
constexpr int kFilmMaxLayers = 10;
struct FilmList {
    FilmLayer l[kFilmMaxLayers];
    int n = 0;
};
void film_mlp_fwd_all(const FilmList& list, const float* camn, int B, bool train, hipStream_t st);
void film_mlp_bwd(const FilmLayer& L, const float* camn, int B, hipStream_t st);
void film_apply(const float* y, int C, const float* scale, const float* shift, const float* gam, const float* bet,
                int B, int64_t HW, float* out, hipStream_t st, bool y_bf16 = false, void* os = nullptr);
void film_affine_bwd(const float* dA, const float* y, int C, const float* scale, const float* shift, int B, int64_t HW,
                     double* scratch, float* dgam, float* dbet, hipStream_t st, bool y_bf16 = false,
                     bool dA_bf16 = false);
int64_t film_reduce_doubles(int B, int64_t HW, int C);

void pack_rgb_rays(const float* rgb, const float* rays, int B, int H, int W, float* out, hipStream_t st);
int chan_pool_slices(int64_t HW);
void chan_pool(const float* x, int64_t ldx, int xcoff, int C, int B, int64_t HW, double* part, float* avg, float* mx,
               int* amax, hipStream_t st);
int64_t attn_scratch_doubles(int B, int64_t HW, int C);

struct Cbam {
    int C = 0, Cr = 0;
// ... 64 lines not shown
```

camera-aware-neural-networks-for-few-view-depth-estimation_amd/csrc/kernels/nn_kernels.hip:

```cpp
#include <algorithm>
#include <stdexcept>
#include <type_traits>
#include <utility>

#include "gemm_s3.hpp"
#include "ew_load.hpp"
#include "kernels.hpp"
#include "mx8_quant.hpp"

namespace cad {
__device__ __forceinline__ float bn_relu1(float y, float s, float t) { return fmaxf(__fmaf_rn(y, s, t), 0.f); }
__device__ __forceinline__ float head_dot4(float4 a, float4 w) {
    return __fmaf_rn(a.w, w.w, __fmaf_rn(a.z, w.z, __fmaf_rn(a.y, w.y, __fmul_rn(a.x, w.x))));
}
namespace {
inline int cdiv(int64_t a, int64_t b) { return (int)((a + b - 1) / b); }
inline int ew_blocks(int64_t n) { return (int)std::min<int64_t>(std::max<int64_t>(1, cdiv(n, 256)), 8192); }
}

template <class Op, class = void>
struct has_prep_slice : std::false_type {};
template <class Op>
struct has_prep_slice<Op, std::void_t<decltype(std::declval<const Op&>().prep_slice(0, int64_t{0}, int64_t{0}))>>
    : std::true_type {};
// ... 1041 lines not shown
        constexpr bool YB = decltype(yb)::value;
        switch (C / 4) {
            case 1: go(k_bn_relu_head_fwd_rows<YB, 1>); break;
            case 2: go(k_bn_relu_head_fwd_rows<YB, 2>); break;
            case 4: go(k_bn_relu_head_fwd_rows<YB, 4>); break;
            case 8: go(k_bn_relu_head_fwd_rows<YB, 8>); break;
            case 16: go(k_bn_relu_head_fwd_rows<YB, 16>); break;
            default: go(k_bn_relu_head_fwd_rows<YB, 32>); break;
        }
    };
    y_bf16 ? pick(std::true_type{}) : pick(std::false_type{});
}
void head_bwd_y(const float* y, int C, const float* scale, const float* shift, const float* dpred, const float* sig,
                float max_depth, int64_t M, double* scratch, float* dw, float* db, hipStream_t st, bool y_bf16) {
    double* part = scratch + 2 * C;
    const int S = y_bf16 ? launch_colreduce<2>(OpHeadBwdY<true>{y, scale, shift, dpred, sig, max_depth, C}, M, C, part, st)
                         : launch_colreduce<2>(OpHeadBwdY<false>{y, scale, shift, dpred, sig, max_depth, C}, M, C, part, st);
    launch_colfinal(part, S, 2 * C, scratch, nullptr, 1.f, st);
    hipLaunchKernelGGL(k_colfinal, dim3(cdiv(C, 64)), dim3(64, kFinalLanes), 0, st, scratch, 1, C, nullptr, dw, 1.f);
    hipLaunchKernelGGL(k_colfinal, dim3(1), dim3(64, kFinalLanes), 0, st, scratch + C, 1, 1, nullptr, db, 1.f);
}

__global__ __launch_bounds__(256) void k_metrics(const float* __restrict__ pred, const float* __restrict__ gt,
                                                 int64_t HW, double* part, int nb) {
    const int b = blockIdx.y;
    double v[8] = {0, 0, 0, 0, 0, 0, 0, 0};
    for (int64_t i = (int64_t)blockIdx.x * 256 + threadIdx.x; i < HW; i += (int64_t)nb * 256) {
        const float p = pred[b * HW + i], g = gt[b * HW + i];
        if (!(g > 0.f)) continue;
        const float ad = fabsf(p - g);
        const float ld = fabsf(logf(p + 1e-8f) - logf(g + 1e-8f));
        const float r = fmaxf(p / g, g / p);
        v[0] += 1.0; v[1] += ad / g; v[2] += (ad * ad) / g; v[3] += ad * ad; v[4] += ld * ld;
        v[5] += r < 1.25f; v[6] += r < 1.5625f; v[7] += r < 1.953125f;
    }
    __shared__ double red[4][8];
    for (int q = 0; q < 8; ++q) {
        double x = v[q];
        for (int o = 32; o > 0; o >>= 1) x += __shfl_xor(x, o);
        if ((threadIdx.x & 63) == 0) red[threadIdx.x >> 6][q] = x;
    }
    __syncthreads();
    if (threadIdx.x < 8)
        part[((int64_t)b * nb + blockIdx.x) * 8 + threadIdx.x] =
            red[0][threadIdx.x] + red[1][threadIdx.x] + red[2][threadIdx.x] + red[3][threadIdx.x];
}
int metrics_blocks(int64_t HW) { return std::max(1, std::min(64, cdiv(HW, 256))); }
void depth_metrics_partials(const float* pred, const float* gt, int B, int64_t HW, double* part, int nb,
                            hipStream_t st) {
    hipLaunchKernelGGL(k_metrics, dim3(nb, B), dim3(256), 0, st, pred, gt, HW, part, nb);
}

__global__ void k_repack_conv_dgrad(const float* __restrict__ w, float* __restrict__ wd, int cout, int cin) {
    const int64_t n = (int64_t)cout * 9 * cin;
    for (int64_t i = (int64_t)blockIdx.x * blockDim.x + threadIdx.x; i < n; i += (int64_t)gridDim.x * blockDim.x) {
        const int co = (int)(i % cout);
        const int64_t t2 = i / cout;
        const int t = (int)(t2 % 9);
        const int ci = (int)(t2 / 9);
        wd[i] = w[((int64_t)co * 9 + (8 - t)) * cin + ci];
    }
}
void repack_conv_dgrad(const float* w, float* wd, int cout, int cin, hipStream_t st) {
    hipLaunchKernelGGL(k_repack_conv_dgrad, dim3(ew_blocks((int64_t)cout * 9 * cin)), dim3(256), 0, st, w, wd, cout, cin);
}
__global__ void k_repack_convT_fwd(const float* __restrict__ wm, float* __restrict__ wf, int cin, int cout) {
    const int64_t n = (int64_t)4 * cout * cin;
    for (int64_t i = (int64_t)blockIdx.x * blockDim.x + threadIdx.x; i < n; i += (int64_t)gridDim.x * blockDim.x) {
        const int ci = (int)(i % cin);
        const int64_t qc = i / cin;
        wf[i] = wm[(int64_t)ci * 4 * cout + qc];
    }
}
void repack_convT_fwd(const float* wm, float* wf, int cin, int cout, hipStream_t st) {
    hipLaunchKernelGGL(k_repack_convT_fwd, dim3(ew_blocks((int64_t)4 * cout * cin)), dim3(256), 0, st, wm, wf, cin, cout);
}

__global__ __launch_bounds__(256) void k_weight_prep(WPrepList list) {
    int j = 0;
    while (j + 1 < list.njobs && (int)blockIdx.x >= list.job[j + 1].blk0) ++j;
    const WPrepJob& jb = list.job[j];
    const int64_t i = ((int64_t)(blockIdx.x - jb.blk0) * 256 + threadIdx.x) * 8;
    if (i >= jb.n) return;
    const int ne = (int)min<int64_t>(8, jb.n - i);
    float v[8];
#pragma unroll
    for (int e = 0; e < 8; ++e) {
        const int64_t k = i + (e < ne ? e : 0);
        int64_t src;
        if (jb.kind == WPREP_SPLIT) {
            src = k;
        } else if (jb.kind == WPREP_DGRAD) {
            const int co = (int)(k % jb.cout);
            const int64_t t2 = k / jb.cout;
            const int t = (int)(t2 % 9), ci = (int)(t2 / 9);
            src = ((int64_t)co * 9 + (8 - t)) * jb.cin + ci;
        } else if (jb.kind == WPREP_CONVT) {
            const int ci = (int)(k % jb.cin);
            src = (int64_t)ci * 4 * jb.cout + k / jb.cin;
        } else {
            const int co = (int)(k % jb.cout);
            src = (int64_t)co * jb.cin + k / jb.cout;
        }
        v[e] = jb.src[src];
    }
    if (jb.d32) {
        if (ne == 8) {
            *reinterpret_cast<float4*>(jb.d32 + i) = make_float4(v[0], v[1], v[2], v[3]);
            *reinterpret_cast<float4*>(jb.d32 + i + 4) = make_float4(v[4], v[5], v[6], v[7]);
        } else {
            for (int e = 0; e < ne; ++e) jb.d32[i + e] = v[e];
        }
    }
    if (jb.d16) {
        const auto sa = split_np<1>(make_float4(v[0], v[1], v[2], v[3]));
        const auto sb = split_np<1>(make_float4(v[4], v[5], v[6], v[7]));
        *reinterpret_cast<uint4*>(static_cast<char*>(jb.d16) + i * 2) = make_uint4(sa.p[0].x, sa.p[0].y, sb.p[0].x, sb.p[0].y);
    }
}
void weight_prep(WPrepList& list, hipStream_t st) {
    if (list.njobs <= 0) return;
    if (list.njobs > kWPrepMaxJobs) throw std::runtime_error("weight_prep: too many jobs");
    int blocks = 0;
    for (int j = 0; j < list.njobs; ++j) {
        WPrepJob& jb = list.job[j];
        if (jb.d16 && jb.n % 8) throw std::runtime_error("weight_prep: bf16 twin size not a multiple of 8");
        jb.blk0 = blocks;
        blocks += (int)cdiv(cdiv(jb.n, 8), (int64_t)256);
    }
    hipLaunchKernelGGL(k_weight_prep, dim3(blocks), dim3(256), 0, st, list);
}

}
```

Before: 144.1 images/s.

## Pre-split conv3x3 weights into tile-ordered bf16x3 twins loaded by LDS DMA

Adds a weight-prep job that splits each 3x3 conv weight (forward and dgrad orientation) into three bf16 planes. The planes are laid out in the window kernel's per-stage LDS tile order. The s3 window kernel gets a template variant that streams these twins straight into LDS with buffer_load...lds DMA, which removes per-iteration fp32-to-bf16 splitting and reordering of weights inside the hot GEMM loop. The cost is extra weight-prep work each step and 6 bytes per weight element of extra memory. The new path is on by default via an env flag and applies only when the presplit activation path is off.

After: 148.5 images/s (median of 6 runs). 1.03x the previous value.

```diff
diff --git a/camera-aware-neural-networks-for-few-view-depth-estimation_amd/csrc/host/cad_api.cpp b/camera-aware-neural-networks-for-few-view-depth-estimation_amd/csrc/host/cad_api.cpp
--- a/camera-aware-neural-networks-for-few-view-depth-estimation_amd/csrc/host/cad_api.cpp
+++ b/camera-aware-neural-networks-for-few-view-depth-estimation_amd/csrc/host/cad_api.cpp
@@ -101,6 +101,8 @@
     int pidx = -1, cin = 0, cout = 0;
     float* wd = nullptr;
     void *ws = nullptr, *wds = nullptr;
+    void *wt = nullptr, *wtd = nullptr;
+    int wt_bn = 0, wtd_bn = 0;
 };
 struct Film {
     int p0 = -1;
@@ -355,6 +357,12 @@
         c.ws = sp(n);
         if (dgrad) c.wds = sp(n);
     };
+    auto conv_wtwin_alloc = [&](Conv& c, int l, bool dgrad) {
+        c.wt_bn = cad::conv3x3_wtwin_bn(c.cin, h->Wl(l), c.cout);
+        if (c.wt_bn) c.wt = a.take((size_t)cad::conv3x3_wtwin_bytes(c.cin, c.cout));
+        c.wtd_bn = dgrad ? cad::conv3x3_wtwin_bn(c.cout, h->Wl(l), c.cin) : 0;
+        if (c.wtd_bn) c.wtd = a.take((size_t)cad::conv3x3_wtwin_bytes(c.cout, c.cin));
+    };
     h->flat_p = a.f(h->n_flat);
     h->flat_g = a.f(h->n_flat);
     h->norm_coef = a.f(4);
@@ -371,6 +379,8 @@
         e.c2.wd = a.f((int64_t)e.c2.cout * 9 * e.c2.cin);
         conv_split_alloc(e.c1, l > 0);
         conv_split_alloc(e.c2, true);
+        conv_wtwin_alloc(e.c1, l, l > 0);
+        conv_wtwin_alloc(e.c2, l, true);
         if (l < 4) { h->cat[l] = a.f(2 * MC); h->cats[l] = sp(2 * MC); }
         if (l > 0) {
             h->pool[l] = a.f(h->Ml(l, B) * h->Cl(l - 1));
@@ -394,6 +404,8 @@
         d.c2.wd = a.f((int64_t)d.c2.cout * 9 * d.c2.cin);
         conv_split_alloc(d.c1, true);
         conv_split_alloc(d.c2, true);
+        conv_wtwin_alloc(d.c1, l, true);
+        conv_wtwin_alloc(d.c2, l, true);
         h->up[l].wf = a.f((int64_t)4 * h->up[l].cout * h->up[l].cin);
         h->up[l].wfs = sp((int64_t)4 * h->up[l].cout * h->up[l].cin);
         h->up[l].wms = sp((int64_t)4 * h->up[l].cout * h->up[l].cin);
@@ -525,6 +537,10 @@
     cad::WPrepJob& j = L.job[L.njobs++];
     j.src = src; j.d32 = d32; j.d16 = d16; j.kind = kind; j.cout = cout; j.cin = cin; j.n = n;
 }
+void wprep_twin_add(cad::WPrepList& L, int kind, const float* src, void* twin, int cout, int cin, int bn) {
+    wprep_add(L, kind, src, nullptr, twin, cout, cin, (int64_t)cout * 9 * cin);
+    L.job[L.njobs - 1].bn = bn;
+}
 void prep_fwd_weights(const cad_unet* h, bool ps, hipStream_t st) {
     cad::WPrepList L{};
     for (int l = 0; l < 4; ++l) {
@@ -537,9 +553,17 @@
         };
         for (int l = 0; l < 5; ++l) { sw(h->enc[l].c1); sw(h->enc[l].c2); }
         for (int l = 0; l < 4; ++l) { sw(h->dec[l].c1); sw(h->dec[l].c2); }
+    } else if (cad::conv3x3_wtwin_on()) {
+        auto tw = [&](const Conv& c) {
+            if (c.wt) wprep_twin_add(L, cad::WPREP_WTWIN_FWD, h->P(c.pidx), c.wt, c.cout, c.cin, c.wt_bn);
+        };
+        for (int l = 0; l < 5; ++l) { tw(h->enc[l].c1); tw(h->enc[l].c2); }
+        for (int l = 0; l < 4; ++l) { tw(h->dec[l].c1); tw(h->dec[l].c2); }
     }
     cad::weight_prep(L, st);
 }
+const void* fwd_wtwin(const Conv& c) { return cad::conv3x3_wtwin_on() ? c.wt : nullptr; }
+const void* dgrad_wtwin(const Conv& c) { return cad::conv3x3_wtwin_on() ? c.wtd : nullptr; }
 
 int env_flag(const char* name, int dflt) {
     const char* e = std::getenv(name);
@@ -582,7 +606,8 @@
     if (ps1) {
         cad::conv3x3_fwd_ps(in_s, dc.c1.cin, sv(dc.c1.ws, 9 * dc.c1.cin), C, dc.y1, C, 0, B, Hh, Ww, stats, st, dc.y1b);
     } else {
-        cad::conv3x3_fwd(in, ldin, 0, dc.c1.cin, h->P(dc.c1.pidx), C, dc.y1, C, 0, B, Hh, Ww, stats, st);
+        cad::conv3x3_fwd(in, ldin, 0, dc.c1.cin, h->P(dc.c1.pidx), C, dc.y1, C, 0, B, Hh, Ww, stats, st,
+                         ps ? nullptr : fwd_wtwin(dc.c1));
     }
     bn(dc.b1, dc.c1.cin, ps1);
     if (dc.has_film()) {
@@ -595,7 +620,7 @@
     if (ps)
         cad::conv3x3_fwd_ps(sv(dc.a1s, C), C, sv(dc.c2.ws, 9 * C), C, dc.y2, C, 0, B, Hh, Ww, stats, st, true);
     else
-        cad::conv3x3_fwd(dc.a1, C, 0, C, h->P(dc.c2.pidx), C, dc.y2, C, 0, B, Hh, Ww, stats, st);
+        cad::conv3x3_fwd(dc.a1, C, 0, C, h->P(dc.c2.pidx), C, dc.y2, C, 0, B, Hh, Ww, stats, st, fwd_wtwin(dc.c2));
     bn(dc.b2, C, ps);
     if (head_pred && att_head) {
         cad::cbam_head_fwd(cbam_view(h, 0), cbam_head_view(h), B, Hh, Ww, head_pred, h->dscr, st);
@@ -765,8 +790,9 @@
     } else {
         cad::conv3x3_wgrad(dY, C, dc.a1, C, 0, C, h->G(dc.c2.pidx), B, Hh, Ww, h->slab, h->slab_cap, wg);
         HIPCHK(hipEventRecord(h->evA, wg));
-        if (bs.part) bn1_tiles = cad::conv3x3_dgrad_bnsums(dY, C, dc.c2.wd, C, dA1, C, B, Hh, Ww, bs, st);
-        if (!bn1_tiles) cad::conv3x3_dgrad(dY, C, dc.c2.wd, C, dA1, C, B, Hh, Ww, st);
+        const void* tw = dgrad_wtwin(dc.c2);
+        if (bs.part) bn1_tiles = cad::conv3x3_dgrad_bnsums(dY, C, dc.c2.wd, C, dA1, C, B, Hh, Ww, bs, st, tw);
+        if (!bn1_tiles) cad::conv3x3_dgrad(dY, C, dc.c2.wd, C, dA1, C, B, Hh, Ww, st, tw);
     }
     const int64_t HW = (int64_t)Hh * Ww;
     static const bool film_fuse = env_flag("CAD_FILMFUSE", 1) != 0;
@@ -801,15 +827,17 @@
                                                     Ww, st, din_bf16, din_hi, dc.c1.cin / 2, dc.c1.cin / 2);
             if (din_hi_done) *din_hi_done = done && din_hi;
         } else
-            cad::conv3x3_dgrad(dY1, C, dc.c1.wd, dc.c1.cin, din, lddin, B, Hh, Ww, st);
+            cad::conv3x3_dgrad(dY1, C, dc.c1.wd, dc.c1.cin, din, lddin, B, Hh, Ww, st, ps ? nullptr : dgrad_wtwin(dc.c1));
     }
 }
 
 void repack_dgrad_weights(cad_unet* h, hipStream_t st) {
     const bool ps = h->fwd_np > 0 && h->fwd_np == cad::split_planes();
     cad::WPrepList L{};
+    const bool twins = !ps && cad::conv3x3_wtwin_on();
     auto rp = [&](Conv& c) {
         wprep_add(L, cad::WPREP_DGRAD, h->P(c.pidx), c.wd, ps ? c.wds : nullptr, c.cout, c.cin, (int64_t)c.cout * 9 * c.cin);
+        if (twins && c.wtd) wprep_twin_add(L, cad::WPREP_WTWIN_DGRAD, h->P(c.pidx), c.wtd, c.cout, c.cin, c.wtd_bn);
     };
     for (int l = 0; l < 5; ++l) {
         if (l > 0) rp(h->enc[l].c1);
@@ -2471,7 +2499,16 @@
     return guard([&] {
         require(cin % 4 == 0 && cout % 4 == 0 && ldx % 4 == 0 && ldy % 4 == 0 && xcoff % 4 == 0 && ycoff % 4 == 0,
                 "channels / strides must be multiples of 4");
-        cad::conv3x3_fwd(x, ldx, xcoff, cin, w, cout, y, ldy, ycoff, B, H, W, nullptr, S(stream));
+        void* twin = nullptr;
+        const int bn = cad::conv3x3_wtwin_on() ? cad::conv3x3_wtwin_bn(cin, W, cout) : 0;
+        if (bn) {
+            HIPCHK(hipMallocAsync(&twin, (size_t)cad::conv3x3_wtwin_bytes(cin, cout), S(stream)));
+            cad::WPrepList L{};
+            wprep_twin_add(L, cad::WPREP_WTWIN_FWD, w, twin, cout, cin, bn);
+            cad::weight_prep(L, S(stream));
+        }
+        cad::conv3x3_fwd(x, ldx, xcoff, cin, w, cout, y, ldy, ycoff, B, H, W, nullptr, S(stream), twin);
+        if (twin) HIPCHK(hipFreeAsync(twin, S(stream)));
         HIPCHK(hipGetLastError());
     });
 }
@@ -2482,7 +2519,16 @@
         float* wd = nullptr;
         HIPCHK(hipMallocAsync((void**)&wd, sizeof(float) * (size_t)cout * 9 * cin, S(stream)));
         cad::repack_conv_dgrad(w, wd, cout, cin, S(stream));
-        cad::conv3x3_dgrad(dz, cout, wd, cin, dx, lddx, B, H, W, S(stream));
+        void* twin = nullptr;
+        const int bn = cad::conv3x3_wtwin_on() ? cad::conv3x3_wtwin_bn(cout, W, cin) : 0;
+        if (bn) {
+            HIPCHK(hipMallocAsync(&twin, (size_t)cad::conv3x3_wtwin_bytes(cout, cin), S(stream)));
+            cad::WPrepList L{};
+            wprep_twin_add(L, cad::WPREP_WTWIN_DGRAD, w, twin, cout, cin, bn);
+            cad::weight_prep(L, S(stream));
+        }
+        cad::conv3x3_dgrad(dz, cout, wd, cin, dx, lddx, B, H, W, S(stream), twin);
+        if (twin) HIPCHK(hipFreeAsync(twin, S(stream)));
         HIPCHK(hipFreeAsync(wd, S(stream)));
         HIPCHK(hipGetLastError());
     });
diff --git a/camera-aware-neural-networks-for-few-view-depth-estimation_amd/csrc/kernels/conv_kernels.hip b/camera-aware-neural-networks-for-few-view-depth-estimation_amd/csrc/kernels/conv_kernels.hip
--- a/camera-aware-neural-networks-for-few-view-depth-estimation_amd/csrc/kernels/conv_kernels.hip
+++ b/camera-aware-neural-networks-for-few-view-depth-estimation_amd/csrc/kernels/conv_kernels.hip
@@ -115,9 +115,9 @@
 template <int WM, int WN, int KB>
 __global__ __launch_bounds__(256) void k_convT_wgrad_s3(GemmArgs a) { convT_wgrad_np<3, WM, WN, 2, 2, KB>(a); }
 
-template <int R, int CW, class Epi>
+template <int R, int CW, class Epi, bool WT = false>
 __global__ __launch_bounds__(256, 3) void k_conv3x3_win_s3(GemmArgs a) {
-    conv3x3_win_body<3, R, CW, R * CW == 128 ? 2 : 4, R * CW == 128 ? 2 : 1, Epi>(a);
+    conv3x3_win_body<3, R, CW, R * CW == 128 ? 2 : 4, R * CW == 128 ? 2 : 1, Epi, WT>(a);
 }
 
 template <int R, int CW, class Epi>
@@ -400,9 +400,9 @@
     bool n96 = false;
     int bn() const { return n96 ? 96 : big ? (R * CW == 256 ? 128 : 64) : R * CW == 128 ? 128 : 64; }
 };
-WinPick pick_win(int cin, int W, int N) {
+WinPick pick_win_shape(int cin, int W, int N) {
     WinPick w;
-    if (engine() != 1 || cin % 16) return w;
+    if (cin % 16) return w;
     const int BM = N <= 64 ? 256 : 128;
     if (N % (BM == 128 ? 128 : 64)) return w;
     static const int c128[] = {64, 32, 16, 8}, c256[] = {128, 64};
@@ -416,6 +416,7 @@
         }
     return w;
 }
+WinPick pick_win(int cin, int W, int N) { return engine() == 1 ? pick_win_shape(cin, W, N) : WinPick{}; }
 int win_blocks(const WinPick& w, int B, int H, int W) { return B * cdiv(H, w.R) * (W / w.CW); }
 template <bool PS, int R, int CW, class Epi, bool BIG = false, bool N96 = false>
 void launch_win1(const GemmArgs& a, hipStream_t st) {
@@ -425,13 +426,14 @@
     void (*fn)(GemmArgs);
     if constexpr (N96) fn = k_conv3x3_win_bf16p3<R, CW, Epi>;
     else if constexpr (BIG) fn = k_conv3x3_win_bf16p4<R, CW, Epi, BN == 64>;
-    else fn = PS ? (void (*)(GemmArgs))k_conv3x3_win_bf16p<R, CW, Epi> : (void (*)(GemmArgs))k_conv3x3_win_s3<R, CW, Epi>;
+    else if constexpr (PS) fn = k_conv3x3_win_bf16p<R, CW, Epi>;
+    else fn = a.wtwin ? (void (*)(GemmArgs))k_conv3x3_win_s3<R, CW, Epi, true> : (void (*)(GemmArgs))k_conv3x3_win_s3<R, CW, Epi>;
     if (prof_enabled()) {
         char name[160];
-        snprintf(name, sizeof(name), "void cad::k_conv3x3_win_%s<%d, %d, cad::%s%s>(cad::GemmArgs)",
+        snprintf(name, sizeof(name), "void cad::k_conv3x3_win_%s<%d, %d, cad::%s%s%s>(cad::GemmArgs)",
                  N96 ? "bf16p3" : BIG ? "bf16p4" : PS ? "bf16p" : "s3", R, CW,
                  Epi::STATS ? "EpiStoreStats" : is_bnsums<Epi>::value ? "EpiStoreBnSums" : "EpiStore",
-                 Epi::BF16 ? "B16" : "");
+                 Epi::BF16 ? "B16" : "", !PS && !N96 && !BIG && a.wtwin ? ", true" : "");
         prof_push(name, 2.0 * a.M * a.N * (double)a.K, st);
         hipLaunchKernelGGL(fn, grid, dim3(256), 0, st, a);
         prof_pop(st);
@@ -764,10 +766,22 @@
     return cdiv((int64_t)B * H * W, tile_m(pick_cfg(B * H * W, cout)));
 }
 
+int conv3x3_wtwin_bn(int cin, int W, int N) {
+    const WinPick w = pick_win_shape(cin, W, N);
+    return w.R ? w.bn() : 0;
+}
+int64_t conv3x3_wtwin_bytes(int cin, int N) { return (int64_t)N * 9 * cin * 6; }
+bool conv3x3_wtwin_on() {
+    const char* e = std::getenv("CAD_S3_WTWIN");
+    const bool on = e && e[0] ? std::atoi(e) != 0 : kWtwinDefault;
+    return on && engine() == 1;
+}
+
 void conv3x3_fwd(const float* x, int64_t ldx, int xcoff, int cin, const float* w, int cout, float* y,
-                 int64_t ldy, int ycoff, int B, int H, int W, float* stats, hipStream_t st) {
+                 int64_t ldy, int ycoff, int B, int H, int W, float* stats, hipStream_t st, const void* wtwin) {
     CAD_NO_ALIAS("conv3x3_fwd", {aview(y, (int64_t)B * H * W, ldy, ycoff, cout, 4, "y")},
-                 {aview(x, (int64_t)B * H * W, ldx, xcoff, cin, 4, "x"), aview(w, cout, 9 * cin, 0, 9 * cin, 4, "w")});
+                 {aview(x, (int64_t)B * H * W, ldx, xcoff, cin, 4, "x"), aview(w, cout, 9 * cin, 0, 9 * cin, 4, "w"),
+                  aview(wtwin, 1, conv3x3_wtwin_bytes(cin, cout), 0, wtwin ? conv3x3_wtwin_bytes(cin, cout) : 0, 1, "wtwin")});
     GemmArgs a{};
     a.M = B * H * W; a.N = cout; a.K = 9 * cin;
     a.B = B; a.H = H; a.W = W;
@@ -776,6 +790,7 @@
     a.C = y; a.ldc = ldy; a.c_coff = ycoff;
     a.stats = stats;
     if (const WinPick w = pick_win(cin, W, cout); w.R) {
+        a.wtwin = wtwin;
         if (stats) launch_win<EpiStoreStats>(w, a, st);
         else launch_win<EpiStore>(w, a, st);
         return;
@@ -799,9 +814,10 @@
 }
 
 void conv3x3_dgrad(const float* dz, int cout, const float* wd, int cin, float* dx, int64_t lddx,
-                   int B, int H, int W, hipStream_t st) {
+                   int B, int H, int W, hipStream_t st, const void* wtwin) {
     CAD_NO_ALIAS("conv3x3_dgrad", {aview(dx, (int64_t)B * H * W, lddx, 0, cin, 4, "dx")},
-                 {aview(dz, (int64_t)B * H * W, cout, 0, cout, 4, "dz"), aview(wd, cin, 9 * cout, 0, 9 * cout, 4, "w")});
+                 {aview(dz, (int64_t)B * H * W, cout, 0, cout, 4, "dz"), aview(wd, cin, 9 * cout, 0, 9 * cout, 4, "w"),
+                  aview(wtwin, 1, conv3x3_wtwin_bytes(cout, cin), 0, wtwin ? conv3x3_wtwin_bytes(cout, cin) : 0, 1, "wtwin")});
     GemmArgs a{};
     a.M = B * H * W; a.N = cin; a.K = 9 * cout;
     a.B = B; a.H = H; a.W = W;
@@ -809,6 +825,7 @@
     a.Bm = wd; a.ldb = 9 * cout;
     a.C = dx; a.ldc = lddx; a.c_coff = 0;
     if (const WinPick w = pick_win(cout, W, cin); w.R) {
+        a.wtwin = wtwin;
         launch_win<EpiStore>(w, a, st);
         return;
     }
@@ -938,7 +955,7 @@
 }
 
 int conv3x3_dgrad_bnsums(const float* dz, int cout, const float* wd, int cin, float* dx, int64_t lddx, int B, int H,
-                         int W, const BnSums& bn, hipStream_t st) {
+                         int W, const BnSums& bn, hipStream_t st, const void* wtwin) {
     const WinPick w = pick_win(cout, W, cin);
     if (!w.R || bn.y_bf16) return 0;
     GemmArgs a{};
@@ -947,6 +964,7 @@
     a.A = dz; a.lda = cout; a.a_coff = 0; a.a_cin = cout;
     a.Bm = wd; a.ldb = 9 * cout;
     a.C = dx; a.ldc = lddx; a.c_coff = 0;
+    a.wtwin = wtwin;
     return dgrad_bnsums_launch<false, false>(w, a, bn, st);
 }
 
diff --git a/camera-aware-neural-networks-for-few-view-depth-estimation_amd/csrc/kernels/gemm_mfma.hpp b/camera-aware-neural-networks-for-few-view-depth-estimation_amd/csrc/kernels/gemm_mfma.hpp
--- a/camera-aware-neural-networks-for-few-view-depth-estimation_amd/csrc/kernels/gemm_mfma.hpp
+++ b/camera-aware-neural-networks-for-few-view-depth-estimation_amd/csrc/kernels/gemm_mfma.hpp
@@ -34,6 +34,7 @@
     const float *bn_scale, *bn_shift, *bn_mean, *bn_invstd, *bn_coef;
     const void* bn_g; int64_t bn_ldg;
     double* bn_part;
+    const void* wtwin;
 };
 
 
diff --git a/camera-aware-neural-networks-for-few-view-depth-estimation_amd/csrc/kernels/gemm_win.hpp b/camera-aware-neural-networks-for-few-view-depth-estimation_amd/csrc/kernels/gemm_win.hpp
--- a/camera-aware-neural-networks-for-few-view-depth-estimation_amd/csrc/kernels/gemm_win.hpp
+++ b/camera-aware-neural-networks-for-few-view-depth-estimation_amd/csrc/kernels/gemm_win.hpp
@@ -17,6 +17,32 @@
     static constexpr int PLA = WPIX * 16;
     static constexpr int PLB = BN * 16;
 };
+
+typedef int i32x4_t __attribute__((ext_vector_type(4)));
+struct DmaRsrc {
+    i32x4_t d;
+};
+__device__ __forceinline__ DmaRsrc dma_rsrc(const void* base) {
+    const uint64_t a = reinterpret_cast<uint64_t>(base);
+    DmaRsrc r;
+    r.d[0] = __builtin_amdgcn_readfirstlane((int)(uint32_t)a);
+    r.d[1] = __builtin_amdgcn_readfirstlane((int)((uint32_t)(a >> 32) & 0xFFFF));
+    r.d[2] = (int)kRecords;
+    r.d[3] = 0x00020000;
+    return r;
+}
+__device__ __forceinline__ void dma16(const DmaRsrc& r, const void* lds_dst, uint32_t voff) {
+    const uint32_t m0 = __builtin_amdgcn_readfirstlane(
+        (uint32_t)reinterpret_cast<uintptr_t>((const __attribute__((address_space(3))) void*)lds_dst));
+    asm volatile("s_mov_b32 m0, %2\n\tbuffer_load_dwordx4 %0, %1, 0 offen lds" ::"v"(voff), "s"(r.d), "s"(m0)
+                 : "memory", "m0");
+}
+
+template <int WAITN>
+__device__ __forceinline__ void wgd_wait_barrier() {
+    if constexpr (WAITN == 0) asm volatile("s_waitcnt vmcnt(0)\n\ts_waitcnt lgkmcnt(0)\n\ts_barrier" ::: "memory");
+    else asm volatile("s_waitcnt vmcnt(%0)\n\ts_waitcnt lgkmcnt(0)\n\ts_barrier" ::"n"(WAITN) : "memory");
+}
 
 template <int R, int CW, int BN>
 struct WinA {
@@ -333,13 +359,29 @@
     if constexpr (BNS) bns.template finish<WM, WN>(a, lds, tile_lin, n0);
 }
 
-template <int NP, int R, int CW, int WM, int WN, class Epi>
+template <int BN>
+struct WinTwinGeo {
+    static constexpr int STAGE = 9 * BN * 32;
+    static constexpr int NI = STAGE / 1024;
+    static constexpr int SLOTS = (NI + 3) / 4;
+};
+__device__ __forceinline__ void dma16_m0(const DmaRsrc& r, const void* lds_dst, uint32_t voff) {
+    const uint32_t m0 = __builtin_amdgcn_readfirstlane(
+        (uint32_t)reinterpret_cast<uintptr_t>((const __attribute__((address_space(3))) void*)lds_dst));
+    asm volatile("s_mov_b32 m0, %2\n\ts_nop 0\n\tbuffer_load_dwordx4 %0, %1, 0 offen lds" ::"v"(voff), "s"(r.d), "s"(m0)
+                 : "memory", "m0");
+}
+
+template <int NP, int R, int CW, int WM, int WN, class Epi, bool WT = false>
 __device__ __forceinline__ void conv3x3_win_body(const GemmArgs& a) {
     constexpr int MI = 2, NJ = 2;
     constexpr int BM = 32 * MI * WM, BN = 32 * NJ * WN;
     static_assert(BM == R * CW, "tile");
+    static_assert(!WT || NP == 3, "weight twin: S3 only");
     using G = WinGeo<R, CW, BN>;
+    using T = WinTwinGeo<BN>;
     constexpr int SA = NP * G::PLA, SB = 3 * NP * G::PLB;
+    static_assert(!WT || (SB * 2 == T::STAGE && (SA * 2) % 16 == 0), "twin stage = the B image");
     __shared__ __attribute__((aligned(16))) uint16_t lds[SA + SB];
 
     const int tid = threadIdx.x;
@@ -352,10 +394,13 @@
     const int cin = a.a_cin;
     const int S = 3 * (cin / 16);
 
+    [[maybe_unused]] DmaRsrc rsw;
+    [[maybe_unused]] const int wv = __builtin_amdgcn_readfirstlane(wave);
+    if constexpr (WT) rsw = dma_rsrc(static_cast<const char*>(a.wtwin) + (int64_t)tile.y * S * T::STAGE);
     WinA<R, CW, BN> la;
-    WinB<R, CW, BN> lb;
+    [[maybe_unused]] WinB<R, CW, BN> lb;
     la.init(a.A, a.lda, a.a_coff, a.H, a.W, b, y0, x0, tid, 0);
-    lb.init(a.Bm, a.ldb, cin, n0, tid, 0);
+    if constexpr (!WT) lb.init(a.Bm, a.ldb, cin, n0, tid, 0);
 
     int wpix[MI];
 #pragma unroll
@@ -367,8 +412,18 @@
 
     floatx16 acc[MI][NJ];
     acc_zero(acc);
-    float4 ra[G::NVA], rb[G::NVB];
-
+    float4 ra[G::NVA];
+    [[maybe_unused]] float4 rb[WT ? 1 : G::NVB];
+
+    auto dma_b = [&](int s) {
+        const uint32_t src = (uint32_t)s * T::STAGE + (uint32_t)lane * 16;
+        const char* dst = reinterpret_cast<const char*>(lds + SA);
+#pragma unroll
+        for (int t = 0; t < T::SLOTS; ++t) {
+            const int q = wv + 4 * t;
+            if (T::NI % 4 == 0 || q < T::NI) dma16_m0(rsw, dst + q * 1024, src + (uint32_t)q * 1024);
+        }
+    };
     auto store = [&]() {
 #pragma unroll
         for (int j = 0; j < G::NVA; ++j) {
@@ -380,14 +435,16 @@
                 for (int p = 0; p < NP; ++p) *reinterpret_cast<uint2*>(lds + p * G::PLA + off) = sp.p[p];
             }
         }
-#pragma unroll
-        for (int j = 0; j < G::NVB; ++j) {
-            const int f = tid + 256 * j;
-            const int t = f / (BN * 4), rem = f - t * (BN * 4);
-            const auto sp = split_np<NP>(rb[j]);
-            const int off = SA + t * NP * G::PLB + s3_off<16>(rem >> 2, (rem & 3) * 4);
-#pragma unroll
-            for (int p = 0; p < NP; ++p) *reinterpret_cast<uint2*>(lds + off + p * G::PLB) = sp.p[p];
+        if constexpr (!WT) {
+#pragma unroll
+            for (int j = 0; j < G::NVB; ++j) {
+                const int f = tid + 256 * j;
+                const int t = f / (BN * 4), rem = f - t * (BN * 4);
+                const auto sp = split_np<NP>(rb[j]);
+                const int off = SA + t * NP * G::PLB + s3_off<16>(rem >> 2, (rem & 3) * 4);
+#pragma unroll
+                for (int p = 0; p < NP; ++p) *reinterpret_cast<uint2*>(lds + off + p * G::PLB) = sp.p[p];
+            }
         }
     };
     auto compute = [&]() {
@@ -406,23 +463,52 @@
         }
     };
 
-    if (S > 0) {
-        la.load(ra);
-        lb.load(rb);
-        store();
-    }
-    __syncthreads();
-    for (int s = 0; s < S; ++s) {
-        const bool more = s + 1 < S;
-        if (more) {
+    if constexpr (WT) {
+        auto a_landed = [&]() {
+#pragma unroll
+            for (int j = 0; j < G::NVA; ++j)
+                asm volatile("" : "+v"(ra[j].x), "+v"(ra[j].y), "+v"(ra[j].z), "+v"(ra[j].w));
+        };
+        if (S > 0) {
+            la.load(ra);
+            a_landed();
+            dma_b(0);
+            store();
+        }
+        asm volatile("s_waitcnt vmcnt(0)" ::: "memory");
+        __syncthreads();
+        for (int s = 0; s < S; ++s) {
+            const bool more = s + 1 < S;
+            if (more) la.load(ra);
+            compute();
+            __syncthreads();
+            if (more) {
+                a_landed();
+                dma_b(s + 1);
+                store();
+                asm volatile("s_waitcnt vmcnt(0)" ::: "memory");
+                __syncthreads();
+            }
+        }
+    } else {
+        if (S > 0) {
             la.load(ra);
             lb.load(rb);
-        }
-        compute();
+            store();
+        }
         __syncthreads();
-        if (more) {
-            store();
+        for (int s = 0; s < S; ++s) {
+            const bool more = s + 1 < S;
+            if (more) {
+                la.load(ra);
+                lb.load(rb);
+            }
+            compute();
             __syncthreads();
+            if (more) {
+                store();
+                __syncthreads();
+            }
         }
     }
     win_epilogue<WM, WN, MI, NJ, CW, Epi>(a, acc, tile.x, n0, b, y0, x0, reinterpret_cast<float*>(lds));
@@ -1079,32 +1165,6 @@
     static constexpr int SA = P * 128, SB = NIB * 8 * 128, STAGE = SA + SB;
     static constexpr int NBUF = NBUF_;
 };
-
-typedef int i32x4_t __attribute__((ext_vector_type(4)));
-struct DmaRsrc {
-    i32x4_t d;
-};
-__device__ __forceinline__ DmaRsrc dma_rsrc(const void* base) {
-    const uint64_t a = reinterpret_cast<uint64_t>(base);
-    DmaRsrc r;
-    r.d[0] = __builtin_amdgcn_readfirstlane((int)(uint32_t)a);
-    r.d[1] = __builtin_amdgcn_readfirstlane((int)((uint32_t)(a >> 32) & 0xFFFF));
-    r.d[2] = (int)kRecords;
-    r.d[3] = 0x00020000;
-    return r;
-}
-__device__ __forceinline__ void dma16(const DmaRsrc& r, const void* lds_dst, uint32_t voff) {
-    const uint32_t m0 = __builtin_amdgcn_readfirstlane(
-        (uint32_t)reinterpret_cast<uintptr_t>((const __attribute__((address_space(3))) void*)lds_dst));
-    asm volatile("s_mov_b32 m0, %2\n\tbuffer_load_dwordx4 %0, %1, 0 offen lds" ::"v"(voff), "s"(r.d), "s"(m0)
-                 : "memory", "m0");
-}
-
-template <int WAITN>
-__device__ __forceinline__ void wgd_wait_barrier() {
-    if constexpr (WAITN == 0) asm volatile("s_waitcnt vmcnt(0)\n\ts_waitcnt lgkmcnt(0)\n\ts_barrier" ::: "memory");
-    else asm volatile("s_waitcnt vmcnt(%0)\n\ts_waitcnt lgkmcnt(0)\n\ts_barrier" ::"n"(WAITN) : "memory");
-}
 
 template <int P, int NBUF = 3>
 __device__ __forceinline__ void conv3x3_wgrad_win_dma_body(const GemmArgs& a) {
diff --git a/camera-aware-neural-networks-for-few-view-depth-estimation_amd/csrc/kernels/kernels.hpp b/camera-aware-neural-networks-for-few-view-depth-estimation_amd/csrc/kernels/kernels.hpp
--- a/camera-aware-neural-networks-for-few-view-depth-estimation_amd/csrc/kernels/kernels.hpp
+++ b/camera-aware-neural-networks-for-few-view-depth-estimation_amd/csrc/kernels/kernels.hpp
@@ -33,10 +33,14 @@
 void set_gemm_engine(int e);
 int gemm_engine();
 void conv3x3_fwd(const float* x, int64_t ldx, int xcoff, int cin, const float* w, int cout, float* y,
-                 int64_t ldy, int ycoff, int B, int H, int W, float* stats, hipStream_t st);
+                 int64_t ldy, int ycoff, int B, int H, int W, float* stats, hipStream_t st, const void* wtwin = nullptr);
+constexpr bool kWtwinDefault = true;
+int conv3x3_wtwin_bn(int cin, int W, int N);
+int64_t conv3x3_wtwin_bytes(int cin, int N);
+bool conv3x3_wtwin_on();
 int conv3x3_stats_rows(int cin, int B, int H, int W, int cout, bool ps = false);
 void conv3x3_dgrad(const float* dz, int cout, const float* wd, int cin, float* dx, int64_t lddx,
-                   int B, int H, int W, hipStream_t st);
+                   int B, int H, int W, hipStream_t st, const void* wtwin = nullptr);
 void conv3x3_wgrad(const float* dz, int cout, const float* x, int64_t ldx, int xcoff, int cin, float* dw,
                    int B, int H, int W, float* slab, int64_t slab_cap, hipStream_t st);
 void convT_fwd(const float* x, int64_t ldx, int cin, const float* wf, const float* bias, int cout,
@@ -183,7 +187,7 @@
     double* part = nullptr; int64_t part_cap = 0;
 };
 int conv3x3_dgrad_bnsums(const float* dz, int cout, const float* wd, int cin, float* dx, int64_t lddx, int B, int H,
-                         int W, const BnSums& bn, hipStream_t st);
+                         int W, const BnSums& bn, hipStream_t st, const void* wtwin = nullptr);
 void bn_relu_pool_fwd(const float* y, int C, const float* scale, const float* shift, float* out, int64_t ldo,
                       void* os, int64_t ldos, int B, int H, int W, bool y_bf16, float* pool, uint8_t* idx,
                       void* pool_split, hipStream_t st);
@@ -245,16 +249,17 @@
                 float max_depth, const EvalAlignWs& ws, int nb, float* table, uint8_t* flags, int64_t base, hipStream_t st);
 void repack_conv_dgrad(const float* w, float* wd, int cout, int cin, hipStream_t st);
 void repack_convT_fwd(const float* wm, float* wf, int cin, int cout, hipStream_t st);
-enum { WPREP_SPLIT = 0, WPREP_DGRAD = 1, WPREP_CONVT = 2, WPREP_TRANSPOSE = 3 };
+enum { WPREP_SPLIT = 0, WPREP_DGRAD = 1, WPREP_CONVT = 2, WPREP_TRANSPOSE = 3, WPREP_WTWIN_FWD = 4, WPREP_WTWIN_DGRAD = 5 };
 struct WPrepJob {
     const float* src;
     float* d32;
     void* d16;
     int kind, cout, cin;
     int blk0;
+    int bn;
     int64_t n;
 };
-constexpr int kWPrepMaxJobs = 24;
+constexpr int kWPrepMaxJobs = 40;
 struct WPrepList {
     WPrepJob job[kWPrepMaxJobs];
     int njobs;
diff --git a/camera-aware-neural-networks-for-few-view-depth-estimation_amd/csrc/kernels/nn_kernels.hip b/camera-aware-neural-networks-for-few-view-depth-estimation_amd/csrc/kernels/nn_kernels.hip
--- a/camera-aware-neural-networks-for-few-view-depth-estimation_amd/csrc/kernels/nn_kernels.hip
+++ b/camera-aware-neural-networks-for-few-view-depth-estimation_amd/csrc/kernels/nn_kernels.hip
@@ -1147,6 +1147,38 @@
     const WPrepJob& jb = list.job[j];
     const int64_t i = ((int64_t)(blockIdx.x - jb.blk0) * 256 + threadIdx.x) * 8;
     if (i >= jb.n) return;
+    if (jb.kind == WPREP_WTWIN_FWD || jb.kind == WPREP_WTWIN_DGRAD) {
+        const bool fwd = jb.kind == WPREP_WTWIN_FWD;
+        const int kc = fwd ? jb.cin : jb.cout, bn = jb.bn;
+        const int S = 3 * (kc / 16);
+        int64_t o = i >> 3;
+        const int hs = (int)(o & 1); o >>= 1;
+        const int row = (int)(o % bn); o /= bn;
+        const int kx = (int)(o % 3); o /= 3;
+        const int s = (int)(o % S);
+        const int nt = (int)(o / S);
+        const int cb = s / 3, ky = s - 3 * cb;
+        const int n = nt * bn + row, tap = 3 * ky + kx;
+        const int k0 = cb * 16 + ((hs ^ ((row >> 3) & 1)) << 3);
+        float4 v0, v1;
+        if (fwd) {
+            const float* p = jb.src + ((int64_t)n * 9 + tap) * jb.cin + k0;
+            v0 = *reinterpret_cast<const float4*>(p);
+            v1 = *reinterpret_cast<const float4*>(p + 4);
+        } else {
+            float t[8];
+#pragma unroll
+            for (int e = 0; e < 8; ++e) t[e] = jb.src[((int64_t)(k0 + e) * 9 + (8 - tap)) * jb.cin + n];
+            v0 = make_float4(t[0], t[1], t[2], t[3]);
+            v1 = make_float4(t[4], t[5], t[6], t[7]);
+        }
+        const Split4 sa = split3(v0), sb = split3(v1);
+        char* dst = static_cast<char*>(jb.d16) + ((int64_t)nt * S + s) * (9 * bn * 32) + (kx * 3 * bn + row) * 32 + hs * 16;
+#pragma unroll
+        for (int p = 0; p < 3; ++p)
+            *reinterpret_cast<uint4*>(dst + p * bn * 32) = make_uint4(sa.p[p].x, sa.p[p].y, sb.p[p].x, sb.p[p].y);
+        return;
+    }
     const int ne = (int)min<int64_t>(8, jb.n - i);
     float v[8];
 #pragma unroll
@@ -1190,6 +1222,11 @@
     for (int j = 0; j < list.njobs; ++j) {
         WPrepJob& jb = list.job[j];
         if (jb.d16 && jb.n % 8) throw std::runtime_error("weight_prep: bf16 twin size not a multiple of 8");
+        if (jb.kind == WPREP_WTWIN_FWD || jb.kind == WPREP_WTWIN_DGRAD) {
+            const int rows = jb.kind == WPREP_WTWIN_FWD ? jb.cout : jb.cin, kc = jb.kind == WPREP_WTWIN_FWD ? jb.cin : jb.cout;
+            if (!jb.d16 || jb.d32 || jb.bn <= 0 || rows % jb.bn || kc % 16 || jb.n != (int64_t)jb.cout * 9 * jb.cin)
+                throw std::runtime_error("weight_prep: weight twin job does not match the window kernels' tiles");
+        }
         jb.blk0 = blocks;
         blocks += (int)cdiv(cdiv(jb.n, 8), (int64_t)256);
     }
diff --git a/profiles/win_compare.py b/profiles/win_compare.py
--- /dev/null
+++ b/profiles/win_compare.py
@@ -0,0 +1,50 @@
+import sys
+
+from summarize import durations, pmc
+
+NAMES = ["SQ_INSTS_VALU", "SQ_VALU_MFMA_BUSY_CYCLES", "SQ_WAVE_CYCLES", "SQ_WAIT_INST_ANY", "GRBM_GUI_ACTIVE"]
+
+
+def table(trace, pm):
+    dur = durations(trace)
+    c = {n: pmc(pm, n) for n in NAMES}
+    rows = {}
+    for k, v in dur.items():
+        if "k_conv3x3_win_s3" not in k:
+            continue
+        avg = {n: (sum(c[n][k]) / len(c[n][k]) if c[n].get(k) else 0.0) for n in NAMES}
+        ns = sum(v) / len(v)
+        act = avg["GRBM_GUI_ACTIVE"] / 8
+        rows[k.replace(" >", ">").replace(", true>", ">")] = {
+            "launches": len(v), "us": ns / 1e3, "valu": avg["SQ_INSTS_VALU"], "ghz": act / ns if ns else 0.0,
+            "mfma": avg["SQ_VALU_MFMA_BUSY_CYCLES"] / (1024 * act) if act else 0.0,
+            "stalled": avg["SQ_WAIT_INST_ANY"] / avg["SQ_WAVE_CYCLES"] if avg["SQ_WAVE_CYCLES"] else 0.0}
+    return rows
+
+
+def main():
+    a = table(sys.argv[1], sys.argv[2])
+    b = table(sys.argv[3], sys.argv[4]) if len(sys.argv) > 4 else None
+    f = "{us:.1f} | {valu:.3e} | {mfma:.3f} | {stalled:.2f} | {ghz:.2f}"
+    head = "avg us | VALU / launch | MFMA busy | stalled | GHz"
+    if b is None:
+        print(f"| kernel | launches | {head} |\n|---|---|---|---|---|---|---|")
+        for k, r in sorted(a.items(), key=lambda kv: -kv[1]["us"] * kv[1]["launches"]):
+            print(f"| `{k}` | {r['launches']} | " + f.format(**r) + " |")
+        return
+    print(f"| kernel | launches | A: {head} | B: {head} | us B/A | VALU B/A |")
+    print("|---|---|" + "---|" * 12)
+    ta = tb = 0.0
+    for k, r in sorted(a.items(), key=lambda kv: -kv[1]["us"] * kv[1]["launches"]):
+        s = b.get(k)
+        if not s:
+            continue
+        ta += r["us"] * r["launches"]
+        tb += s["us"] * s["launches"]
+        print(f"| `{k}` | {r['launches']} | " + f.format(**r) + " | " + f.format(**s) +
+              f" | {s['us'] / r['us']:.3f} | {s['valu'] / r['valu'] if r['valu'] else 0:.3f} |")
+    print(f"\nsum over the launches of the traced run: A {ta / 1e3:.2f} ms, B {tb / 1e3:.2f} ms ({tb / ta:.4f})")
+
+
+if __name__ == "__main__":
+    main()
```
